# play-with-HOI-generation/HOIG

Hardware: AMD Instinct MI355X
Metric: HOGAN train images/sec at 256x256 (higher is better)
Workload: dtype f16x3 fwd (both operands split hi+lo on fp16, 3 MFMAs per product) / bf16x2 bwd (dy split hi+lo, weights and x single bf16, 2 MFMAs per product), f32 accumulate; 1 GPU; 256x256 HO3Dv3-shaped synthetic, batch 8 per GPU, G+D full step (generator_spade_attn, VGG19 surrogate weights); global_batch=8, parallelism=dp1

## Files before the change

### hoig_amd/_lib.py

```python
import ctypes
import os
import re
import subprocess

_HERE = os.path.dirname(os.path.abspath(__file__))
LIB_PATH = os.path.join(_HERE, 'csrc', '_build', 'libhoig_hip.so')
HEADER_PATH = os.path.join(os.path.dirname(_HERE), 'include', 'hoig_kernels.h')

OK, EINVAL, ELAUNCH, EUNSUPPORTED = 0, -1, -2, -3
ACT_NONE, ACT_RELU, ACT_LRELU, ACT_TANH, ACT_SIGMOID = 0, 1, 2, 3, 4
PREC_F32, PREC_BF16X3, PREC_BF16, PREC_F16X2, PREC_F16F6 = 0, 1, 2, 3, 4
LOSS_L1, LOSS_MSE, LOSS_BCE = 0, 1, 2
POOL_MAX, POOL_AVG = 0, 1
JPEG_SUBSEQ_BYTES = 64
_ERR = {EINVAL: 'invalid argument', ELAUNCH: 'kernel launch failed', EUNSUPPORTED: 'unsupported shape'}


class HoigKernelError(RuntimeError):
    pass


class ConvDesc(ctypes.Structure):
    _fields_ = [(n, ctypes.c_int32) for n in ('B', 'Hi', 'Wi', 'Ci', 'Ho', 'Wo', 'Co', 'R', 'S', 'stride', 'pad',
                                              'transposed', 'act')] + \
               [('slope', ctypes.c_float), ('precision', ctypes.c_int32)]


def build(verbose=False):
    script = os.path.join(_HERE, 'csrc', 'build.sh')
    out = subprocess.run(['bash', script], stdout=subprocess.PIPE, stderr=subprocess.STDOUT, text=True)
    if verbose or out.returncode != 0:
        print(out.stdout)
    if out.returncode != 0:
        raise RuntimeError('hipcc build of libhoig_hip.so failed')
    return LIB_PATH


def declared_symbols():
    text = open(HEADER_PATH).read()
    return sorted(set(re.findall(r'\b(hoig_[a-z0-9_]+)\s*\(', text)) - {'hoig_stream_t'})


_vp, _i, _i64, _f, _d = ctypes.c_void_p, ctypes.c_int, ctypes.c_int64, ctypes.c_float, ctypes.c_double
_SIGS = {
    'hoig_conv2d_fwd': [ctypes.POINTER(ConvDesc), _vp, _vp, _vp, _vp, _vp],
    'hoig_conv2d_bwd_data': [ctypes.POINTER(ConvDesc), _vp, _vp, _vp, _vp],
    'hoig_conv2d_fwd_heads': [ctypes.POINTER(ConvDesc), _vp, _vp, _vp, _vp, ctypes.c_uint64, _vp],
    'hoig_conv2d_bwd_weight': [ctypes.POINTER(ConvDesc), _vp, _vp, _vp, _vp, _vp],
    'hoig_pack_conv_weight_bf16': [_vp, _i, _i, _i, _i, _vp, _vp, _vp],
    'hoig_pack_conv_weights_bf16_all': [_vp, _vp, _i, _i64, _vp, _vp, _vp, _vp, _vp],
    'hoig_conv2d_fwd_packed': [ctypes.POINTER(ConvDesc), _vp, _vp, _vp, _vp, _vp, _vp],
    'hoig_conv2d_bwd_data_packed': [ctypes.POINTER(ConvDesc), _vp, _vp, _vp, _vp, _vp],
    'hoig_conv2d_fwd_packed_stats': [ctypes.POINTER(ConvDesc), _vp, _vp, _vp, _vp, _vp, _vp, _vp],
    'hoig_conv2d_fwd_stats': [ctypes.POINTER(ConvDesc), _vp, _vp, _vp, _vp, _vp, _vp],
    'hoig_conv2d_cat_fwd_packed_stats': [ctypes.POINTER(ConvDesc), _vp, _i, _vp, _vp, _vp, _vp, _vp, _vp, _vp],
    'hoig_inorm_stats_from_sums': [_vp, _i, _i, _i, _f, _vp, _vp, _vp, _vp],
    'hoig_conv2d_bwd_data_packed_add': [ctypes.POINTER(ConvDesc), _vp, _vp, _vp, _vp, _vp, _vp],
    'hoig_pack_conv_weight_f6': [_vp, _i, _i, _i, _vp, _vp, _vp],
    'hoig_conv2d_fwd_f6': [ctypes.POINTER(ConvDesc), _vp, _vp, _vp, _vp, _vp, _vp, _vp],
    'hoig_pack_conv_weights_f6_all': [_vp, _vp, _i, _i64, _vp, _vp, _vp],
    'hoig_conv2d_cat_fwd_f6': [ctypes.POINTER(ConvDesc), _vp, _i, _vp, _vp, _vp, _vp, _vp, _vp, _vp],
    'hoig_conv2d_fwd_f6_ex': [ctypes.POINTER(ConvDesc), _vp, _i, _vp, _vp, _vp, _vp, _vp, _vp, _vp, _i, _vp, _vp, _vp],
    'hoig_conv2d_cat_fwd_packed': [ctypes.POINTER(ConvDesc), _vp, _i, _vp, _vp, _vp, _vp, _vp, _vp],
    'hoig_conv2d_cat_bwd_data_packed': [ctypes.POINTER(ConvDesc), _vp, _vp, _vp, _vp, _i, _vp, _vp],
    'hoig_split_planes_bf16': [_vp, _vp, _i64, _i, _vp],
    'hoig_conv2d_bwd_weight_split': [ctypes.POINTER(ConvDesc), _vp, _vp, _vp, _vp],
    'hoig_conv2d_bwd_data_packed_split': [ctypes.POINTER(ConvDesc), _vp, _vp, _vp, _vp, _vp, _vp],
    'hoig_conv2d_fwd_packed_pair': [ctypes.POINTER(ConvDesc)] + [_vp] * 11,
    'hoig_conv2d_bwd_data_packed_split_pair': [ctypes.POINTER(ConvDesc)] + [_vp] * 11,
    'hoig_conv2d_bwd_weight_split_pair': [ctypes.POINTER(ConvDesc)] + [_vp] * 7,
    'hoig_conv2d_cat_bwd_weight': [ctypes.POINTER(ConvDesc), _vp, _i, _vp, _vp, _vp, _vp, _vp],
    'hoig_inorm_stats': [_vp, _i, _i, _i, _f, _vp, _vp, _vp, _vp],
    'hoig_inorm_apply': [_vp, _vp, _vp, _i, _vp, _vp, _i, _f, _vp, _vp, _i, _i, _i, _vp],
    'hoig_inorm_apply_ld': [_vp, _vp, _vp, _i, _vp, _vp, _i, _i, _f, _vp, _vp, _i, _i, _i, _vp],
    'hoig_inorm_bwd_ld': [_vp, _vp, _vp, _i, _vp, _vp, _i, _vp, _vp, _i, _f, _vp, _vp, _vp, _i, _i, _i, _vp, _vp],
    'hoig_inorm_fwd_fused': [_vp, _i, _vp, _vp, _i, _i, _f, _vp, _f, _vp, _vp, _vp, _i, _i, _i, _vp],
    'hoig_inorm_bwd_fused': [_vp, _vp, _vp, _i, _vp, _vp, _i, _vp, _vp, _i, _f, _vp, _vp, _vp, _i, _i, _i, _vp],
    'hoig_inorm_bwd_add_ld': [_vp, _vp, _vp, _i, _vp, _vp, _i, _vp, _vp, _i, _f, _vp, _vp, _vp, _vp, _i, _i, _i, _vp, _vp],
    'hoig_inorm_bwd_add_ld_split': [_vp, _vp, _vp, _i, _vp, _vp, _i, _vp, _vp, _i, _f, _vp, _vp, _vp, _vp, _i, _i, _i, _vp, _vp],
    'hoig_inorm_bwd_fused_add_split': [_vp, _vp, _vp, _i, _vp, _vp, _i, _vp, _vp, _i, _f, _vp, _vp, _vp, _vp, _i, _i, _i, _vp],
    'hoig_inorm_fold': [_vp, _vp, _vp, _vp, _i, _i, _vp, _vp, _i, _vp],
    'hoig_conv2d_fwd_packed_normin': [_vp, _vp, _i, _vp, _vp, _vp, _vp, _vp, _vp, _i, _vp, _vp, _vp],
    'hoig_unsplit_planes_bf16': [_vp, _vp, _i64, _i, _vp],
    'hoig_inorm_bwd_fused_add': [_vp, _vp, _vp, _i, _vp, _vp, _i, _vp, _vp, _i, _f, _vp, _vp, _vp, _vp, _i, _i, _i, _vp],
    'hoig_inorm_bwd': [_vp, _vp, _vp, _i, _vp, _vp, _vp, _vp, _i, _f, _vp, _vp, _vp, _i, _i, _i, _vp, _vp],
    'hoig_replicate_pad_fwd': [_vp, _vp, _i, _i, _i, _i, _i, _vp],
    'hoig_replicate_pad_bwd': [_vp, _vp, _i, _i, _i, _i, _i, _vp],
    'hoig_replicate_pad_bwd_add': [_vp, _vp, _vp, _i, _i, _i, _i, _i, _vp],
    'hoig_attn_pixel_fwd': [_vp] * 10 + [_i, _i, _i, _i, _vp],
    'hoig_attn_pixel_bwd': [_vp] * 10 + [_i, _i, _i, _i, _vp],
    'hoig_attn_build_index': [_vp, _vp, _i, _i, _i, _vp],
    'hoig_attn_src_gather': [_vp, _vp, _vp, _vp, _vp, _i, _i, _i, _i, _vp],
    'hoig_attn_gs_gather': [_vp, _vp, _vp, _vp, _i, _i, _i, _vp],
    'hoig_block_extractor_forward': [_vp, _vp, _vp] + [_i] * 7 + [_vp],
    'hoig_block_extractor_backward': [_vp] * 5 + [_i] * 7 + [_vp],
    'hoig_local_attn_reshape_forward': [_vp, _vp] + [_i] * 4 + [_vp],
    'hoig_local_attn_reshape_backward': [_vp, _vp] + [_i] * 4 + [_vp],
    'hoig_grid_sample_fwd': [_vp, _vp, _vp] + [_i] * 6 + [_vp],
    'hoig_grid_sample_bwd': [_vp, _vp, _vp] + [_i] * 6 + [_vp],
    'hoig_resize_bilinear_ac': [_vp, _vp] + [_i] * 6 + [_vp],
    'hoig_resize_nearest': [_vp, _vp] + [_i] * 6 + [_vp],
    'hoig_attn_flow': [_vp, _vp, _i, _i, _vp],
    'hoig_maxpool2_fwd': [_vp, _vp] + [_i] * 4 + [_vp],
    'hoig_maxpool2_bwd': [_vp, _vp, _vp, _vp] + [_i] * 4 + [_vp],
    'hoig_nchw_to_nhwc': [_vp, _vp] + [_i] * 4 + [_vp],
    'hoig_nhwc_to_nchw': [_vp, _vp] + [_i] * 4 + [_vp],
    'hoig_copy_channels': [_vp, _vp, _i64, _i, _i, _i, _i, _i, _i, _vp],
    'hoig_cat2_channels': [_vp, _i, _vp, _i, _vp, _i64, _vp],
    'hoig_add': [_vp, _vp, _vp, _i64, _vp],
    'hoig_add_act': [_vp, _vp, _vp, _i, _f, _i64, _vp],
    'hoig_act_bwd': [_vp, _vp, _vp, _i, _f, _i64, _vp],
    'hoig_act_bwd_colsum': [_vp, _vp, _vp, _vp, _i, _f, _i64, _i, _vp],
    'hoig_colsum_accum': [_vp, _vp, _i64, _i, _vp],
    'hoig_compose_fwd': [_vp] * 6 + [_i64, _i, _vp],
    'hoig_compose_bwd': [_vp] * 11 + [_i64, _i, _vp],
    'hoig_loss_fwd_bwd': [_i, _vp, _vp, _f, _f, _vp, _vp, _i64, _vp],
    'hoig_tv_fwd_bwd': [_vp, _f, _f, _vp, _vp, _i, _i, _i, _vp],
    'hoig_loss_accumulate': [_i, _vp, _vp, _f, _f, _vp, _vp, _i64, _vp],
    'hoig_tv_accumulate': [_vp, _f, _f, _vp, _vp, _i, _i, _i, _vp],
    'hoig_sum': [_vp, _vp, _i64, _vp],
    'hoig_sum_scaled': [_vp, _f, _vp, _i64, _vp],
    'hoig_adam_step': [_vp, _vp, _vp, _vp, _i64, _d, _d, _d, _d, _i, _f, _vp],
    'hoig_adam_tick': [_vp, _vp, _vp],
    'hoig_adam_step_dev': [_vp, _vp, _vp, _vp, _i64, _vp, _f, _vp],
    'hoig_resize_linear_u8': [_vp, _i, _i, _i, _i, _vp, _i, _i, _vp],
    'hoig_warp_affine_u8': [_vp, _i, _i, _i, _i, _vp, _i, _i, _i, _vp, _vp],
    'hoig_adam_pack_step': [_vp, _vp, _vp, _vp, _vp, _f, _vp, _i, _i64, _vp, _i64, _vp, _vp, _vp, _vp, _vp],
    'hoig_stream_create': [ctypes.POINTER(ctypes.c_void_p)],
    'hoig_stream_destroy': [_vp],
    'hoig_stream_scratch_set': [_vp, _vp, _i64],
    'hoig_tensor2im_u8': [_vp, _vp] + [_i] * 6 + [_vp],
    'hoig_tensor2im_nhwc_u8': [_vp, _vp, _i64, _i, _vp],
    'hoig_prep_texture': [_vp] * 9,
    'hoig_prep_lookup': [_vp] * 5 + [_i] + [_vp] * 8,
    'hoig_prep_assemble': [_i] + [_vp] * 17 + [_i] + [_vp] * 6,
    'hoig_rasterize_fim_wim': [_vp, _i, _i, _i, _f, _f, _vp, _vp, _vp, _vp],
    'hoig_pack_conv_weight_wino': [_vp, _i, _i, _vp, _vp, _vp],
    'hoig_conv2d_fwd_wino': [ctypes.POINTER(ConvDesc), _vp, _vp, _vp, _vp, _vp, _vp],
    'hoig_project_faces': [_vp, _i, _vp, _i, _vp, _vp, _i, _i, _f, _f, _vp, _vp],
    'hoig_prep_texture_batched': [_i, _vp, _vp, _i64, _vp, _vp, _vp, _vp, _vp, _vp, _vp],
    'hoig_prep_lookup_batched': [_i, _vp, _vp, _vp, _vp, _vp, _vp, _vp, _vp, _i64, _vp, _vp, _vp, _vp, _vp, _vp],
    'hoig_mano_lbs': [_vp, _vp, _vp, _vp, _vp, _vp, _vp, _vp, _vp, _i, _i, _vp, _vp, _vp, _vp, _vp, _i, _vp, _i, _vp],
    'hoig_pool2d_fwd': [_vp, _vp] + [_i] * 10 + [_vp],
    'hoig_stage_images_u8': [_vp, _vp] + [_i] * 7 + [_vp, _vp],
    'hoig_pad2d': [_vp, _vp] + [_i] * 6 + [_vp],
    'hoig_global_avgpool': [_vp, _vp, _i, _i, _i, _vp],
    'hoig_lpips_layer': [_vp, _vp, _vp, _vp, _i, _i, _i, _vp, _vp],
    'hoig_ssim': [_vp, _vp, _vp, _vp, _i, _i, _i, _i, _f, _f, _f, _i, _f, _vp, _vp],
    'hoig_jpeg_entropy_host': [_vp, _i64, _vp, _i, _vp, _i64, _vp, _i64, _vp],
    'hoig_jpeg_decode_bgr_u8': [_vp, _i64, _vp, _vp, _i, _vp, _i64, _vp, _i64, _vp, _vp, _i64, _vp],
    'hoig_jpeg_reconstruct_bgr_u8': [_vp, _vp, _i, _vp, _i64, _vp, _i64, _vp],
    'hoig_jpeg_entropy_par_host': [_vp, _i64, _vp, _i, _vp, _i64, _i, _i, _vp, _i64, _vp, _vp, _vp, _i64],
    'hoig_jpeg_decode_bgr_u8_par': [_vp, _i64, _vp, _vp, _i, _vp, _i64, _vp, _i64, _vp, _vp, _i64, _i, _vp],
    'hoig_pil_bilinear_ksize': [_i, _i],
    'hoig_pil_bilinear_table': [_i, _i, _vp],
    'hoig_resize_pil_bilinear_u8_host': [_vp, _i, _i, _i, _i, _vp, _i, _i],
    'hoig_resize_pil_bilinear_u8': [_vp, _i, _i, _i, _i, _vp, _i, _i, _vp, _vp, _vp, _vp],
}


def _load():
    if not os.path.exists(LIB_PATH):
        raise ImportError(
            'hoig_amd: %s not found. The HIP extension is mandatory (no CPU / eager fallback exists); build it with '
            '`python -c "import __graft_entry__ as g; g.build()"` or `bash hoig_amd/csrc/build.sh`.' % LIB_PATH)
    lib = ctypes.CDLL(LIB_PATH)
    for name, args in _SIGS.items():
        fn = getattr(lib, name)
        fn.argtypes = args
        fn.restype = ctypes.c_int
    lib.hoig_inorm_workspace_bytes.argtypes = [_i, _i, _i]
    lib.hoig_inorm_workspace_bytes.restype = ctypes.c_int64
    lib.hoig_set_f6_min_tiles.argtypes = [_i]
    lib.hoig_set_f6_min_tiles.restype = ctypes.c_int
    lib.hoig_f6_plane_bytes.argtypes = [_i, _i, _i]
    lib.hoig_f6_plane_bytes.restype = ctypes.c_int64
    lib.hoig_wino_plane_halfs.argtypes = [_i, _i]
    lib.hoig_wino_plane_halfs.restype = ctypes.c_int64
    lib.hoig_attn_index_ints.argtypes = [_i, _i, _i]
    lib.hoig_attn_index_ints.restype = ctypes.c_int64
    lib.hoig_rasterize_workspace_bytes.restype = ctypes.c_size_t
    lib.hoig_rasterize_workspace_bytes.argtypes = [ctypes.c_int, ctypes.c_int]
    lib.hoig_set_tuning.argtypes = [ctypes.c_char_p, _i]
    lib.hoig_set_tuning.restype = ctypes.c_int
    lib.hoig_stream_scratch_bytes.argtypes = []
    lib.hoig_stream_scratch_bytes.restype = ctypes.c_int64
    lib.hoig_conv2d_bwd_weight_scratch_bytes.argtypes = [ctypes.POINTER(ConvDesc)]
# ... 46 lines not shown
```

### hoig_amd/csrc/conv_bf16_common.h

```cpp
#pragma once
#include "common.h"

namespace hoig_detail {

#define HOIG_NS_SWITCH(ns, ...)                                                \
    do {                                                                       \
        if ((ns) == 2) { constexpr int NSX = 2; __VA_ARGS__; }                 \
        else if ((ns) == 3) { constexpr int NSX = 3; __VA_ARGS__; }            \
        else { constexpr int NSX = 1; __VA_ARGS__; }                           \
    } while (0)
__host__ __device__ constexpr int ns_a(int nsx) { return nsx == 1 ? 1 : 2; }
__host__ __device__ constexpr int ns_b(int nsx) { return nsx == 2 ? 2 : 1; }
inline int ns_of_precision(int precision) {
    return precision == HOIG_PREC_BF16X3 ? 2 : (precision == HOIG_PREC_F16X2 ? 3 : 1);
}
inline bool is_16bit_precision(int precision) {
    return precision == HOIG_PREC_BF16X3 || precision == HOIG_PREC_BF16 || precision == HOIG_PREC_F16X2;
}

typedef __bf16 bf2_t __attribute__((ext_vector_type(2)));
typedef float f2_t __attribute__((ext_vector_type(2)));
__device__ __forceinline__ unsigned cvt2(float a, float b) {
    f2_t v = {a, b};
    return __builtin_bit_cast(unsigned, __builtin_convertvector(v, bf2_t));
}
typedef _Float16 h2_t __attribute__((ext_vector_type(2)));
typedef _Float16 f16x8 __attribute__((ext_vector_type(8)));
constexpr float W_SCALE_F16 = 256.f;
__device__ __forceinline__ unsigned cvt2h(float a, float b) {
    f2_t v = {a, b};
    return __builtin_bit_cast(unsigned, __builtin_convertvector(v, h2_t));
}
__device__ __forceinline__ void split4h(const float4 v, uint2 &hi, uint2 &lo) {
    hi.x = cvt2h(v.x, v.y);
    hi.y = cvt2h(v.z, v.w);
    const h2_t h0 = __builtin_bit_cast(h2_t, hi.x), h1 = __builtin_bit_cast(h2_t, hi.y);
    lo.x = cvt2h(v.x - (float)h0[0], v.y - (float)h0[1]);
    lo.y = cvt2h(v.z - (float)h1[0], v.w - (float)h1[1]);
}
template <bool F16>
__device__ __forceinline__ f32x16 mfma16(const bf16x8 a, const bf16x8 b, const f32x16 c) {
    if constexpr (F16)
        return __builtin_amdgcn_mfma_f32_32x32x16_f16(__builtin_bit_cast(f16x8, a), __builtin_bit_cast(f16x8, b), c, 0, 0, 0);
    else
        return __builtin_amdgcn_mfma_f32_32x32x16_bf16(a, b, c, 0, 0, 0);
}

__device__ __forceinline__ void split4(const float4 v, uint2 &hi, uint2 &lo) {
    hi.x = cvt2(v.x, v.y);
    hi.y = cvt2(v.z, v.w);
    const float r0 = v.x - __uint_as_float(hi.x << 16), r1 = v.y - __uint_as_float(hi.x & 0xFFFF0000u);
    const float r2 = v.z - __uint_as_float(hi.y << 16), r3 = v.w - __uint_as_float(hi.y & 0xFFFF0000u);
    lo.x = cvt2(r0, r1);
    lo.y = cvt2(r2, r3);
}
template <bool F16>
__device__ __forceinline__ void split4t(const float4 v, uint2 &hi, uint2 &lo) {
    if constexpr (F16) split4h(v, hi, lo);
    else split4(v, hi, lo);
}

__host__ __device__ __forceinline__ size_t plane_index(int n, int k, int K) {
    return ((size_t)(n >> 5) * (K >> 5) + (k >> 5)) * 1024 + (n & 31) * 32 + (((((k & 31) >> 3) ^ ((n >> 2) & 3))) << 3) +
           (k & 7);
}

struct HaloArgs {
    const float *A;
    const unsigned short *Wh, *Wl;
    const float *bias;
    float *C;
    int Bn, H, W, Cg;
    int N, K;
    int pad;
    int flip;
    int act;
    float slope;
    int nblk_n, nblk;
    int tiles_x, tiles_y;
    int nmajor;
    int f16;
    float oscale;
    const float *A2;
    int cg1;
    float *C2;
    int n1;
    const float *addend;
    const float *in_scale = nullptr, *in_shift = nullptr;
    int in_relu_c0 = 0;
    int b_split;
    const float *A_g2;
    const unsigned short *Wh_g2, *Wl_g2;
    const float *bias_g2, *addend_g2;
    float *C_g2;
    int a_split;
    double *stats;
};

struct Geom {
    int Bn, Hg, Wg, Cg;
    int Hp, Wp;
    int R, S, stride, pad;
    int gatherT, phase_major, tile_skip;
};

struct Args {
    const float *A;
    const unsigned short *Wh;
    const unsigned short *Wl;
    const float *bias;
    float *C;
    Geom g;
    int M, N, K;
    int act;
    float slope;
    int nblk_n, nblk;
    int ksplit, steps_per_split;
    int f16;
    float oscale;
};

__device__ __forceinline__ void decode_m(const Geom &g, int m, int &b, int &hp, int &wp) {
    if (!g.phase_major) {
        const int hw = g.Hp * g.Wp;
        b = m / hw;
        const int rem = m - b * hw;
        hp = rem / g.Wp;
        wp = rem - hp * g.Wp;
    } else {
        const int W2 = g.Wp >> 1, q = (g.Hp >> 1) * W2, bq = g.Bn * q;
        const int ph = m / bq;
        const int rem = m - ph * bq;
        b = rem / q;
        const int r2 = rem - b * q;
        const int h2 = r2 / W2;
        hp = 2 * h2 + (ph >> 1);
        wp = 2 * (r2 - h2 * W2) + (ph & 1);
    }
}
__device__ __forceinline__ int row_base(const Geom &g, int p) { return g.gatherT ? p + g.pad : p * g.stride - g.pad; }
__device__ __forceinline__ int gcoord(const Geom &g, int base, int r, int lim) {
    if (!g.gatherT) {
        const int c = base + r;
        return (c >= 0 && c < lim) ? c : -1;
    }
    int t = base - r;
    if (t < 0) return -1;
    if (g.stride == 2) {
        if (t & 1) return -1;
        t >>= 1;
    } else if (g.stride != 1) {
        if (t % g.stride) return -1;
        t /= g.stride;
    }
    return t < lim ? t : -1;
}
__device__ __forceinline__ bool tap_alive(const Geom &g, int hp, int wp, int rs) {
    const int r = rs / g.S, s = rs - r * g.S;
    return (((hp + g.pad - r) & 1) == 0) && (((wp + g.pad - s) & 1) == 0);
}

struct WFlatArgs {
    const float *X, *DY;
    float *DW, *DB;
    int Ci, Co, Wc, HWc, Q, Ho, Wo, HPOS;
    int nblk_ci, nblk, n_mtiles, mt_per_split;
};
int launch_wgrad_flat5(const float *x, const float *dy, float *dw, float *dbias, int Bn, int Hi, int Wi, int Ci, int Co, int ns,
                       hipStream_t st);

int launch_igemm_m16(Args a, int ns, int cfg, hipStream_t st);

struct FlatArgs {
    const float *A;
    const unsigned short *Wh, *Wl;
    const float *bias;
    float *C;
    const float *addend;
    int Bn, Hc, Wc;
    int Hs, Ws, oy, ox;
    int Hd, Wd;
    int KS, Cg, N, K, flip, f16;
    int act;
    float slope, oscale;
    int HWc, Q, HP;
    int nblk, nblk_n, steps_per_split;
};
int launch_flat_m16(FlatArgs a, int ns, hipStream_t st);
int launch_halo5_m16(FlatArgs a, int ns, hipStream_t st);

struct WHaloArgs {
    const float *DY, *X, *X2;
    int ci1;
    float *DW, *DB;
    int Bn, H, W, Co, Ci;
    int Hin, Win, pad;
    int tout;
    int tiles_x, tiles_y, n_mtiles, mt_per_split;
    int nblk_ci, nblk;
    int b_split;
    const float *DY_g2, *X_g2;
    float *DW_g2;
};

int launch_halo_s2_m16p(const HaloArgs &a, int ns, bool scatter, bool rows8, hipStream_t st);
int launch_dgrad_thin(const float *dy, const unsigned short *wh, const unsigned short *wl, float *dx, int M, int N, int ns, hipStream_t st);
int launch_wgrad_dma(const WHaloArgs &a, int ns, dim3 grid, hipStream_t st);

int launch_halo3_m16(HaloArgs a, int ns, int bn, hipStream_t st);
int launch_halo_s2_m16(const HaloArgs &a, int ns, bool scatter, hipStream_t st);

}
```

### hoig_amd/csrc/conv_flat16.hip

```cpp
#include "conv_bf16_common.h"
#include "tuning.h"

namespace hoig_detail {
namespace {

template <bool F16>
__device__ __forceinline__ f32x4 mfma_m16(const bf16x8 a, const bf16x8 b, const f32x4 c) {
    if constexpr (F16)
        return __builtin_amdgcn_mfma_f32_16x16x32_f16(__builtin_bit_cast(f16x8, a), __builtin_bit_cast(f16x8, b), c, 0, 0, 0);
    else
        return __builtin_amdgcn_mfma_f32_16x16x32_bf16(a, b, c, 0, 0, 0);
}
typedef unsigned u2_t __attribute__((ext_vector_type(2)));
constexpr int round128(int v) { return (v + 127) / 128 * 128; }

constexpr int PT = 256, BN = 128, TPS = 3, HSL = 8;
constexpr int W23 = BN * 32 + 64, PLANE_W = round128(W23 + BN * 32);

template <int NSX, int KS, bool F16, bool SPLITK, bool WDMA = false>
__global__ __launch_bounds__(512) void conv_flat_m16_kernel(const FlatArgs p) {
    constexpr int NS = NSX == 1 ? 1 : 2, NB = NSX == 2 ? 2 : 1;
    constexpr int NT = 512, WN = 2, MT = 4, NTW = 4, KK = KS * KS;
    constexpr int NGRP = (KK + TPS - 1) / TPS;
    constexpr int BBUF = TPS * NB * PLANE_W;
// ... 164 lines not shown
                    } else {
                        if (NS == 2) acc[j][m] = mfma_m16<F16>(wc.h, pc.l[m], acc[j][m]);
                        if (NB == 2) acc[j][m] = mfma_m16<F16>(wc.l, pc.h[m], acc[j][m]);
                        acc[j][m] = mfma_m16<F16>(wc.h, pc.h[m], acc[j][m]);
                    }
                }
                __builtin_amdgcn_sched_barrier(0);
            }
        }
        if constexpr (WDMA) {
            if (dma_step >= 0) {
#pragma unroll
                for (int i = 0; i < NPW; ++i)
                    if (i >= ntap * NTW) dma_piece(dma_step, bbuf ^ 1, i);
            }
        }
    };

    if (T > 0) {
        halo_load(s_begin / NGRP);
        halo_store();
        if constexpr (WDMA) {
#pragma unroll
            for (int i = 0; i < NPW; ++i) dma_piece(0, 0, i);
        } else {
            load_b(0);
            store_b(0);
            if (T > 1) load_b(1);
        }
    }
    if constexpr (WDMA) asm volatile("s_waitcnt vmcnt(0)" ::: "memory");
    __syncthreads();
    int bbuf = 0;
#pragma unroll 1
    for (int step = 0; step < T; ++step) {
        const int cb = (s_begin + step) / NGRP, g = (s_begin + step) - cb * NGRP;
        const bool more = step + 1 < T;
        const bool boundary = more && g == NGRP - 1;
        if constexpr (!WDMA) {
            if (more) store_b(bbuf ^ 1);
            if (step + 2 < T) load_b(step + 2);
        }
        if (boundary) halo_load(cb + 1);
        compute(g, bbuf, (WDMA && more) ? step + 1 : -1);
        if (boundary) {
            __syncthreads();
            halo_store();
        }
        if constexpr (WDMA) asm volatile("s_waitcnt vmcnt(0)" ::: "memory");
        __syncthreads();
        bbuf ^= 1;
    }

    auto dest = [&](int q) -> long {
        if (q >= p.Q) return -1;
        const int b = q / p.HWc, rem = q - b * p.HWc;
        const int y = rem / p.Wc, x = rem - y * p.Wc;
        if (y >= p.Hd || x >= p.Wd) return -1;
        return ((long)(b * p.Hd + y) * p.Wd + x) * p.N;
    };
    if (!SPLITK) {
        const float nslope = p.act == HOIG_ACT_NONE ? 1.f : (p.act == HOIG_ACT_RELU ? 0.f : p.slope);
        const bool special = p.act == HOIG_ACT_TANH || p.act == HOIG_ACT_SIGMOID;
#pragma unroll
        for (int m = 0; m < MT; ++m) {
            const long d = dest(q0 + wm * 64 + m * 16 + l15);
            if (d < 0) continue;
#pragma unroll
            for (int j = 0; j < NTW; ++j) {
                const int n = n0 + wn * 64 + j * 16 + lg * 4;
                if (n < p.N) {
                    float4 o = make_float4(acc[j][m][0] * p.oscale, acc[j][m][1] * p.oscale, acc[j][m][2] * p.oscale,
                                           acc[j][m][3] * p.oscale);
                    if (p.bias) {
                        const float4 bv = *reinterpret_cast<const float4 *>(p.bias + n);
                        o.x += bv.x; o.y += bv.y; o.z += bv.z; o.w += bv.w;
                    }
                    o.x = fast_act(o.x, nslope, special, p.act, p.slope); o.y = fast_act(o.y, nslope, special, p.act, p.slope);
                    o.z = fast_act(o.z, nslope, special, p.act, p.slope); o.w = fast_act(o.w, nslope, special, p.act, p.slope);
                    if (p.addend) {
                        const float4 ad = *reinterpret_cast<const float4 *>(p.addend + d + n);
                        o.x += ad.x; o.y += ad.y; o.z += ad.z; o.w += ad.w;
                    }
                    *reinterpret_cast<float4 *>(p.C + d + n) = o;
                }
            }
        }
    } else {
        const int l31 = lane & 31, lh = lane >> 5;
#pragma unroll
        for (int m = 0; m < MT; ++m)
#pragma unroll
            for (int r = 0; r < 4; ++r) {
                long d[2];
#pragma unroll
                for (int h = 0; h < 2; ++h) d[h] = dest(q0 + wm * 64 + m * 16 + r + 8 * lh + 4 * h);
#pragma unroll
                for (int j = 0; j < NTW; j += 2) {
                    const int n = n0 + wn * 64 + j * 16 + l31;
                    const u2_t sw = __builtin_amdgcn_permlane16_swap(__float_as_uint(acc[j][m][r]), __float_as_uint(acc[j + 1][m][r]),
                                                                     false, false);
#pragma unroll
                    for (int h = 0; h < 2; ++h)
                        if (d[h] >= 0 && n < p.N) {
                            float v = __uint_as_float(sw[h]) * p.oscale;
                            if (blockIdx.y == 0 && p.bias) v += p.bias[n];
                            atomicAdd(p.C + d[h] + n, v);
                        }
                }
            }
    }
}

template <int NSX, int KS, bool F16, bool SPLITK>
int launch_one(const FlatArgs &a, dim3 grid, size_t shm, hipStream_t st) {
    if (hoig_tuning(HOIG_TUNE_WDMA16) >= 2) {
        static hoig_once once_d;
        if (!once_d.done()) {
            if (hipFuncSetAttribute(reinterpret_cast<const void *>(&conv_flat_m16_kernel<NSX, KS, F16, SPLITK, true>),
                                    hipFuncAttributeMaxDynamicSharedMemorySize, 160 * 1024) != hipSuccess)
                return HOIG_ELAUNCH;
            once_d.set();
        }
        conv_flat_m16_kernel<NSX, KS, F16, SPLITK, true><<<grid, 512, shm, st>>>(a);
        HOIG_LAUNCH_CHECK();
        return HOIG_OK;
    }
    static hoig_once once;
    if (!once.done()) {
        if (hipFuncSetAttribute(reinterpret_cast<const void *>(&conv_flat_m16_kernel<NSX, KS, F16, SPLITK>),
                                hipFuncAttributeMaxDynamicSharedMemorySize, 160 * 1024) != hipSuccess)
            return HOIG_ELAUNCH;
        once.set();
    }
    conv_flat_m16_kernel<NSX, KS, F16, SPLITK><<<grid, 512, shm, st>>>(a);
    HOIG_LAUNCH_CHECK();
    return HOIG_OK;
}

template <int KS>
int launch_ks(const FlatArgs &a, int ns, dim3 grid, size_t shm, bool split, hipStream_t st) {
    if (split) {
        if (a.f16) HOIG_NS_SWITCH(ns, return launch_one<NSX, KS, true, true>(a, grid, shm, st));
        else HOIG_NS_SWITCH(ns, return launch_one<NSX, KS, false, true>(a, grid, shm, st));
    }
    if (a.f16) HOIG_NS_SWITCH(ns, return launch_one<NSX, KS, true, false>(a, grid, shm, st));
    else HOIG_NS_SWITCH(ns, return launch_one<NSX, KS, false, false>(a, grid, shm, st));
    return HOIG_EINVAL;
}

}

int launch_flat_m16(FlatArgs a, int ns, hipStream_t st) {
    const int KS = a.KS;
    if ((KS != 3 && KS != 5) || a.N % 128 || a.Cg % 32) return HOIG_EUNSUPPORTED;
    a.HWc = a.Hc * a.Wc;
    a.Q = a.Bn * a.HWc;
    a.HP = PT + (KS - 1) * (a.Wc + 1);
    if (a.HP * 8 > HSL * 512) return HOIG_EUNSUPPORTED;
    const int p23 = round128(a.HP * 32) + 64, plane_p = round128(p23 + a.HP * 32);
    const size_t shm = (size_t)ns_a(ns) * plane_p + 2 * TPS * ns_b(ns) * PLANE_W;
    if (shm > 160 * 1024) return HOIG_EUNSUPPORTED;
    const int n_mt = (int)hoig_cdiv(a.Q, PT);
    a.nblk_n = a.N / BN;
    a.nblk = n_mt * a.nblk_n;
    const int ncb = a.Cg >> 5;
    const int steps = ncb * ((KS * KS + TPS - 1) / TPS);
    int split = 1;
    if (a.nblk <= 128 && !a.addend && a.act == HOIG_ACT_NONE) {
        split = 256 / a.nblk;
        if (split > steps / 8) split = steps / 8;
        if (split < 1) split = 1;
    }
    a.steps_per_split = (int)hoig_cdiv(steps, split);
    split = (int)hoig_cdiv(steps, a.steps_per_split);
    dim3 grid(a.nblk, split);
    if (split > 1 && hipMemsetAsync(a.C, 0, (size_t)a.Bn * a.Hd * a.Wd * a.N * sizeof(float), st) != hipSuccess) return HOIG_ELAUNCH;
    return KS == 3 ? launch_ks<3>(a, ns, grid, shm, split > 1, st) : launch_ks<5>(a, ns, grid, shm, split > 1, st);
}

}
```

### hoig_amd/csrc/conv_halo16.hip

```cpp
#include "conv_bf16_common.h"
#include "conv_m16_common.h"
#include "tuning.h"

namespace hoig_detail {
namespace {

template <int WM, int BN>
struct M16Layout {
    static constexpr int TH = 2 * WM, HW = 34, HPIX = (TH + 2) * HW;
    static constexpr int PHALF = HPIX * 32;
    static constexpr int P23 = round128(PHALF) + 64;
    static constexpr int PLANE_P = round128(P23 + PHALF);
    static constexpr int W23 = BN * 32 + 64;
    static constexpr int PLANE_W = round128(W23 + BN * 32);
    static constexpr size_t bytes(int nsx) { return (size_t)ns_a(nsx) * PLANE_P + 2 * 3 * ns_b(nsx) * PLANE_W; }
};

template <int NSX, int WM, int WN, int BN, bool F16, bool ASPLIT = false, bool WDMA = false, bool NORMIN = false>
__global__ __launch_bounds__(64 * WM * WN) void conv_halo3_m16_kernel(const HaloArgs p) {
    constexpr int NS = NSX == 1 ? 1 : 2, NB = NSX == 2 ? 2 : 1;
    using LY = M16Layout<WM, BN>;
    constexpr int KS = 3, TH = LY::TH, HW = LY::HW, HPIX = LY::HPIX;
    constexpr int NT = 64 * WM * WN;
    constexpr int P23 = LY::P23, PLANE_P = LY::PLANE_P, W23 = LY::W23, PLANE_W = LY::PLANE_W;
// ... 219 lines not shown
            if (t + 1 < KS) {
#pragma unroll
                for (int q = 0; q < PPG; ++q)
                    if (j * PPG + q < MT) read_p(pf[(t + 1) & 1], t + 1, j * PPG + q);
            }
            if constexpr (WDMA) {
                if (dma_step >= 0 && g < NPW) dma_piece(dma_step, bbuf ^ 1, g);
            }
            __builtin_amdgcn_sched_barrier(0);
            const PF &pc = pf[t & 1];
            const WF &wc = wf[g & 1];
#pragma unroll
            for (int m = 0; m < MT; ++m) {
                if (NS == 2) acc[j][m] = mfma_m16<F16>(wc.h, pc.l[m], acc[j][m]);
                if (NB == 2) acc[j][m] = mfma_m16<F16>(wc.l, pc.h[m], acc[j][m]);
                acc[j][m] = mfma_m16<F16>(wc.h, pc.h[m], acc[j][m]);
            }
            __builtin_amdgcn_sched_barrier(0);
        }
    };

    halo_load(0);
    halo_store();
    if constexpr (WDMA) {
#pragma unroll
        for (int i = 0; i < NPW; ++i) dma_piece(0, 0, i);
        asm volatile("s_waitcnt vmcnt(0)" ::: "memory");
    } else {
        load_b(0);
        store_b(0);
        if (T > 1) load_b(1);
    }
    __syncthreads();
    int bbuf = 0;
#pragma unroll 1
    for (int step = 0; step < T; ++step) {
        const int cb = step / KS, r = step - cb * KS;
        const bool more = step + 1 < T;
        const bool boundary = more && r == KS - 1;
        if constexpr (!WDMA) {
            if (more) store_b(bbuf ^ 1);
            if (step + 2 < T) load_b(step + 2);
        }
        if (boundary) halo_load(cb + 1);
        compute(r, bbuf, (WDMA && more) ? step + 1 : -1);
        if (boundary) {
            __syncthreads();
            halo_store();
        }
        if constexpr (WDMA) asm volatile("s_waitcnt vmcnt(0)" ::: "memory");
        __syncthreads();
        bbuf ^= 1;
    }

    const float nslope = p.act == HOIG_ACT_NONE ? 1.f : (p.act == HOIG_ACT_RELU ? 0.f : p.slope);
    const bool special = p.act == HOIG_ACT_TANH || p.act == HOIG_ACT_SIGMOID;
    float4 bias_r[NTW];
#pragma unroll
    for (int j = 0; j < NTW; ++j) {
        const int n = n0 + wn * (NTW * 16) + j * 16 + lg * 4;
        bias_r[j] = (gbias && n < p.N) ? *reinterpret_cast<const float4 *>(gbias + n) : make_float4(0.f, 0.f, 0.f, 0.f);
    }
    float st1[NTW][4], st2[NTW][4];
#pragma unroll
    for (int j = 0; j < NTW; ++j)
#pragma unroll
        for (int q = 0; q < 4; ++q) st1[j][q] = st2[j][q] = 0.f;
#pragma unroll
    for (int m = 0; m < MT; ++m) {
        const int oy = y0 + wm * 2 + (m >> 1), ox = x0 + (m & 1) * 16 + l15;
        const size_t pix = ((size_t)bi * p.H + oy) * p.W + ox;
#pragma unroll
        for (int j = 0; j < NTW; ++j) {
            const int n = n0 + wn * (NTW * 16) + j * 16 + lg * 4;
            if (n < p.N) {
                float v[4];
                const float bq[4] = {bias_r[j].x, bias_r[j].y, bias_r[j].z, bias_r[j].w};
#pragma unroll
                for (int q = 0; q < 4; ++q) v[q] = fast_act(acc[j][m][q] * p.oscale + bq[q], nslope, special, p.act, p.slope);
                if (gadd) {
                    const float4 ad = *reinterpret_cast<const float4 *>(gadd + pix * p.N + n);
                    v[0] += ad.x; v[1] += ad.y; v[2] += ad.z; v[3] += ad.w;
                }
#pragma unroll
                for (int q = 0; q < 4; ++q) {
                    st1[j][q] += v[q];
                    st2[j][q] += v[q] * v[q];
                }
                const float4 o = make_float4(v[0], v[1], v[2], v[3]);
                if (!p.C2) *reinterpret_cast<float4 *>(gC + pix * p.N + n) = o;
                else if (n < p.n1) *reinterpret_cast<float4 *>(gC + pix * p.n1 + n) = o;
                else *reinterpret_cast<float4 *>(p.C2 + pix * (p.N - p.n1) + (n - p.n1)) = o;
            }
        }
    }
    if (p.stats) m16_stats_epilogue<NTW, WM, BN, NT>(st1, st2, smem, p.stats, b, p.N, n0, wm, wn, lane, tid);
}

template <int NSX, int BN, bool SCATTER, bool F16>
__global__ __launch_bounds__(256) void conv_halo_s2_m16_kernel(const HaloArgs p) {
    constexpr int NS = NSX == 1 ? 1 : 2, NB = NSX == 2 ? 2 : 1;
    constexpr int TH = 4, TW = 32, NT = 256, WN = 2;
    constexpr int RB = BN * 4 / NT;
    constexpr int HH = TH + 1, HW = TW + 1, HPIX = HH * HW;
    constexpr int PHALF = HPIX * 32, P23 = round128(PHALF) + 64, PLANE_P = round128(P23 + PHALF);
    constexpr int W23 = BN * 32 + 64, PLANE_W = round128(W23 + BN * 32);
    constexpr int MT = 4, NTW = BN / (16 * WN);
    __shared__ __attribute__((aligned(16))) unsigned char smem[NS * PLANE_P + 2 * NB * PLANE_W];
    unsigned char *Ph = smem, *Pl = smem + PLANE_P;
    unsigned char *Wbase = smem + NS * PLANE_P;

    const int tid = threadIdx.x, lane = tid & 63, wave = tid >> 6;
    const int l15 = lane & 15, lg = lane >> 4;
    const int wm = wave / WN, wn = wave % WN;
    int tile = hoig_xcd_remap(blockIdx.x, p.nblk);
    int P = 0, Q = 0;
    if (SCATTER) {
        P = (tile >> 1) & 1;
        Q = tile & 1;
        tile >>= 2;
    }
    int mt_ = tile / p.nblk_n;
    const int n0 = (tile % p.nblk_n) * BN;
    const int tx_ = mt_ % p.tiles_x;
    mt_ /= p.tiles_x;
    const int ty_ = mt_ % p.tiles_y, b = mt_ / p.tiles_y;
    const int y0 = ty_ * TH, x0 = tx_ * TW;

    const int brow = tid >> 2, bpos = tid & 3;
    const unsigned short *wrow_h[RB], *wrow_l[RB];
    int woff[RB];
#pragma unroll
    for (int i = 0; i < RB; ++i) {
        const int row = brow + (NT / 4) * i;
        const int n = n0 + row;
        const size_t o = ((size_t)(n >> 5) * (p.K >> 5)) * 1024 + (n & 31) * 32 + bpos * 8;
        wrow_h[i] = n < p.N ? p.Wh + o : nullptr;
        wrow_l[i] = (NB == 2 && n < p.N) ? p.Wl + o : nullptr;
        const int c = bpos ^ ((row >> 2) & 3);
        woff[i] = (c >> 1) * W23 + row * 32 + (c & 1) * 16;
    }
    int wread[NTW], pread[MT];
#pragma unroll
    for (int j = 0; j < NTW; ++j) wread[j] = (lg >> 1) * W23 + (wn * (NTW * 16) + j * 16 + l15) * 32 + (lg & 1) * 16;
#pragma unroll
    for (int m = 0; m < MT; ++m)
        pread[m] = (lg >> 1) * P23 + ((wm * 2 + (m >> 1)) * HW + (m & 1) * 16 + l15) * 32 + (lg & 1) * 16;

    f32x4 acc[NTW][MT];
#pragma unroll
    for (int j = 0; j < NTW; ++j)
#pragma unroll
        for (int m = 0; m < MT; ++m) acc[j][m] = f32x4{0.f, 0.f, 0.f, 0.f};

    struct Step {
        int cb, ntap, tap[2], pp, qq;
        bool load;
    };
    const int spc = SCATTER ? ((P ? 2 : 1) * (Q ? 2 : 1) + 1) / 2 : 5;
    const int ncb = p.Cg >> 5, T = ncb * spc;
    auto step_info = [&](int step) -> Step {
        Step s_;
        s_.cb = step / spc;
        const int idx = step - s_.cb * spc;
        s_.pp = s_.qq = 0;
        if (!SCATTER) {
// ... 307 lines not shown
```

### hoig_amd/csrc/conv_igemm_bf16.hip

```cpp
#include "conv_bf16_common.h"
#include "tuning.h"
#include <cstdlib>

#ifndef HOIG_HALO_BSTAGES
#define HOIG_HALO_BSTAGES 1
#endif

namespace {
using namespace hoig_detail;


template <int BK>
__device__ __forceinline__ int lds_swz(int row) {
    return BK == 32 ? ((row >> 2) & 3) : ((row >> 1) & 7);
}
template <int BK>
__device__ __forceinline__ int lds_off(int row, int k) {
    return row * (BK * 2) + (((k >> 3) ^ lds_swz<BK>(row)) << 4) + ((k & 4) << 1);
}

template <int BM, int BN, int WM, int WN, int NSX, int BK, bool F16>
__global__ __launch_bounds__(WM * WN * 64) void igemm_bf16_kernel(const Args p) {
    constexpr int NS = NSX == 1 ? 1 : 2, NB = NSX == 2 ? 2 : 1;
    constexpr int NT = WM * WN * 64;
// ... 847 lines not shown
            if (more) load_b(step + 1);
            if (boundary) halo_load(cb + 1);
            compute(r, 0, 0);
            if (more) {
                __syncthreads();
                if (boundary) halo_store(0);
                store_b(0);
                __syncthreads();
            }
        }
    }

    const float nslope = p.act == HOIG_ACT_NONE ? 1.f : (p.act == HOIG_ACT_RELU ? 0.f : p.slope);
    const bool special = p.act == HOIG_ACT_TANH || p.act == HOIG_ACT_SIGMOID;
    float bias_r[TN];
#pragma unroll
    for (int j = 0; j < TN; ++j) {
        const int n = n0 + wn * (TN * 32) + j * 32 + l31;
        bias_r[j] = (p.bias && n < p.N) ? p.bias[n] : 0.f;
    }
    float st1[TN], st2[TN];
#pragma unroll
    for (int j = 0; j < TN; ++j) st1[j] = st2[j] = 0.f;
#pragma unroll
    for (int i = 0; i < TM; ++i) {
        const int oy = y0 + wm * TM + i;
#pragma unroll
        for (int r = 0; r < 16; ++r) {
            const int ox = x0 + (r & 3) + 8 * (r >> 2) + 4 * lh;
            const size_t pix = ((size_t)b * p.H + oy) * p.W + ox;
#pragma unroll
            for (int j = 0; j < TN; ++j) {
                const int n = n0 + wn * (TN * 32) + j * 32 + l31;
                if (n < p.N) {
                    float v = acc[i][j][r] * p.oscale;
                    v += bias_r[j];
                    v = fast_act(v, nslope, special, p.act, p.slope);
                    if (p.addend) v += p.addend[pix * p.N + n];
                    st1[j] += v;
                    st2[j] += v * v;
                    if (!p.C2) p.C[pix * p.N + n] = v;
                    else if (n < p.n1) p.C[pix * p.n1 + n] = v;
                    else p.C2[pix * (p.N - p.n1) + (n - p.n1)] = v;
                }
            }
        }
    }
    if (p.stats) halo_stats_epilogue<TN, WM, WN, NT>(st1, st2, smem, p.stats, b, p.N, n0, wm, wn, lane);
}

template <int NS, int WM, int WN, int BN, int MODE>
int launch_halo3_one(const HaloArgs &a, hipStream_t st) {
    constexpr int HPIX = (2 * WM + 2) * 34;
    constexpr size_t shm = (MODE == 1 ? 2 : 1) * (ns_a(NS) * (HPIX * 80)) + (MODE == 0 ? 1 : 2) * (3 * ns_b(NS) * (BN * 64));
    static hoig_once once;
    if (!once.done()) {
        if (hipFuncSetAttribute(reinterpret_cast<const void *>(&conv_halo3_bf16_kernel<NS, WM, WN, BN, MODE, true>),
                                hipFuncAttributeMaxDynamicSharedMemorySize, (int)shm) != hipSuccess ||
            hipFuncSetAttribute(reinterpret_cast<const void *>(&conv_halo3_bf16_kernel<NS, WM, WN, BN, MODE, false>),
                                hipFuncAttributeMaxDynamicSharedMemorySize, (int)shm) != hipSuccess)
            return HOIG_ELAUNCH;
        once.set();
    }
    if (a.f16) conv_halo3_bf16_kernel<NS, WM, WN, BN, MODE, true><<<a.nblk, 64 * WM * WN, shm, st>>>(a);
    else conv_halo3_bf16_kernel<NS, WM, WN, BN, MODE, false><<<a.nblk, 64 * WM * WN, shm, st>>>(a);
    HOIG_LAUNCH_CHECK();
    return HOIG_OK;
}


int launch_halo3(HaloArgs a, int ns, hipStream_t st) {
    a.tiles_x = a.W / 32;
    a.tiles_y = a.H / 4;
    a.nmajor = 1;
    const bool n64 = (a.N % 128) != 0 || (a.C2 && a.n1 % 128 != 0);
    a.nblk_n = (int)hoig_cdiv(a.N, n64 ? 64 : 128);
    a.nblk = a.Bn * a.tiles_x * a.tiles_y * a.nblk_n;
    if (n64) {
        if (a.H % 8 == 0 && a.nblk / 2 >= 256) {
            a.tiles_y = a.H / 8;
            a.nblk = a.Bn * a.tiles_x * a.tiles_y * a.nblk_n;
            return launch_halo3_m16(a, ns, 64, st);
        }
        if (a.a_split || a.b_split || a.in_scale) return HOIG_EUNSUPPORTED;
        HOIG_NS_SWITCH(ns, return launch_halo3_one<NSX, 2, 2, 64, 0>(a, st));
    }
    if (a.H % 8 == 0 && a.nblk / 2 < 256 && a.nblk >= 192 && a.N % 128 == 0) {
        a.tiles_y = a.H / 8;
        a.nblk = a.Bn * a.tiles_x * a.tiles_y * a.nblk_n;
        return launch_halo3_m16(a, ns, 128, st);
    }
    if (a.H % 8 == 0 && a.nblk / 2 < 256 && a.nblk >= 192) {
        a.tiles_y = a.H / 8;
        a.nblk_n = a.N / 64;
        a.nblk = a.Bn * a.tiles_x * a.tiles_y * a.nblk_n;
        return launch_halo3_m16(a, ns, 64, st);
    }
    if (a.H % 8 == 0 && a.nblk / 2 >= 256) {
        a.tiles_y = a.H / 8;
        a.nblk = a.Bn * a.tiles_x * a.tiles_y * a.nblk_n;
        return launch_halo3_m16(a, ns, 128, st);
    }
    if (a.a_split || a.b_split || a.in_scale) return HOIG_EUNSUPPORTED;
    const bool wide = a.nblk < 384;
    HOIG_NS_SWITCH(ns, return wide ? launch_halo3_one<NSX, 2, 4, 128, 1>(a, st) : launch_halo3_one<NSX, 2, 2, 128, 0>(a, st));
    return HOIG_EINVAL;
}

template <int NSX, int BN, bool SCATTER, bool F16>
__global__ __launch_bounds__(256) void conv_halo_s2_bf16_kernel(const HaloArgs p) {
    constexpr int NS = NSX == 1 ? 1 : 2, NB = NSX == 2 ? 2 : 1;
    constexpr int TH = 4, TW = 32, NT = 256, WN = 2;
    constexpr int RB = BN * 4 / NT;
    constexpr int HH = TH + 1, HW = TW + 1, HPIX = HH * HW;
    constexpr int AROW = 80;
    constexpr int PLANE_A = HPIX * AROW, PLANE_B = BN * 64;
    constexpr int TM = 2, TN = BN / (32 * WN);
    __shared__ __attribute__((aligned(16))) unsigned char smem[NS * PLANE_A + 2 * NB * PLANE_B];
    unsigned char *Ah = smem, *Al = smem + PLANE_A;
    unsigned char *Bbase = smem + NS * PLANE_A;

    const int tid = threadIdx.x, lane = tid & 63, wave = tid >> 6;
    const int l31 = lane & 31, lh = lane >> 5;
    const int wm = wave / WN, wn = wave % WN;
    int tile = hoig_xcd_remap(blockIdx.x, p.nblk);
    int P = 0, Q = 0;
    if (SCATTER) {
        P = (tile >> 1) & 1;
        Q = tile & 1;
        tile >>= 2;
    }
    int mt = tile / p.nblk_n;
    const int n0 = (tile % p.nblk_n) * BN;
    const int tx_ = mt % p.tiles_x;
    mt /= p.tiles_x;
    const int ty_ = mt % p.tiles_y, b = mt / p.tiles_y;
    const int y0 = ty_ * TH, x0 = tx_ * TW;

    const int brow = tid >> 2, bchunk = tid & 3;
    const unsigned short *wrow_h[RB], *wrow_l[RB];
    int boff[RB];
#pragma unroll
    for (int i = 0; i < RB; ++i) {
        const int n = n0 + brow + (NT / 4) * i;
        const size_t o = plane_index(n, bchunk * 8, p.K);
        wrow_h[i] = n < p.N ? p.Wh + o : nullptr;
        wrow_l[i] = (NB == 2 && n < p.N) ? p.Wl + o : nullptr;
        const int row = brow + (NT / 4) * i;
        boff[i] = row * 64 + ((bchunk ^ ((row >> 2) & 3)) << 4);
    }
    int aread[TM], bread[TN];
#pragma unroll
    for (int i = 0; i < TM; ++i) aread[i] = ((wm * TM + i) * HW + l31) * AROW + lh * 16;
#pragma unroll
    for (int j = 0; j < TN; ++j) {
        const int row = wn * (TN * 32) + j * 32 + l31;
        bread[j] = row * 64 + ((lh ^ ((row >> 2) & 3)) << 4);
    }
    f32x16 acc[TM][TN];
#pragma unroll
    for (int i = 0; i < TM; ++i)
#pragma unroll
        for (int j = 0; j < TN; ++j)
#pragma unroll
            for (int r = 0; r < 16; ++r) acc[i][j][r] = 0.f;

    struct Step {
        int cb, ntap, tap[2], pp, qq;
        bool load;
    };
    const int spc = SCATTER ? ((P ? 2 : 1) * (Q ? 2 : 1) + 1) / 2 : 5;
    const int ncb = p.Cg >> 5, T = ncb * spc;
    auto step_info = [&](int step) -> Step {
        Step s_;
        s_.cb = step / spc;
        const int idx = step - s_.cb * spc;
        s_.pp = s_.qq = 0;
        if (!SCATTER) {
            s_.load = idx != 1;
            switch (idx) {
                case 0: s_.pp = 1; s_.qq = 1; s_.ntap = 2; s_.tap[0] = 0; s_.tap[1] = 2; break;
                case 1: s_.pp = 1; s_.qq = 1; s_.ntap = 2; s_.tap[0] = 6; s_.tap[1] = 8; break;
                case 2: s_.pp = 1; s_.qq = 0; s_.ntap = 2; s_.tap[0] = 1; s_.tap[1] = 7; break;
                case 3: s_.pp = 0; s_.qq = 1; s_.ntap = 2; s_.tap[0] = 3; s_.tap[1] = 5; break;
                default: s_.ntap = 1; s_.tap[0] = 4; s_.tap[1] = 4; break;
            }
// ... 177 lines not shown
                    st2[j] += v * v;
                    p.C[pix * p.N + n] = v;
                }
            }
        }
    }
    if (p.stats) halo_stats_epilogue<TN, 2, WN, NT>(st1, st2, smem, p.stats, b, p.N, n0, wm, wn, lane);
}

template <bool SCATTER>
int launch_halo_s2(HaloArgs a, int ns, hipStream_t st) {
    const int ch = SCATTER ? a.H : a.H / 2, cw = SCATTER ? a.W : a.W / 2;
    a.tiles_x = cw / 32;
    a.tiles_y = ch / 4;
    const bool n64 = (a.N % 128) != 0;
    a.nblk_n = a.N / (n64 ? 64 : 128);
    a.nblk = a.Bn * a.tiles_x * a.tiles_y * a.nblk_n * (SCATTER ? 4 : 1);
    a.nmajor = 0;
    if (hoig_tuning(HOIG_TUNE_S2_16) != 0 && !(SCATTER && n64 && ns == 2)) return launch_halo_s2_m16(a, ns, SCATTER, st);
    if (n64) {
        if (a.f16) HOIG_NS_SWITCH(ns, conv_halo_s2_bf16_kernel<NSX, 64, SCATTER, true><<<a.nblk, 256, 0, st>>>(a));
        else HOIG_NS_SWITCH(ns, conv_halo_s2_bf16_kernel<NSX, 64, SCATTER, false><<<a.nblk, 256, 0, st>>>(a));
    } else {
        if (a.f16) HOIG_NS_SWITCH(ns, conv_halo_s2_bf16_kernel<NSX, 128, SCATTER, true><<<a.nblk, 256, 0, st>>>(a));
        else HOIG_NS_SWITCH(ns, conv_halo_s2_bf16_kernel<NSX, 128, SCATTER, false><<<a.nblk, 256, 0, st>>>(a));
    }
    HOIG_LAUNCH_CHECK();
    return HOIG_OK;
}

template <int KS>
int launch_halo(HaloArgs a, int ns, hipStream_t st) {
    a.tiles_x = a.W / 32;
    a.tiles_y = a.H / 4;
    const bool n64 = (a.N % 128) != 0;
    a.nblk_n = (int)hoig_cdiv(a.N, n64 ? 64 : 128);
    a.nblk = a.Bn * a.tiles_x * a.tiles_y * a.nblk_n;
    if (n64) {
        if (a.f16) HOIG_NS_SWITCH(ns, conv_halo_bf16_kernel<KS, NSX, 2, 64, true><<<a.nblk, 256, 0, st>>>(a));
        else HOIG_NS_SWITCH(ns, conv_halo_bf16_kernel<KS, NSX, 2, 64, false><<<a.nblk, 256, 0, st>>>(a));
        HOIG_LAUNCH_CHECK();
        return HOIG_OK;
    }
    const bool wide = a.nblk < 384;
    if (wide) {
        if (a.f16) HOIG_NS_SWITCH(ns, conv_halo_bf16_kernel<KS, NSX, 4, 128, true><<<a.nblk, 512, 0, st>>>(a));
        else HOIG_NS_SWITCH(ns, conv_halo_bf16_kernel<KS, NSX, 4, 128, false><<<a.nblk, 512, 0, st>>>(a));
    } else {
        if (a.f16) HOIG_NS_SWITCH(ns, conv_halo_bf16_kernel<KS, NSX, 2, 128, true><<<a.nblk, 256, 0, st>>>(a));
        else HOIG_NS_SWITCH(ns, conv_halo_bf16_kernel<KS, NSX, 2, 128, false><<<a.nblk, 256, 0, st>>>(a));
    }
    HOIG_LAUNCH_CHECK();
    return HOIG_OK;
}

struct InNorm {
    const float *scale, *shift;
    int relu_c0;
};
struct PairSet {
    const float *a;
    const unsigned short *wh, *wl;
    const float *bias, *addend;
    float *c;
};

struct Conv {
    const hoig_conv_desc *d = nullptr;
    const float *a = nullptr;
    const unsigned short *wh = nullptr, *wl = nullptr;
    const float *bias = nullptr;
    float *c = nullptr;
    bool dgrad = false;
    hipStream_t st = nullptr;
    const float *a2 = nullptr;
    int cg1 = 0;
    float *c2 = nullptr;
    int n1 = 0;
    const float *addend = nullptr;
    double *stats = nullptr;
    bool a_split = false;
    const PairSet *g2 = nullptr;
    const InNorm *in = nullptr;
};

int run(const Conv &q) {
    const hoig_conv_desc *d = q.d;
    const float *a = q.a, *bias = q.bias, *a2 = q.a2, *addend = q.addend;
    const unsigned short *wh = q.wh, *wl = q.wl;
    float *c = q.c, *c2 = q.c2;
    const bool dgrad = q.dgrad, a_split = q.a_split;
    const int cg1 = q.cg1, n1 = q.n1;
    double *stats = q.stats;
    const PairSet *g2 = q.g2;
    const InNorm *in = q.in;
    hipStream_t st = q.st;
    if (in && (dgrad || d->R != 3 || d->S != 3 || d->stride != 1 || d->pad != 1 || d->transposed || a_split || g2))
        return HOIG_EUNSUPPORTED;
    Args p;
    p.A = a; p.Wh = wh; p.Wl = wl; p.bias = bias; p.C = c;
    p.f16 = dgrad ? 0 : 1;
    p.oscale = dgrad ? 1.f : 1.f / W_SCALE_F16;
    Geom &g = p.g;
    g.Bn = d->B;
    if (!dgrad) {
        g.Hg = d->Hi; g.Wg = d->Wi; g.Cg = d->Ci; g.Hp = d->Ho; g.Wp = d->Wo;
        g.gatherT = d->transposed ? 1 : 0;
        p.M = d->B * d->Ho * d->Wo; p.N = d->Co; p.K = d->R * d->S * d->Ci;
        p.act = d->act; p.slope = d->slope;
    } else {
        g.Hg = d->Ho; g.Wg = d->Wo; g.Cg = d->Co; g.Hp = d->Hi; g.Wp = d->Wi;
        g.gatherT = d->transposed ? 0 : 1;
        p.M = d->B * d->Hi * d->Wi; p.N = d->Ci; p.K = d->R * d->S * d->Co;
        p.act = HOIG_ACT_NONE; p.slope = 0.f;
    }
    g.R = d->R; g.S = d->S; g.stride = d->stride; g.pad = d->pad;
    g.phase_major = 0; g.tile_skip = 0;
    if (g.Cg % 32 != 0) return HOIG_EUNSUPPORTED;
    if (g.gatherT && g.stride == 2 && ((g.Hp | g.Wp) & 1)) return HOIG_EUNSUPPORTED;
    const int ns = ns_of_precision(d->precision);
    if (ns == 2 && !wl) return HOIG_EINVAL;
    const long t128 = hoig_cdiv(p.M, 128);
    if (p.N <= 32 || p.N % 32 != 0) return HOIG_EUNSUPPORTED;
    if (dgrad && !d->transposed && d->R == 1 && d->S == 1 && d->stride == 1 && d->pad == 0 && g.Cg == 128 &&
        p.N >= 1024 && p.N % 64 == 0 && p.M % 128 == 0 && !a2 && !c2 && !addend && !stats)
        return launch_dgrad_thin(a, wh, wl, c, p.M, p.N, ns, st);
    if (!d->transposed && d->stride == 1 && d->R == d->S && 2 * d->pad == d->R - 1 && (d->R == 1 || d->R == 3 || d->R == 5) &&
        d->Wi % 32 == 0 && d->Hi % 4 == 0 && p.N % 64 == 0 &&
        (long)(g2 ? 2 : 1) * d->B * (d->Hi / 4) * (d->Wi / 32) * ((p.N + 127) / 128) >= 160) {
        HaloArgs h;
        h.b_split = 0;
        h.A_g2 = nullptr; h.Wh_g2 = h.Wl_g2 = nullptr; h.bias_g2 = h.addend_g2 = nullptr; h.C_g2 = nullptr;
        h.A = a; h.Wh = wh; h.Wl = wl; h.bias = bias; h.C = c;
        h.A2 = a2; h.cg1 = cg1; h.C2 = c2; h.n1 = n1;
        h.addend = addend;
        h.stats = stats;
        h.a_split = a_split ? 1 : 0;
        h.in_scale = in ? in->scale : nullptr; h.in_shift = in ? in->shift : nullptr; h.in_relu_c0 = in ? in->relu_c0 : 0;
        if (a_split && (d->R != 3 || a2 || !dgrad)) return HOIG_EUNSUPPORTED;
        if ((addend || stats) && c2) return HOIG_EUNSUPPORTED;
        if (stats && d->R != 3) return HOIG_EUNSUPPORTED;
        if ((a2 || c2) && d->R != 3) return HOIG_EUNSUPPORTED;
        if (a2 && (cg1 % 32 || cg1 <= 0 || cg1 >= g.Cg)) return HOIG_EINVAL;
        if (c2 && (n1 % 64 || n1 <= 0 || n1 >= p.N)) return HOIG_EINVAL;
        h.Bn = d->B; h.H = d->Hi; h.W = d->Wi; h.Cg = g.Cg; h.N = p.N; h.K = p.K;
        if (g2) {
            if (d->R != 3 || a2 || c2 || stats) return HOIG_EUNSUPPORTED;
            h.Bn = 2 * d->B; h.b_split = d->B;
            h.A_g2 = g2->a; h.Wh_g2 = g2->wh; h.Wl_g2 = g2->wl; h.bias_g2 = g2->bias; h.addend_g2 = g2->addend; h.C_g2 = g2->c;
        }
        h.pad = d->pad;
        h.flip = dgrad ? 1 : 0;
        h.act = p.act; h.slope = p.slope;
            h.f16 = p.f16; h.oscale = p.oscale;
        if (d->R == 1) return launch_halo<1>(h, ns, st);
        if (d->R == 3) return launch_halo3(h, ns, st);
        return launch_halo<5>(h, ns, st);
    }
    if (a2 || c2 || a_split || g2 || in) return HOIG_EUNSUPPORTED;
    if (hoig_tuning(HOIG_TUNE_FLAT5) >= 2 && !d->transposed && d->stride == 1 && d->R == 3 && d->S == 3 && d->pad == 1 &&
        p.N % 128 == 0 && !stats) {
        FlatArgs f;
        f.A = a; f.Wh = wh; f.Wl = wl; f.bias = bias; f.C = c; f.addend = addend;
        f.Bn = d->B; f.Hc = d->Hi + 2; f.Wc = d->Wi + 2; f.KS = 3; f.act = p.act; f.slope = p.slope;
        f.Cg = g.Cg; f.N = p.N; f.K = p.K; f.flip = dgrad ? 1 : 0; f.f16 = p.f16; f.oscale = p.oscale;
        f.Hs = d->Hi; f.Ws = d->Wi; f.oy = f.ox = 1; f.Hd = d->Hi; f.Wd = d->Wi;
        const int rc = launch_flat_m16(f, ns, st);
        if (rc != HOIG_EUNSUPPORTED) return rc;
    }
    if (hoig_tuning(HOIG_TUNE_FLAT5) != 0 && !d->transposed && d->stride == 1 && d->R == 5 && d->S == 5 && d->pad == 0 &&
        d->Ho == d->Hi - 4 && d->Wo == d->Wi - 4 && p.N % 128 == 0 && !stats) {
        FlatArgs f;
        f.A = a; f.Wh = wh; f.Wl = wl; f.bias = bias; f.C = c; f.addend = addend;
        f.Bn = d->B; f.Hc = d->Hi; f.Wc = d->Wi; f.KS = 5; f.act = p.act; f.slope = p.slope;
        f.Cg = g.Cg; f.N = p.N; f.K = p.K; f.flip = dgrad ? 1 : 0; f.f16 = p.f16; f.oscale = p.oscale;
        if (!dgrad) {
            f.Hs = d->Hi; f.Ws = d->Wi; f.oy = f.ox = 0; f.Hd = d->Ho; f.Wd = d->Wo;
        } else {
            f.Hs = d->Ho; f.Ws = d->Wo; f.oy = f.ox = 4; f.Hd = d->Hi; f.Wd = d->Wi;
        }
        const int rc = launch_flat_m16(f, ns, st);
        if (rc != HOIG_EUNSUPPORTED) return rc;
        if (hoig_tuning(HOIG_TUNE_HALO5) != 0) {
            const int rc5 = launch_halo5_m16(f, ns, st);
            if (rc5 != HOIG_EUNSUPPORTED) return rc5;
        }
    }
    if (d->stride == 2 && d->R == 3 && d->S == 3 && d->pad == 1 && d->Hi % 2 == 0 && d->Wi % 2 == 0 &&
        p.N % 64 == 0) {
        const int fine_h = d->transposed ? d->Ho : d->Hi, fine_w = d->transposed ? d->Wo : d->Wi;
        const int coarse_h = d->transposed ? d->Hi : d->Ho, coarse_w = d->transposed ? d->Wi : d->Wo;
        if (fine_h == 2 * coarse_h && fine_w == 2 * coarse_w && coarse_w % 32 == 0 && coarse_h % 4 == 0) {
            HaloArgs h;
            h.A = a; h.Wh = wh; h.Wl = wl; h.bias = bias; h.C = c;
            h.Bn = d->B; h.Cg = g.Cg; h.N = p.N; h.K = p.K;
            h.pad = 1; h.flip = 0;
            h.A2 = nullptr; h.cg1 = 0; h.C2 = nullptr; h.n1 = 0; h.addend = addend; h.stats = stats; h.a_split = 0;
            h.b_split = 0;
            h.act = p.act; h.slope = p.slope;
            h.f16 = p.f16; h.oscale = p.oscale;
            const bool gather = !g.gatherT;
            if (gather) {
                h.H = fine_h; h.W = fine_w;
                return launch_halo_s2<false>(h, ns, st);
            }
            h.H = coarse_h; h.W = coarse_w;
            return launch_halo_s2<true>(h, ns, st);
        }
    }
    if (addend || stats) return HOIG_EUNSUPPORTED;
    const int t16 = hoig_tuning(HOIG_TUNE_IGEMM16);
    const bool m16 = t16 >= 2 || (t16 == 1 && !dgrad);
    if (p.N <= 64) {
        if (t128 >= 512) return m16 ? launch_igemm_m16(p, ns, 3, st) : launch<128, 64, 2, 2>(p, ns, st);
        return m16 ? launch_igemm_m16(p, ns, 4, st) : launch<64, 64, 2, 2>(p, ns, st);
    }
    const long n128 = hoig_cdiv(p.N, 128);
    if (t128 * n128 >= 512) return m16 ? launch_igemm_m16(p, ns, 0, st) : launch<128, 128, 2, 2>(p, ns, st);
    if (t128 * n128 >= 128) return m16 ? launch_igemm_m16(p, ns, 1, st) : launch<128, 128, 2, 4>(p, ns, st);
    return m16 ? launch_igemm_m16(p, ns, 2, st) : launch<64, 128, 2, 2>(p, ns, st);
}

}

extern "C" int hoig_pack_conv_weight_bf16(const float *w, int Co, int RS, int Ci, int for_dgrad, uint16_t *hi,
                                          uint16_t *lo, hoig_stream_t stream) {
    if (!w || !hi || Co <= 0 || RS <= 0 || Ci <= 0) return HOIG_EINVAL;
    if ((Co & 31) || (Ci & 31)) return HOIG_EUNSUPPORTED;
    const int64_t n = (int64_t)Co * RS * Ci;
    pack_weight_kernel<<<hoig_stream_grid(n, 256), 256, 0, (hipStream_t)stream>>>(w, Co, RS, Ci, for_dgrad ? 1 : 0, hi, lo);
    HOIG_LAUNCH_CHECK();
    return HOIG_OK;
}

extern "C" int hoig_pack_conv_weights_bf16_all(const float *flat, const int64_t *segs, int nseg, int64_t ntiles,
                                               uint16_t *hi_f, uint16_t *lo_f, uint16_t *hi_d, uint16_t *lo_d,
                                               hoig_stream_t stream) {
    if (!flat || !segs || nseg <= 0 || ntiles <= 0 || !hi_f || !lo_f || !hi_d || !lo_d) return HOIG_EINVAL;
    pack_all_kernel<<<(unsigned)ntiles, 256, 0, (hipStream_t)stream>>>(flat, segs, nseg, hi_f, lo_f, hi_d, lo_d);
    HOIG_LAUNCH_CHECK();
    return HOIG_OK;
}

extern "C" int hoig_adam_pack_step(float *flat, const float *grad, float *exp_avg, float *exp_avg_sq, const float *derived,
                                   float grad_scale, const int64_t *segs, int nseg, int64_t ntiles, const int64_t *plain,
                                   int64_t nplain, uint16_t *hi_f, uint16_t *lo_f, uint16_t *hi_d, uint16_t *lo_d,
                                   hoig_stream_t stream) {
    if (!flat || !grad || !exp_avg || !exp_avg_sq || !derived || !segs || nseg <= 0 || ntiles <= 0 || nplain < 0 || (nplain && !plain) ||
        !hi_f || !lo_f || !hi_d || !lo_d)
        return HOIG_EINVAL;
    adam_pack_kernel<<<(unsigned)(ntiles + nplain), 256, 0, (hipStream_t)stream>>>(flat, grad, exp_avg, exp_avg_sq, derived, grad_scale, segs,
                                                                                 nseg, ntiles, plain, hi_f, lo_f, hi_d, lo_d);
    HOIG_LAUNCH_CHECK();
    return HOIG_OK;
}

extern "C" int hoig_conv2d_fwd_packed(const hoig_conv_desc *d, const float *x, const uint16_t *w_hi, const uint16_t *w_lo,
                                      const float *bias, float *y, hoig_stream_t stream) {
    if (!d || !x || !w_hi || !y) return HOIG_EINVAL;
    if (!is_16bit_precision(d->precision)) return HOIG_EINVAL;
    return run(Conv{.d = d, .a = x, .wh = w_hi, .wl = w_lo, .bias = bias, .c = y, .st = (hipStream_t)stream});
}

extern "C" int hoig_conv2d_bwd_data_packed(const hoig_conv_desc *d, const float *dy, const uint16_t *wt_hi,
                                           const uint16_t *wt_lo, float *dx, hoig_stream_t stream) {
    if (!d || !dy || !wt_hi || !dx) return HOIG_EINVAL;
    if (!is_16bit_precision(d->precision)) return HOIG_EINVAL;
    return run(Conv{.d = d, .a = dy, .wh = wt_hi, .wl = wt_lo, .c = dx, .dgrad = true, .st = (hipStream_t)stream});
}

extern "C" int hoig_conv2d_fwd_packed_stats(const hoig_conv_desc *d, const float *x, const uint16_t *w_hi, const uint16_t *w_lo,
                                            const float *bias, float *y, double *stats, hoig_stream_t stream) {
    if (!d || !x || !w_hi || !y || !stats) return HOIG_EINVAL;
    if (!is_16bit_precision(d->precision)) return HOIG_EINVAL;
    return run(Conv{.d = d, .a = x, .wh = w_hi, .wl = w_lo, .bias = bias, .c = y, .st = (hipStream_t)stream, .stats = stats});
}
extern "C" int hoig_conv2d_cat_fwd_packed_stats(const hoig_conv_desc *d, const float *x1, int C1, const float *x2,
                                                const uint16_t *w_hi, const uint16_t *w_lo, const float *bias, float *y,
                                                double *stats, hoig_stream_t stream) {
    if (!d || !x1 || !x2 || !w_hi || !y || !stats) return HOIG_EINVAL;
    if (!is_16bit_precision(d->precision)) return HOIG_EINVAL;
    return run(Conv{.d = d, .a = x1, .wh = w_hi, .wl = w_lo, .bias = bias, .c = y, .st = (hipStream_t)stream, .a2 = x2, .cg1 = C1, .stats = stats});
}

extern "C" int hoig_conv2d_fwd_packed_normin(const hoig_conv_desc *d, const float *x, int C1, const float *x2, const uint16_t *w_hi,
                                             const uint16_t *w_lo, const float *bias, const float *in_scale, const float *in_shift,
                                             int in_relu_c0, float *y, double *stats, hoig_stream_t stream) {
    if (!d || !x || !w_hi || !y || !in_scale || !in_shift || in_relu_c0 < 0) return HOIG_EINVAL;
    if (!is_16bit_precision(d->precision)) return HOIG_EINVAL;
    const InNorm in{in_scale, in_shift, in_relu_c0};
    return run(Conv{.d = d, .a = x, .wh = w_hi, .wl = w_lo, .bias = bias, .c = y, .st = (hipStream_t)stream, .a2 = x2, .cg1 = x2 ? C1 : 0,
                    .stats = stats, .in = &in});
}

extern "C" int hoig_conv2d_bwd_data_packed_add(const hoig_conv_desc *d, const float *dy, const uint16_t *wt_hi,
                                               const uint16_t *wt_lo, const float *addend, float *dx, hoig_stream_t stream) {
    if (!d || !dy || !wt_hi || !dx || !addend) return HOIG_EINVAL;
    if (!is_16bit_precision(d->precision)) return HOIG_EINVAL;
    return run(Conv{.d = d, .a = dy, .wh = wt_hi, .wl = wt_lo, .c = dx, .dgrad = true, .st = (hipStream_t)stream, .addend = addend});
}

extern "C" int hoig_conv2d_bwd_data_packed_split(const hoig_conv_desc *d, const uint16_t *dy_split, const uint16_t *wt_hi,
                                                 const uint16_t *wt_lo, const float *addend, float *dx, hoig_stream_t stream) {
    if (!d || !dy_split || !wt_hi || !dx) return HOIG_EINVAL;
    if (!is_16bit_precision(d->precision)) return HOIG_EINVAL;
    if (d->precision == HOIG_PREC_BF16X3 || d->transposed || d->stride != 1 || d->R != 3 || d->S != 3) return HOIG_EUNSUPPORTED;
    return run(Conv{.d = d, .a = reinterpret_cast<const float *>(dy_split), .wh = wt_hi, .wl = wt_lo, .c = dx, .dgrad = true,
                    .st = (hipStream_t)stream, .addend = addend, .a_split = true});
}

extern "C" int hoig_conv2d_fwd_packed_pair(const hoig_conv_desc *d, const float *xa, const float *xb, const uint16_t *wa_hi,
                                           const uint16_t *wa_lo, const uint16_t *wb_hi, const uint16_t *wb_lo, const float *bias_a,
                                           const float *bias_b, float *ya, float *yb, hoig_stream_t stream) {
    if (!d || !xa || !xb || !wa_hi || !wb_hi || !ya || !yb) return HOIG_EINVAL;
    if (!is_16bit_precision(d->precision)) return HOIG_EINVAL;
    if (d->transposed || d->stride != 1 || d->R != 3 || d->S != 3) return HOIG_EUNSUPPORTED;
    const PairSet g2{xb, wb_hi, wb_lo, bias_b, nullptr, yb};
    return run(Conv{.d = d, .a = xa, .wh = wa_hi, .wl = wa_lo, .bias = bias_a, .c = ya, .st = (hipStream_t)stream, .g2 = &g2});
}
extern "C" int hoig_conv2d_bwd_data_packed_split_pair(const hoig_conv_desc *d, const uint16_t *dys_a, const uint16_t *dys_b,
                                                      const uint16_t *wta_hi, const uint16_t *wta_lo, const uint16_t *wtb_hi,
                                                      const uint16_t *wtb_lo, const float *addend_a, const float *addend_b, float *dxa,
                                                      float *dxb, hoig_stream_t stream) {
    if (!d || !dys_a || !dys_b || !wta_hi || !wtb_hi || !dxa || !dxb) return HOIG_EINVAL;
    if (!is_16bit_precision(d->precision)) return HOIG_EINVAL;
    if (d->precision == HOIG_PREC_BF16X3 || d->transposed || d->stride != 1 || d->R != 3 || d->S != 3) return HOIG_EUNSUPPORTED;
    if ((addend_a == nullptr) != (addend_b == nullptr)) return HOIG_EINVAL;
    const PairSet g2{reinterpret_cast<const float *>(dys_b), wtb_hi, wtb_lo, nullptr, addend_b, dxb};
    return run(Conv{.d = d, .a = reinterpret_cast<const float *>(dys_a), .wh = wta_hi, .wl = wta_lo, .c = dxa, .dgrad = true,
                    .st = (hipStream_t)stream, .addend = addend_a, .a_split = true, .g2 = &g2});
}

extern "C" int hoig_conv2d_cat_fwd_packed(const hoig_conv_desc *d, const float *x1, int C1, const float *x2,
                                          const uint16_t *w_hi, const uint16_t *w_lo, const float *bias, float *y,
                                          hoig_stream_t stream) {
    if (!d || !x1 || !x2 || !w_hi || !y) return HOIG_EINVAL;
    if (!is_16bit_precision(d->precision)) return HOIG_EINVAL;
    return run(Conv{.d = d, .a = x1, .wh = w_hi, .wl = w_lo, .bias = bias, .c = y, .st = (hipStream_t)stream, .a2 = x2, .cg1 = C1});
}
extern "C" int hoig_conv2d_cat_bwd_data_packed(const hoig_conv_desc *d, const float *dy, const uint16_t *wt_hi,
                                               const uint16_t *wt_lo, float *dx1, int C1, float *dx2,
                                               hoig_stream_t stream) {
    if (!d || !dy || !wt_hi || !dx1 || !dx2) return HOIG_EINVAL;
    if (!is_16bit_precision(d->precision)) return HOIG_EINVAL;
    return run(Conv{.d = d, .a = dy, .wh = wt_hi, .wl = wt_lo, .c = dx1, .dgrad = true, .st = (hipStream_t)stream, .c2 = dx2, .n1 = C1});
}
```

### hoig_amd/csrc/pointwise.hip

```cpp
#include "common.h"
#include <cstdio>
#include <map>
#include <mutex>

namespace {
constexpr int NT = 256;

__device__ __forceinline__ float block_sum(float v) {
    __shared__ float part[NT / 64];
    v = hoig_wave_sum(v);
    const int lane = threadIdx.x & 63, w = threadIdx.x >> 6;
    __syncthreads();
    if (lane == 0) part[w] = v;
    __syncthreads();
    float s = 0.f;
#pragma unroll
    for (int i = 0; i < NT / 64; ++i) s += part[i];
    return s;
}

__global__ void transpose_kernel(const float *__restrict__ x, float *__restrict__ y, int rows, int cols) {
    __shared__ float t[32][33];
    const size_t base = (size_t)blockIdx.z * rows * cols;
    const int c0 = blockIdx.x * 32, r0 = blockIdx.y * 32;
// ... 62 lines not shown
        int64_t pix = e0 / Cy;
        int c = (int)(e0 - pix * Cy);
        float v[4];
#pragma unroll
        for (int k = 0; k < 4; ++k) {
            v[k] = c < C1 ? x1[pix * C1 + c] : x2[pix * C2 + (c - C1)];
            if (++c == Cy) {
                c = 0;
                ++pix;
            }
        }
        reinterpret_cast<float4 *>(y)[i] = make_float4(v[0], v[1], v[2], v[3]);
    }
    if (blockIdx.x == 0 && threadIdx.x < (ntotal & 3)) {
        const int64_t e = (n4 << 2) + threadIdx.x;
        const int64_t pix = e / Cy;
        const int c = (int)(e - pix * Cy);
        y[e] = c < C1 ? x1[pix * C1 + c] : x2[pix * C2 + (c - C1)];
    }
}

template <int VEC>
__global__ void cat2_kernel(const float *__restrict__ x1, int C1, const float *__restrict__ x2, int C2,
                            float *__restrict__ y, int64_t npix) {
    const int Cy = C1 + C2;
    if (VEC == 4) {
        const int Q1 = C1 >> 2, Qy = Cy >> 2;
        const int64_t n = npix * Qy;
        for (int64_t i = (int64_t)blockIdx.x * NT + threadIdx.x; i < n; i += (int64_t)gridDim.x * NT) {
            const int64_t p = i / Qy;
            const int q = (int)(i - p * Qy);
            const float4 v = q < Q1 ? reinterpret_cast<const float4 *>(x1)[p * Q1 + q]
                                    : reinterpret_cast<const float4 *>(x2)[p * (C2 >> 2) + (q - Q1)];
            reinterpret_cast<float4 *>(y)[i] = v;
        }
    } else {
        const int64_t n = npix * Cy;
        if (n < (int64_t)1 << 31) {
            const unsigned n32 = (unsigned)n, n4 = n32 >> 2, step = gridDim.x * NT, cy = (unsigned)Cy;
            const unsigned c1 = (unsigned)C1, c2 = (unsigned)C2;
            for (unsigned q = blockIdx.x * NT + threadIdx.x; q < n4; q += step) {
                float v[4];
#pragma unroll
                for (int k = 0; k < 4; ++k) {
                    const unsigned i = q * 4 + k, p = i / cy, c = i - p * cy;
                    v[k] = c < c1 ? x1[p * c1 + c] : x2[p * c2 + (c - c1)];
                }
                reinterpret_cast<float4 *>(y)[q] = make_float4(v[0], v[1], v[2], v[3]);
            }
            for (unsigned i = (n4 << 2) + blockIdx.x * NT + threadIdx.x; i < n32; i += step) {
                const unsigned p = i / cy, c = i - p * cy;
                y[i] = c < c1 ? x1[p * c1 + c] : x2[p * c2 + (c - c1)];
            }
            return;
        }
        for (int64_t i = (int64_t)blockIdx.x * NT + threadIdx.x; i < n; i += (int64_t)gridDim.x * NT) {
            const int64_t p = i / Cy;
            const int c = (int)(i - p * Cy);
            y[i] = c < C1 ? x1[p * C1 + c] : x2[p * C2 + (c - C1)];
        }
    }
}

__global__ void add_kernel(const float *__restrict__ a, const float *__restrict__ b, float *__restrict__ y, int64_t n) {
    const int64_t n4 = n >> 2;
    for (int64_t i = (int64_t)blockIdx.x * NT + threadIdx.x; i < n4; i += (int64_t)gridDim.x * NT) {
        const float4 u = reinterpret_cast<const float4 *>(a)[i], v = reinterpret_cast<const float4 *>(b)[i];
        reinterpret_cast<float4 *>(y)[i] = make_float4(u.x + v.x, u.y + v.y, u.z + v.z, u.w + v.w);
    }
    for (int64_t i = (n4 << 2) + (int64_t)blockIdx.x * NT + threadIdx.x; i < n; i += (int64_t)gridDim.x * NT)
        y[i] = a[i] + b[i];
}

__global__ void add_act_kernel(const float *__restrict__ a, const float *__restrict__ b, float *__restrict__ y, int act,
                               float slope, int64_t n) {
    for (int64_t i = (int64_t)blockIdx.x * NT + threadIdx.x; i < n; i += (int64_t)gridDim.x * NT)
        y[i] = hoig_act(a[i] + b[i], act, slope);
}

__global__ void act_bwd_kernel(const float *__restrict__ y, const float *__restrict__ dy, float *__restrict__ dx,
                               int act, float slope, int64_t n) {
    for (int64_t i = (int64_t)blockIdx.x * NT + threadIdx.x; i < n; i += (int64_t)gridDim.x * NT)
        dx[i] = dy[i] * hoig_act_grad_from_y(y[i], act, slope);
}

__global__ __launch_bounds__(NT) void act_bwd_colsum_kernel(const float *__restrict__ y, const float *__restrict__ dy,
                                                            float *__restrict__ g, float *__restrict__ dbias, int act,
                                                            float slope, int64_t rows, int C, int64_t rows_per_block) {
    const int64_t r0 = (int64_t)blockIdx.x * rows_per_block;
    const int64_t r1 = r0 + rows_per_block < rows ? r0 + rows_per_block : rows;
    const int lanes = C < NT ? C : NT;
    const int rl_n = NT / lanes;
    const int c0 = threadIdx.x % lanes, rl = threadIdx.x / lanes;
    extern __shared__ float red[];
    if (threadIdx.x < lanes * rl_n) {
        for (int c = c0; c < C; c += lanes) {
            float s = 0.f;
            for (int64_t r = r0 + rl; r < r1; r += rl_n) {
                const float v = dy[r * C + c] * hoig_act_grad_from_y(y[r * C + c], act, slope);
                g[r * C + c] = v;
                s += v;
            }
            red[rl * C + c] = s;
        }
    }
    __syncthreads();
    for (int c = threadIdx.x; c < C; c += NT) {
        float s = 0.f;
        for (int k = 0; k < rl_n; ++k) s += red[k * C + c];
        atomicAdd(&dbias[c], s);
    }
}

template <bool FUSED>
__global__ __launch_bounds__(NT) void colsum4_kernel(const float *__restrict__ y, const float *__restrict__ dy,
                                                     float *__restrict__ g, float *__restrict__ out, int act, float slope,
                                                     int64_t rows, int C, int64_t rows_per_block) {
    const int64_t r0 = (int64_t)blockIdx.x * rows_per_block;
    const int64_t r1 = r0 + rows_per_block < rows ? r0 + rows_per_block : rows;
    const int CV = C >> 2;
    const int lanes = CV < NT ? CV : NT;
    const int rl_n = NT / lanes;
    const int c0 = threadIdx.x % lanes, rl = threadIdx.x / lanes;
    extern __shared__ float red[];
    if (threadIdx.x < lanes * rl_n) {
        for (int cv = c0; cv < CV; cv += lanes) {
            float4 s = make_float4(0.f, 0.f, 0.f, 0.f);
            for (int64_t r = r0 + rl; r < r1; r += rl_n) {
                float4 v = reinterpret_cast<const float4 *>(dy)[r * CV + cv];
                if (FUSED) {
                    const float4 yy = reinterpret_cast<const float4 *>(y)[r * CV + cv];
                    v.x *= hoig_act_grad_from_y(yy.x, act, slope);
                    v.y *= hoig_act_grad_from_y(yy.y, act, slope);
                    v.z *= hoig_act_grad_from_y(yy.z, act, slope);
                    v.w *= hoig_act_grad_from_y(yy.w, act, slope);
                    reinterpret_cast<float4 *>(g)[r * CV + cv] = v;
                }
                s.x += v.x; s.y += v.y; s.z += v.z; s.w += v.w;
            }
            *reinterpret_cast<float4 *>(&red[rl * C + cv * 4]) = s;
        }
    }
    __syncthreads();
    for (int c = threadIdx.x; c < C; c += NT) {
        float s = 0.f;
        for (int k = 0; k < rl_n; ++k) s += red[k * C + c];
        atomicAdd(&out[c], s);
    }
}

__global__ __launch_bounds__(NT) void colsum_kernel(const float *__restrict__ x, float *__restrict__ out, int64_t rows,
                                                    int C, int64_t rows_per_block) {
    const int64_t r0 = (int64_t)blockIdx.x * rows_per_block;
    const int64_t r1 = r0 + rows_per_block < rows ? r0 + rows_per_block : rows;
    const int lanes = C < NT ? C : NT;
    const int rl_n = NT / lanes;
    const int c0 = threadIdx.x % lanes, rl = threadIdx.x / lanes;
    extern __shared__ float red[];
    if (threadIdx.x < lanes * rl_n) {
        for (int c = c0; c < C; c += lanes) {
            float s = 0.f;
            for (int64_t r = r0 + rl; r < r1; r += rl_n) s += x[r * C + c];
            red[rl * C + c] = s;
        }
    }
    __syncthreads();
// ... 87 lines not shown
    for (int64_t i = (int64_t)blockIdx.x * NT + threadIdx.x; i < n; i += (int64_t)gridDim.x * NT) {
        const int x = (int)(i % W), y = (int)((i / W) % H);
        const float v = m[i];
        float g = 0.f;
        if (x + 1 < W) {
            const float d = v - m[i + 1];
            ax += fabsf(d);
            g += gx * (d > 0.f ? 1.f : (d < 0.f ? -1.f : 0.f));
        }
        if (x > 0) {
            const float d = m[i - 1] - v;
            g -= gx * (d > 0.f ? 1.f : (d < 0.f ? -1.f : 0.f));
        }
        if (y + 1 < H) {
            const float d = v - m[i + W];
            ay += fabsf(d);
            g += gy * (d > 0.f ? 1.f : (d < 0.f ? -1.f : 0.f));
        }
        if (y > 0) {
            const float d = m[i - W] - v;
            g -= gy * (d > 0.f ? 1.f : (d < 0.f ? -1.f : 0.f));
        }
        if (dm) dm[i] = g;
    }
    const float sx = block_sum(ax);
    const float sy = block_sum(ay);
    if (threadIdx.x == 0) {
        if (one) {
            atomicAdd(&out[0], sx * gx + sy * gy);
        } else {
            atomicAdd(&out[0], sx);
            atomicAdd(&out[1], sy);
        }
    }
}

__global__ __launch_bounds__(NT) void sum_kernel(const float *__restrict__ x, float *__restrict__ out, int64_t n, float scale) {
    float acc = 0.f;
    for (int64_t i = (int64_t)blockIdx.x * NT + threadIdx.x; i < n; i += (int64_t)gridDim.x * NT) acc += x[i];
    const float s = block_sum(acc);
    if (threadIdx.x == 0) atomicAdd(out, s * scale);
}

__global__ void maxpool_fwd_kernel(const float *__restrict__ x, float *__restrict__ y, int B, int H, int W, int C) {
    const int Ho = H / 2, Wo = W / 2;
    const int64_t n = (int64_t)B * Ho * Wo * C;
    for (int64_t i = (int64_t)blockIdx.x * NT + threadIdx.x; i < n; i += (int64_t)gridDim.x * NT) {
        const int c = (int)(i % C);
        int64_t p = i / C;
        const int wo = (int)(p % Wo);
        p /= Wo;
        const int ho = (int)(p % Ho), b = (int)(p / Ho);
        const float *s = x + (((size_t)b * H + 2 * ho) * W + 2 * wo) * C + c;
        const float a = s[0], bb = s[C], cc = s[(size_t)W * C], d = s[(size_t)W * C + C];
        y[i] = fmaxf(fmaxf(a, bb), fmaxf(cc, d));
    }
}

__global__ void maxpool_bwd_kernel(const float *__restrict__ x, const float *__restrict__ dy, float *__restrict__ dx,
                                   int B, int H, int W, int C) {
    const int Ho = H / 2, Wo = W / 2;
    const int64_t n = (int64_t)B * Ho * Wo * C;
    for (int64_t i = (int64_t)blockIdx.x * NT + threadIdx.x; i < n; i += (int64_t)gridDim.x * NT) {
        const int c = (int)(i % C);
        int64_t p = i / C;
        const int wo = (int)(p % Wo);
        p /= Wo;
        const int ho = (int)(p % Ho), b = (int)(p / Ho);
        const size_t o = (((size_t)b * H + 2 * ho) * W + 2 * wo) * C + c;
        const size_t offs[4] = {0, (size_t)C, (size_t)W * C, (size_t)W * C + C};
        int best = 0;
        float bv = x[o];
#pragma unroll
        for (int k = 1; k < 4; ++k) {
            const float v = x[o + offs[k]];
            if (v > bv) { bv = v; best = k; }
        }
        const float g = dy[i];
#pragma unroll
        for (int k = 0; k < 4; ++k) dx[o + offs[k]] = (k == best) ? g : 0.f;
    }
}

__global__ __launch_bounds__(NT) void adam_kernel(float *__restrict__ p, const float *__restrict__ g, float *__restrict__ m,
                                                  float *__restrict__ v, int64_t n, float step_size, float omb1, float b2,
                                                  float omb2, float eps, float bc2_sqrt, float gscale) {
    const int64_t n4 = n >> 2;
    for (int64_t i = (int64_t)blockIdx.x * NT + threadIdx.x; i < n4; i += (int64_t)gridDim.x * NT) {
        float4 pp = reinterpret_cast<float4 *>(p)[i];
        const float4 gg = reinterpret_cast<const float4 *>(g)[i];
        float4 mm = reinterpret_cast<float4 *>(m)[i], vv = reinterpret_cast<float4 *>(v)[i];
        float *pe = &pp.x, *me = &mm.x, *ve = &vv.x;
        const float *ge = &gg.x;
#pragma unroll
        for (int k = 0; k < 4; ++k) {
            const float gk = ge[k] * gscale;
            me[k] = me[k] + (gk - me[k]) * omb1;
            ve[k] = ve[k] * b2 + omb2 * (gk * gk);
            const float denom = sqrtf(ve[k]) / bc2_sqrt + eps;
            pe[k] = pe[k] - step_size * (me[k] / denom);
        }
        reinterpret_cast<float4 *>(p)[i] = pp;
        reinterpret_cast<float4 *>(m)[i] = mm;
        reinterpret_cast<float4 *>(v)[i] = vv;
    }
    for (int64_t i = (n4 << 2) + (int64_t)blockIdx.x * NT + threadIdx.x; i < n; i += (int64_t)gridDim.x * NT) {
        const float gk = g[i] * gscale;
        const float mk = m[i] + (gk - m[i]) * omb1;
        const float vk = v[i] * b2 + omb2 * (gk * gk);
        m[i] = mk;
        v[i] = vk;
        p[i] = p[i] - step_size * (mk / (sqrtf(vk) / bc2_sqrt + eps));
    }
}

__global__ void adam_tick_kernel(double *__restrict__ state, float *__restrict__ derived) {
    if (threadIdx.x != 0 || blockIdx.x != 0) return;
    const double lr = state[0], b1 = state[1], b2 = state[2], eps = state[3];
    const double step = state[4] + 1.0;
    state[4] = step;
    const double bc1 = 1.0 - pow(b1, step), bc2 = 1.0 - pow(b2, step);
    derived[0] = (float)(lr / bc1);
    derived[1] = (float)(1.0 - b1);
    derived[2] = (float)b2;
    derived[3] = (float)(1.0 - b2);
    derived[4] = (float)eps;
    derived[5] = (float)sqrt(bc2);
}

__global__ __launch_bounds__(NT) void adam_dev_kernel(float *__restrict__ p, const float *__restrict__ g, float *__restrict__ m,
                                                      float *__restrict__ v, int64_t n, const float *__restrict__ derived,
                                                      float gscale) {
    const float step_size = derived[0], omb1 = derived[1], b2 = derived[2], omb2 = derived[3], eps = derived[4],
                bc2_sqrt = derived[5];
    const int64_t n4 = n >> 2;
    for (int64_t i = (int64_t)blockIdx.x * NT + threadIdx.x; i < n4; i += (int64_t)gridDim.x * NT) {
        float4 pp = reinterpret_cast<float4 *>(p)[i];
        const float4 gg = reinterpret_cast<const float4 *>(g)[i];
        float4 mm = reinterpret_cast<float4 *>(m)[i], vv = reinterpret_cast<float4 *>(v)[i];
        float *pe = &pp.x, *me = &mm.x, *ve = &vv.x;
        const float *ge = &gg.x;
#pragma unroll
        for (int k = 0; k < 4; ++k) {
            const float gk = ge[k] * gscale;
            me[k] = me[k] + (gk - me[k]) * omb1;
            ve[k] = ve[k] * b2 + omb2 * (gk * gk);
            const float denom = sqrtf(ve[k]) / bc2_sqrt + eps;
            pe[k] = pe[k] - step_size * (me[k] / denom);
        }
        reinterpret_cast<float4 *>(p)[i] = pp;
        reinterpret_cast<float4 *>(m)[i] = mm;
        reinterpret_cast<float4 *>(v)[i] = vv;
    }
    for (int64_t i = (n4 << 2) + (int64_t)blockIdx.x * NT + threadIdx.x; i < n; i += (int64_t)gridDim.x * NT) {
        const float gk = g[i] * gscale;
        const float mk = m[i] + (gk - m[i]) * omb1;
        const float vk = v[i] * b2 + omb2 * (gk * gk);
        m[i] = mk;
        v[i] = vk;
        p[i] = p[i] - step_size * (mk / (sqrtf(vk) / bc2_sqrt + eps));
    }
}

__device__ __forceinline__ uint8_t tensor2im_byte(float v, int unnorm) {
    if (unnorm) { v += 1.0f; v /= 2.0f; }
    v *= 255.0f;
// ... 116 lines not shown
    if (!bg || !obj || !hand || !mbg || !mh || !img) return HOIG_EINVAL;
    compose_fwd_kernel<<<hoig_stream_grid(npix * C, NT), NT, 0, ST>>>(bg, obj, hand, mbg, mh, img, npix, C);
    HOIG_LAUNCH_CHECK();
    return HOIG_OK;
}
extern "C" int hoig_compose_bwd(const float *bg, const float *obj, const float *hand, const float *mbg, const float *mh,
                                const float *dimg, float *dbg, float *dobj, float *dhand, float *dmbg, float *dmh,
                                int64_t npix, int C, hoig_stream_t stream) {
    if (!bg || !obj || !hand || !mbg || !mh || !dimg || !dbg || !dobj || !dhand || !dmbg || !dmh) return HOIG_EINVAL;
    compose_bwd_kernel<<<hoig_stream_grid(npix, NT), NT, 0, ST>>>(bg, obj, hand, mbg, mh, dimg, dbg, dobj, dhand, dmbg,
                                                                 dmh, npix, C);
    HOIG_LAUNCH_CHECK();
    return HOIG_OK;
}
static bool loss_vec_ok(const void *a, const void *b, const void *c) {
    return (((uintptr_t)a | (uintptr_t)b | (uintptr_t)c) & 15) == 0;
}
extern "C" int hoig_loss_fwd_bwd(int kind, const float *pred, const float *target, float target_const, float gscale,
                                 float *out, float *dpred, int64_t n, hoig_stream_t stream) {
    if (!pred || !out || kind < 0 || kind > 2) return HOIG_EINVAL;
    int g = hoig_stream_grid(n / 4 + 1, NT);
    if (g > 256) g = 256;
    loss_kernel<<<g, NT, 0, ST>>>(kind, pred, target, target_const, gscale, out, dpred, n, 1.f, loss_vec_ok(pred, target, dpred));
    HOIG_LAUNCH_CHECK();
    return HOIG_OK;
}
extern "C" int hoig_loss_accumulate(int kind, const float *pred, const float *target, float target_const, float gscale,
                                    float *term, float *dpred, int64_t n, hoig_stream_t stream) {
    if (!pred || !term || kind < 0 || kind > 2) return HOIG_EINVAL;
    int g = hoig_stream_grid(n / 4 + 1, NT);
    if (g > 256) g = 256;
    loss_kernel<<<g, NT, 0, ST>>>(kind, pred, target, target_const, gscale, term, dpred, n, gscale, loss_vec_ok(pred, target, dpred));
    HOIG_LAUNCH_CHECK();
    return HOIG_OK;
}
extern "C" int hoig_tv_fwd_bwd(const float *m, float gx, float gy, float *out, float *dm, int B, int H, int W,
                               hoig_stream_t stream) {
    if (!m || !out) return HOIG_EINVAL;
    int g = hoig_stream_grid((int64_t)B * H * W, NT);
    if (g > 512) g = 512;
    tv_kernel<<<g, NT, 0, ST>>>(m, gx, gy, out, dm, B, H, W, false);
    HOIG_LAUNCH_CHECK();
    return HOIG_OK;
}
extern "C" int hoig_tv_accumulate(const float *m, float gx, float gy, float *term, float *dm, int B, int H, int W,
                                  hoig_stream_t stream) {
    if (!m || !term) return HOIG_EINVAL;
    int g = hoig_stream_grid((int64_t)B * H * W, NT);
    if (g > 512) g = 512;
    tv_kernel<<<g, NT, 0, ST>>>(m, gx, gy, term, dm, B, H, W, true);
    HOIG_LAUNCH_CHECK();
    return HOIG_OK;
}
extern "C" int hoig_sum(const float *x, float *out, int64_t n, hoig_stream_t stream) {
    if (!x || !out) return HOIG_EINVAL;
    int g = hoig_stream_grid(n, NT);
    if (g > 512) g = 512;
    sum_kernel<<<g, NT, 0, ST>>>(x, out, n, 1.f);
    HOIG_LAUNCH_CHECK();
    return HOIG_OK;
}
extern "C" int hoig_sum_scaled(const float *x, float scale, float *out, int64_t n, hoig_stream_t stream) {
    if (!x || !out) return HOIG_EINVAL;
    int g = hoig_stream_grid(n, NT);
    if (g > 512) g = 512;
    sum_kernel<<<g, NT, 0, ST>>>(x, out, n, scale);
    HOIG_LAUNCH_CHECK();
    return HOIG_OK;
}
extern "C" int hoig_maxpool2_fwd(const float *x, float *y, int B, int H, int W, int C, hoig_stream_t stream) {
    if (!x || !y || (H & 1) || (W & 1)) return HOIG_EINVAL;
    maxpool_fwd_kernel<<<hoig_stream_grid((int64_t)B * H * W * C / 4, NT), NT, 0, ST>>>(x, y, B, H, W, C);
    HOIG_LAUNCH_CHECK();
    return HOIG_OK;
}
extern "C" int hoig_maxpool2_bwd(const float *x, const float *y, const float *dy, float *dx, int B, int H, int W, int C,
                                 hoig_stream_t stream) {
    (void)y;
    if (!x || !dy || !dx || (H & 1) || (W & 1)) return HOIG_EINVAL;
    maxpool_bwd_kernel<<<hoig_stream_grid((int64_t)B * H * W * C / 4, NT), NT, 0, ST>>>(x, dy, dx, B, H, W, C);
    HOIG_LAUNCH_CHECK();
    return HOIG_OK;
}
extern "C" int hoig_adam_step(float *param, const float *grad, float *exp_avg, float *exp_avg_sq, int64_t n, double lr,
                              double beta1, double beta2, double eps, int step, float grad_scale,
                              hoig_stream_t stream) {
    if (!param || !grad || !exp_avg || !exp_avg_sq || step < 1) return HOIG_EINVAL;
    const double bc1 = 1.0 - pow(beta1, step), bc2 = 1.0 - pow(beta2, step);
    const float step_size = (float)(lr / bc1);
    const float bc2_sqrt = (float)sqrt(bc2);
    adam_kernel<<<hoig_stream_grid(n / 4 + 1, NT), NT, 0, ST>>>(param, grad, exp_avg, exp_avg_sq, n, step_size,
                                                               (float)(1.0 - beta1), (float)beta2, (float)(1.0 - beta2),
                                                               (float)eps, bc2_sqrt, grad_scale);
    HOIG_LAUNCH_CHECK();
    return HOIG_OK;
}
extern "C" int hoig_adam_tick(double *state, float *derived, hoig_stream_t stream) {
    if (!state || !derived) return HOIG_EINVAL;
    adam_tick_kernel<<<1, 64, 0, ST>>>(state, derived);
    HOIG_LAUNCH_CHECK();
    return HOIG_OK;
}
extern "C" int hoig_adam_step_dev(float *param, const float *grad, float *exp_avg, float *exp_avg_sq, int64_t n,
                                  const float *derived, float grad_scale, hoig_stream_t stream) {
    if (!param || !grad || !exp_avg || !exp_avg_sq || !derived) return HOIG_EINVAL;
    adam_dev_kernel<<<hoig_stream_grid(n / 4 + 1, NT), NT, 0, ST>>>(param, grad, exp_avg, exp_avg_sq, n, derived, grad_scale);
    HOIG_LAUNCH_CHECK();
    return HOIG_OK;
}
extern "C" int hoig_tensor2im_u8(const float *x, uint8_t *out, int B, int H, int W, int C, int nrow, int unnormalize,
                                 hoig_stream_t stream) {
    if (!x || !out || nrow <= 0) return HOIG_EINVAL;
    const int ncol = nrow < B ? nrow : B;
    const int nrw = (B + ncol - 1) / ncol;
    tensor2im_kernel<<<hoig_stream_grid((int64_t)B * H * W * C, NT), NT, 0, ST>>>(x, out, B, H, W, C, ncol, nrw,
                                                                                 unnormalize);
    HOIG_LAUNCH_CHECK();
    return HOIG_OK;
}
extern "C" int hoig_tensor2im_nhwc_u8(const float *x, uint8_t *out, int64_t n, int unnormalize, hoig_stream_t stream) {
    if (!x || !out || n < 0) return HOIG_EINVAL;
    if (n == 0) return HOIG_OK;
    tensor2im_nhwc_kernel<<<hoig_stream_grid(n, NT), NT, 0, ST>>>(x, out, n, unnormalize);
    HOIG_LAUNCH_CHECK();
    return HOIG_OK;
}
extern "C" int hoig_stream_create(hoig_stream_t *out) {
    if (!out) return HOIG_EINVAL;
    hipStream_t s = nullptr;
    if (hipStreamCreateWithPriority(&s, hipStreamNonBlocking, 0) != hipSuccess) return HOIG_ELAUNCH;
    *out = (hoig_stream_t)s;
    return HOIG_OK;
}
namespace {
struct Scratch { void *ptr; int64_t bytes; };
std::mutex g_scratch_mu;
std::map<std::pair<int, hipStream_t>, Scratch> g_scratch;
std::pair<int, hipStream_t> scratch_key(hipStream_t st) {
    int dev = 0;
    (void)hipGetDevice(&dev);
    return std::make_pair(dev, st);
}
bool g_scratch_warned = false;
}
namespace hoig_detail {
void *stream_scratch(hipStream_t st, size_t bytes) {
    std::lock_guard<std::mutex> lock(g_scratch_mu);
    auto it = g_scratch.find(scratch_key(st));
    if (it != g_scratch.end() && (size_t)it->second.bytes >= bytes) return it->second.ptr;
    if (!g_scratch_warned) {
        g_scratch_warned = true;
        fprintf(stderr, "hoig: no scratch block of %zu bytes registered for stream %p (hoig_stream_scratch_set): partial sums fall back to "
                        "atomics\n", bytes, (void *)st);
    }
    return nullptr;
}
}
extern "C" int64_t hoig_stream_scratch_bytes(void) { return (int64_t)16 << 20; }
extern "C" int hoig_stream_scratch_set(hoig_stream_t stream, void *ptr, int64_t bytes) {
    std::lock_guard<std::mutex> lock(g_scratch_mu);
    if (!ptr || bytes <= 0) g_scratch.erase(scratch_key((hipStream_t)stream));
    else g_scratch[scratch_key((hipStream_t)stream)] = Scratch{ptr, bytes};
    return HOIG_OK;
}
extern "C" int hoig_stream_destroy(hoig_stream_t stream) {
    if (!stream) return HOIG_EINVAL;
// ... 5 lines not shown
```

### hoig_amd/csrc/tuning.h

```cpp
#pragma once
enum HoigTuning { HOIG_TUNE_IGEMM16 = 0, HOIG_TUNE_S2_16, HOIG_TUNE_FLAT5, HOIG_TUNE_WFLAT5, HOIG_TUNE_HEAD16, HOIG_TUNE_D_EARLY, HOIG_TUNE_SPLIT_GRADS, HOIG_TUNE_PAIR, HOIG_TUNE_WDMA16, HOIG_TUNE_S2_PIPE, HOIG_TUNE_NORM_IN, HOIG_TUNE_WINO8, HOIG_TUNE_HALO5, HOIG_TUNE_COUNT };
int hoig_tuning(int id);
```

### hoig_amd/csrc/tuning.hip

```cpp
#include <cstring>
#include "hoig_kernels.h"
#include "tuning.h"

namespace {
struct Entry {
    const char *key;
    int value;
};
Entry g_table[HOIG_TUNE_COUNT] = {
    {"igemm16", 1},
    {"s2_16", 1},
    {"flat5", 2},
    {"wflat5", 1},
    {"head16", 1},
    {"d_early", 1},
    {"split_grads", 1},
    {"pair", 2},
    {"wdma16", 2},
    {"s2_pipe", 1},
    {"norm_in", 1},
    {"wino8", 0},
    {"halo5", 1},
};
}

int hoig_tuning(int id) { return (id >= 0 && id < HOIG_TUNE_COUNT) ? g_table[id].value : 0; }

extern "C" int hoig_set_tuning(const char *key, int value) {
    if (!key) return -1;
    for (int i = 0; i < HOIG_TUNE_COUNT; ++i)
        if (strcmp(g_table[i].key, key) == 0) {
            const int prev = g_table[i].value;
            if (value >= 0) g_table[i].value = value;
            return prev;
        }
    return -1;
}
```

### hoig_amd/ops.py

```python
import collections
import contextlib
import ctypes
import os

import torch
from torch.autograd import Function

from . import _lib as L
from ._lib import ConvDesc

_PREC = {'f32': L.PREC_F32, 'bf16x3': L.PREC_BF16X3, 'f16x3': L.PREC_BF16X3, 'f16x2': L.PREC_F16X2, 'bf16x2': L.PREC_F16X2,
         'bf16': L.PREC_BF16, 'f16': L.PREC_BF16, 'f16f6': L.PREC_F16F6}
precision = precision_dgrad = precision_wgrad = L.PREC_F32


def set_precision(name):
    global precision, precision_dgrad, precision_wgrad
    parts = name.split(':')
    if len(parts) > 3:
        raise ValueError('precision %r' % name)
    precision = _PREC[parts[0]]
    if precision == L.PREC_F16F6 and len(parts) == 1:
        parts = [parts[0], 'f16x2']
    if L.PREC_F16F6 in [_PREC[q] for q in parts[1:]]:
        raise ValueError('f16f6 is a forward arithmetic')
    precision_dgrad = _PREC[parts[1]] if len(parts) > 1 else precision
    precision_wgrad = _PREC[parts[2]] if len(parts) > 2 else precision_dgrad


set_precision(os.environ.get('HOIG_PRECISION', 'f32'))


@contextlib.contextmanager
def inference_forward_precision(name='f16f6'):
    global precision
    if name in (None, '', 'same') or precision != L.PREC_BF16X3 or torch.is_grad_enabled():
        yield False
        return
    prev, precision = precision, _PREC[name]
    try:
        yield True
    finally:
        precision = prev

_subnet_prec = {}


def set_subnet_precision(mapping):
    _subnet_prec.clear()
    if not mapping:
        return
    if isinstance(mapping, str):
        mapping = dict(kv.split('=') for kv in mapping.split(',') if kv)
    for k, v in mapping.items():
        _subnet_prec[k] = _PREC[v]


def subnet_precision(name):
    return None if precision == L.PREC_F32 else _subnet_prec.get(name)


set_subnet_precision(os.environ.get('HOIG_PRECISION_MAP'))


def _bwd_descs(d):
    same = d.precision == precision or (precision == L.PREC_F16F6 and d.precision == L.PREC_BF16X3)
    if not same:
        return d, d
    out = []
    for prec in (precision_dgrad, precision_wgrad):
        if (d.precision == prec and prec != L.PREC_F16F6) or d.precision == L.PREC_F32:
            out.append(d)
        else:
            b = ConvDesc.from_buffer_copy(d)
            b.precision = prec
            out.append(b)
    return tuple(out)


def _st():
    return torch.cuda.current_stream().cuda_stream


def _p(t):
    return None if t is None else t.data_ptr()


def _chk(t, name='tensor'):
    if t is None:
        return
    if not t.is_cuda:
        raise NotImplementedError('%s: hoig_amd ops run on the HIP device only (no CPU path), as the reference ops '
                                  'do (block_extractor.py:23-24)' % name)
    if t.dtype != torch.float32:
        raise TypeError('%s must be float32' % name)


_index_cache = collections.OrderedDict()


def device_index(rows, device):
    dev = torch.device(device)
    key = (dev, torch.cuda.current_stream(dev).cuda_stream, tuple(int(r) for r in rows))
    hit = _index_cache.get(key)
    if hit is not None:
        _index_cache.move_to_end(key)
        return hit
    t = torch.tensor(key[2], dtype=torch.int64).pin_memory().to(dev, non_blocking=True)
    _index_cache[key] = t
    if len(_index_cache) > 1024:
        _index_cache.popitem(last=False)
    return t


def packed_strides(shape, transposed):
    if transposed:
        ci, co, r, s = shape
        return (1, r * s * ci, s * ci, ci)
    co, ci, r, s = shape
    return (r * s * ci, 1, s * ci, ci)


def pack_weight(w, transposed=False):
    out = torch.empty_strided(tuple(w.shape), packed_strides(w.shape, transposed), dtype=w.dtype, device=w.device)
    out.copy_(w)
    return out


_grad_observer = None


def set_grad_observer(fn):
    global _grad_observer
    prev, _grad_observer = _grad_observer, fn
    return prev


def _grad_epoch():
    if _grad_observer is not None:
        _grad_observer(None)


def _grad_target(p):
    if getattr(p, '_hoig_flat', False):
        if p.grad is None:
            raise RuntimeError('flat parameter without a gradient view')
        if _grad_observer is not None:
            _grad_observer(p)
        return p.grad, False
    if p.dim() == 4:
        g = torch.empty_strided(tuple(p.shape), p.stride(), dtype=p.dtype, device=p.device).zero_()
    else:
        g = torch.zeros_like(p)
    return g, True


_plane_cache = {'bf16': {}, 'f6': {}, 'wino': {}}


def _cached_planes(kind, key, w, alloc, pack, size=None):
    owner = getattr(w, '_hoig_owner', None)
    ver = owner.version if owner is not None else None
    cache = _plane_cache[kind]
    hit = cache.get(key)
    if hit is not None and ver is not None and hit[0] == ver:
        return hit[1], hit[2]
    if hit is not None and (size is None or hit[1].numel() == size):
        a, b = hit[1], hit[2]
    else:
        a, b = alloc()
    pack(a, b)
    if ver is not None:
        cache[key] = (ver, a, b)
    return a, b


def _packed_planes(w, transposed, for_dgrad):
    if transposed:
# ... 217 lines not shown

def wgrad_side_streams():
    return list(_wgrad_streams.values())


def join_wgrad_streams():
    if capturing():
        for s in list(_capture_forked):
            torch.cuda.current_stream(s.device).wait_stream(s)
        _capture_forked.clear()
        return
    for s in _wgrad_streams.values():
        torch.cuda.current_stream(s.device).wait_stream(s)
    _wgrad_pending.clear()


class _SplitToken(object):
    __slots__ = ('readers', 'offered', '__weakref__')

    def __init__(self):
        self.readers, self.offered = 0, None


_split_live = set()


def _split_backward_ok(d, w, live_bias, transposed):
    if not L.lib.hoig_set_tuning(b'split_grads', -1) or transposed or live_bias or d.act != L.ACT_NONE:
        return False
    if not getattr(w, '_hoig_flat', False) or (d.R, d.S, d.stride, d.pad) != (3, 3, 1, 1) or (d.Ho, d.Wo) != (d.Hi, d.Wi):
        return False
    if d.Co % 128 or d.Ci % 32 or d.Wo % 32 or d.Ho % 8:
        return False
    dg, wg = _bwd_descs(d)
    return dg.precision in (L.PREC_F16X2, L.PREC_BF16) and wg.precision in (L.PREC_F16X2, L.PREC_BF16)


def _tag_split(y, slot=0):
    tok = _SplitToken()
    toks = getattr(y.grad_fn, 'split_toks', None)
    if toks is None:
        toks = y.grad_fn.split_toks = {}
    toks[slot] = tok
    y._hoig_split_grad = tok
    return y


def _claim_split(x):
    tok = getattr(x, '_hoig_split_grad', None)
    if tok is not None:
        tok.readers += 1
    return tok


def _writes_split(tok):
    return tok is not None and tok.readers == 1


def _offer_split(tok, dx):
    tok.offered = dx
    _split_live.add(tok)


def _take_split(ctx, dy, slot=0):
    tok = getattr(ctx, 'split_toks', {}).get(slot)
    if tok is None or tok.offered is None:
        return False
    off, tok.offered = tok.offered, None
    _split_live.discard(tok)
    if dy is not off and (dy.data_ptr() != off.data_ptr() or dy.shape != off.shape):
        raise RuntimeError('a norm wrote this convolution\'s incoming gradient as bf16 hi | lo planes, but the gradient that arrived is '
                           'another tensor: the tagged output had a second consumer (autograd summed plane bits with an fp32 gradient) '
                           'or a hook replaced it.  Give the second consumer its own copy, or set the tuning key split_grads=0.')
    return True


def check_split_grads_consumed():
    if _split_live:
        n = len(_split_live)
        for tok in list(_split_live):
            tok.offered = None
        _split_live.clear()
        raise RuntimeError('%d pre-split gradient tensor(s) were not consumed by a convolution backward' % n)


def _unsplit(dys):
    out = torch.empty_like(dys)
    L.call('hoig_unsplit_planes_bf16', _p(dys), _p(out), dys.numel() // dys.shape[-1], dys.shape[-1], _st())
    return out


def _wgrad_launch(device, on_caller, held, launch, d, *args):
    side = None if on_caller else _wgrad_side_stream(device)
    if side is not None:
        side.wait_stream(torch.cuda.current_stream())
    with torch.cuda.stream(side) if side is not None else contextlib.nullcontext():
        if side is not None:
            test_delay('wgrad')
        made = launch(d, *args) if callable(launch) else wgrad_call(launch, d, *args, _st())
    made = tuple(made or ())
    if side is not None:
        _wgrad_hold(side, tuple(held) + made)
    return side is not None, made


def _wgrad_from_split(d, x, dys, dw):
    if L.attempt('hoig_conv2d_bwd_weight_split', ctypes.byref(d), _p(x), _p(dys), _p(dw), _st()):
        return ()
    plain = _unsplit(dys)
    wgrad_call('hoig_conv2d_bwd_weight', d, _p(x), _p(plain), _p(dw), None, _st())
    return (plain,)


def _wgrad_pair_from_split(d, xs, dys, dws):
    if None not in dws and L.attempt('hoig_conv2d_bwd_weight_split_pair', ctypes.byref(d), _p(xs[0]), _p(xs[1]), _p(dys[0]), _p(dys[1]),
                                     _p(dws[0]), _p(dws[1]), _st()):
        return ()
    made = ()
    for x, sp, dw in zip(xs, dys, dws):
        if dw is not None:
            made += _wgrad_from_split(d, x, sp, dw)
    return made


def _dgrad_from_split(d, dys, w, planes, add, dx, unsplit=None):
    if not L.attempt('hoig_conv2d_bwd_data_packed_split', ctypes.byref(d), _p(dys), _p(planes[0]), _p(planes[1]), _p(add), _p(dx), _st()):
        _conv_dgrad_raw(d, unsplit if unsplit is not None else _unsplit(dys), w, dx, False, addend=add)


class _Conv(Function):
    @staticmethod
    def forward(ctx, x, w, b, stride, pad, transposed, act, slope, out_hw, prec, dead_bias=False, fork=False):
        _chk(x, 'x'); _chk(w, 'w'); _chk(b, 'bias')
        assert x.is_contiguous() and x.dim() == 4
        B, Hi, Wi, Ci = x.shape
        if transposed:
            ci_w, Co, R, S = w.shape
        else:
            Co, ci_w, R, S = w.shape
        assert ci_w == Ci, 'channel mismatch %d vs %d' % (ci_w, Ci)
        assert tuple(w.stride()) == packed_strides(w.shape, transposed), 'conv weight is not in packed layout'
        if out_hw is None:
            if transposed:
                raise ValueError('out_hw required for transposed conv')
            out_hw = ((Hi + 2 * pad - R) // stride + 1, (Wi + 2 * pad - S) // stride + 1)
        Ho, Wo = out_hw
        y = torch.empty((B, Ho, Wo, Co), dtype=x.dtype, device=x.device)
        d = ConvDesc(B, Hi, Wi, Ci, Ho, Wo, Co, R, S, stride, pad, 1 if transposed else 0, act, slope, prec)
        _conv_fwd_raw(d, x, w, b, y, transposed, norm_next=dead_bias)
        ctx.d = d
        ctx.d_dg, ctx.d_wg = _bwd_descs(d)
        ctx.transposed = transposed
        ctx.has_bias = b is not None and not dead_bias
        ctx.save_for_backward(x, w, b, y if act != L.ACT_NONE else None)
        ctx.fork = fork
        ctx.split_ok = dead_bias and _split_backward_ok(d, w, ctx.has_bias, transposed)
        if fork:
            ctx.set_materialize_grads(False)
            return y, x
        return y

    @staticmethod
    def backward(ctx, dy, dxr=None):
        _grad_epoch()
        x, w, b, y = ctx.saved_tensors
        d = ctx.d
        if dy is None:
            return (dxr,) + (None,) * 11
        dy = dy.contiguous()
        if _take_split(ctx, dy):
            return _Conv._backward_split(ctx, dy, dxr, x, w)
        dw_ret = db_ret = None
        db, ret_b = None, False
        if ctx.needs_input_grad[1] and ctx.has_bias and ctx.needs_input_grad[2]:
            db, ret_b = _grad_target(b)
            db_ret = db if ret_b else None
        if d.act != L.ACT_NONE:
            g = torch.empty_like(dy)
            if db is not None:
                L.call('hoig_act_bwd_colsum', _p(y), _p(dy), _p(g), _p(db), d.act, d.slope, dy.numel() // d.Co, d.Co, _st())
                db = None
            else:
                L.call('hoig_act_bwd', _p(y), _p(dy), _p(g), d.act, d.slope, dy.numel(), _st())
        else:
            g = dy
        if ctx.needs_input_grad[1]:
            dw, ret_w = _grad_target(w)
            _wgrad_launch(x.device, ret_w or (db is not None and ret_b), (x, g),
                          'hoig_conv2d_bwd_weight', ctx.d_wg, _p(x), _p(g), _p(dw), _p(db))
            dw_ret = dw if ret_w else None
        dx = None
        if ctx.needs_input_grad[0]:
            dx = torch.empty_like(x)
            _conv_dgrad_raw(ctx.d_dg, g, w, dx, ctx.transposed, addend=dxr.contiguous() if dxr is not None else None)
        return dx, dw_ret, db_ret, None, None, None, None, None, None, None, None, None

    @staticmethod
    def _backward_split(ctx, dys, dxr, x, w):
        unsplit = None
        if ctx.needs_input_grad[1]:
            dw, ret_w = _grad_target(w)
            on_side, made = _wgrad_launch(x.device, ret_w, (x, dys), _wgrad_from_split, ctx.d_wg, x, dys, dw)
            if made and not on_side:
                unsplit = made[0]
        dx = None
        if ctx.needs_input_grad[0]:
            dx = torch.empty_like(x)
            add = dxr.contiguous() if dxr is not None else None
            _dgrad_from_split(ctx.d_dg, dys, w, _packed_planes(w, False, True), add, dx, unsplit)
        return (dx, (dw if (ctx.needs_input_grad[1] and ret_w) else None)) + (None,) * 10


def conv2d(x, w, b=None, stride=1, pad=0, act=L.ACT_NONE, slope=0.0, prec=None, dead_bias=False):
    y = _Conv.apply(x, w, b, stride, pad, False, act, slope, None, precision if prec is None else prec, dead_bias)
    return _tag_split(y) if getattr(y.grad_fn, 'split_ok', False) else y


def conv2d_fork(x, w, b=None, stride=1, pad=0, act=L.ACT_NONE, slope=0.0, prec=None, dead_bias=False):
    if not x.requires_grad:
        return conv2d(x, w, b, stride, pad, act, slope, prec, dead_bias), x
    y, xr = _Conv.apply(x, w, b, stride, pad, False, act, slope, None, precision if prec is None else prec, dead_bias, True)
    return (_tag_split(y) if getattr(y.grad_fn, 'split_ok', False) else y), xr


def pair_ok(xa, xb, wa, wb, prec=None):
    prec = precision if prec is None else prec
    mode = L.lib.hoig_set_tuning(b'pair', -1)
    if not mode or (mode == 2 and not capturing()) or prec in (L.PREC_F32, L.PREC_F16F6) or not xa.is_cuda:
        return False
    if xa.shape != xb.shape or wa.shape != wb.shape or tuple(wa.shape[2:]) != (3, 3) or wa.shape[1] != xa.shape[-1]:
        return False
    if not (getattr(wa, '_hoig_flat', False) and getattr(wb, '_hoig_flat', False)):
        return False
    B, H, W_, Ci = xa.shape
    Co = wa.shape[0]
    if W_ % 32 or H % 8 or Ci % 32 or Co % 128 or 2 * B * (H // 8) * (W_ // 32) * (Co // 128) < 96:
        return False
    return precision_dgrad in (L.PREC_F16X2, L.PREC_BF16) and precision_wgrad in (L.PREC_F16X2, L.PREC_BF16) and prec == precision


class _ConvPair(Function):

    @staticmethod
    def forward(ctx, xa, xb, wa, wb, ba, bb, prec, dead_bias, fork):
        for t in (xa, xb, wa, wb, ba, bb):
            _chk(t)
        assert xa.is_contiguous() and xb.is_contiguous()
        B, H, W_, Ci = xa.shape
        Co = wa.shape[0]
        d = ConvDesc(B, H, W_, Ci, H, W_, Co, 3, 3, 1, 1, 0, L.ACT_NONE, 0.0, prec)
        ya, yb = torch.empty((B, H, W_, Co), dtype=xa.dtype, device=xa.device), torch.empty((B, H, W_, Co), dtype=xa.dtype, device=xa.device)
        live = ba is not None and not dead_bias
        (ha, la), (hb, lb) = _packed_planes(wa, False, False), _packed_planes(wb, False, False)
        if not L.attempt('hoig_conv2d_fwd_packed_pair', ctypes.byref(d), _p(xa), _p(xb), _p(ha), _p(la), _p(hb), _p(lb),
                         _p(ba) if live else None, _p(bb) if live else None, _p(ya), _p(yb), _st()):
            _conv_fwd_raw(d, xa, wa, ba if live else None, ya)
            _conv_fwd_raw(d, xb, wb, bb if live else None, yb)
        ctx.d_dg, ctx.d_wg = _bwd_descs(d)
        ctx.live_bias = live
        ctx.save_for_backward(xa, xb, wa, wb, ba if live else None, bb if live else None)
        ctx.split_ok = dead_bias and _split_backward_ok(d, wa, live, False)
        ctx.fork = fork
        if fork:
            ctx.set_materialize_grads(False)
            return ya, yb, xa, xb
        return ya, yb

    @staticmethod
    def backward(ctx, dya, dyb, dxra=None, dxrb=None):
        _grad_epoch()
        xa, xb, wa, wb, ba, bb = ctx.saved_tensors
        if dya is None or dyb is None:
            raise RuntimeError('conv2d_pair: both outputs must be used (a grouped launch has no half)')
        d_dg, d_wg = ctx.d_dg, ctx.d_wg
        B, H, W_, Co = dya.shape
        npix = B * H * W_
        dys, db_ret = [], [None, None]
        for i, (dy, b) in enumerate(((dya, ba), (dyb, bb))):
            dy = dy.contiguous()
            if _take_split(ctx, dy, i):
                dys.append(dy)
                continue
            if ctx.live_bias and ctx.needs_input_grad[4 + i]:
                db, ret_b = _grad_target(b)
                L.call('hoig_colsum_accum', _p(dy), _p(db), npix, Co, _st())
                db_ret[i] = db if ret_b else None
            sp = torch.empty_like(dy)
            L.call('hoig_split_planes_bf16', _p(dy), _p(sp), npix, Co, _st())
            dys.append(sp)
        need = (bool(ctx.needs_input_grad[2]), bool(ctx.needs_input_grad[3]))
        dwa, ret_a = _grad_target(wa) if need[0] else (None, False)
        dwb, ret_b = _grad_target(wb) if need[1] else (None, False)
        if need[0] or need[1]:
            _wgrad_launch(xa.device, ret_a or ret_b, (xa, xb, dys[0], dys[1]), _wgrad_pair_from_split, d_wg, (xa, xb), dys, (dwa, dwb))
        dxa = dxb = None
        if ctx.needs_input_grad[0] or ctx.needs_input_grad[1]:
            dxa, dxb = torch.empty_like(xa), torch.empty_like(xb)
            adds = [None if t is None else t.contiguous() for t in (dxra, dxrb)]
            if (adds[0] is None) != (adds[1] is None):
                adds = [t if t is not None else torch.zeros_like(xa) for t in adds]
            pa, pb = _packed_planes(wa, False, True), _packed_planes(wb, False, True)
            if not L.attempt('hoig_conv2d_bwd_data_packed_split_pair', ctypes.byref(d_dg), _p(dys[0]), _p(dys[1]), _p(pa[0]), _p(pa[1]),
                             _p(pb[0]), _p(pb[1]), _p(adds[0]), _p(adds[1]), _p(dxa), _p(dxb), _st()):
                _dgrad_from_split(d_dg, dys[0], wa, pa, adds[0], dxa)
# ... 72 lines not shown
    HW = H * W_
    C1 = first.shape[-1] if first is not None else 0
    Co = w.shape[0]
    if (precision == L.PREC_F32 or tuple(w.shape[2:]) != (3, 3) or w.shape[1] != C1 + C or C % 32 or C1 % 32 or Co % 64
            or W_ % 32 or H % 8 or not xraw.is_contiguous() or (first is not None and (not first.is_contiguous() or first.shape[:3] != xraw.shape[:3]))
            or not L.lib.hoig_set_tuning(b'norm_in', -1)):
        _stats_drop(xraw)
        return None
    dev = xraw.device
    mean = torch.empty(B * C, dtype=torch.float32, device=dev)
    rstd = torch.empty_like(mean)
    ws, have = _norm_workspace(L.lib.hoig_inorm_workspace_bytes(B, HW, C) // 4, dev, take=(xraw.data_ptr(), B, HW, C))
    if have:
        L.call('hoig_inorm_stats_from_sums', _p(xraw), B, HW, C, eps, _p(mean), _p(rstd), _p(ws), _st())
    else:
        L.call('hoig_inorm_stats', _p(xraw), B, HW, C, eps, _p(mean), _p(rstd), _p(ws), _st())
    Cg = C1 + C
    fold = torch.empty(2, B, Cg, dtype=torch.float32, device=dev)
    if C1:
        fold[0, :, :C1] = 1.0
        fold[1, :, :C1] = 0.0
    L.call('hoig_inorm_fold', _p(mean), _p(rstd), _p(gamma), _p(beta), B, C, fold.data_ptr() + 4 * C1, fold.data_ptr() + 4 * (B * Cg + C1), Cg,
           _st())
    y = torch.empty((B, H, W_, Co), dtype=xraw.dtype, device=dev)
    d = ConvDesc(B, H, W_, Cg, H, W_, Co, 3, 3, 1, 1, 0, L.ACT_NONE, 0.0, precision)
    hi, lo = _packed_planes(w, False, False)
    sws = _conv_stats_workspace(y) if norm_next else None
    a, a2 = (first, xraw) if first is not None else (xraw, None)
    done = False
    if precision == L.PREC_F16F6 and Cg % 64 == 0:
        qh, ql = _f6_planes(w)
        done = L.attempt('hoig_conv2d_fwd_f6_ex', ctypes.byref(d), _p(a), C1, _p(a2), _p(hi), _p(qh), _p(ql), _p(b), fold.data_ptr(),
                         fold.data_ptr() + 4 * B * Cg, C1, _p(y), _p(sws), _st())
    if not done:
        d = _x3(d)
        if not L.attempt('hoig_conv2d_fwd_packed_normin', ctypes.byref(d), _p(a), C1, _p(a2), _p(hi), _p(lo), _p(b), fold.data_ptr(),
                         fold.data_ptr() + 4 * B * Cg, C1, _p(y), _p(sws), _st()):
            return None
    if sws is not None:
        _stats_offer(y)
    return y


class _ConvHeads(Function):

    @staticmethod
    def forward(ctx, x, w, splits, acts, prec):
        _chk(x, 'x'); _chk(w, 'w')
        assert x.is_contiguous() and tuple(w.stride()) == packed_strides(w.shape, False)
        B, H, W_, Ci = x.shape
        Co, _, R, S = w.shape
        assert sum(splits) == Co and len(splits) == len(acts)
        assert Co <= 16, 'the activation codes of the fused heads are 4 bits x 16 channels (hoig_conv2d_fwd_heads)'
        if Co > 16:
            raise ValueError('conv_heads: %d output channels, the per-channel activation codes hold 16' % Co)
        d = _x3(ConvDesc(B, H, W_, Ci, H, W_, Co, R, S, 1, R // 2, 0, L.ACT_NONE, 0.0, prec))
        codes, ch = 0, 0
        for n, a in zip(splits, acts):
            for _ in range(n):
                codes |= (a & 15) << (4 * ch)
                ch += 1
        y = torch.empty((B, H, W_, Co), dtype=x.dtype, device=x.device)
        L.call('hoig_conv2d_fwd_heads', ctypes.byref(d), _p(x), _p(w), None, _p(y), codes, _st())
        outs, off = [], 0
        for n in splits:
            o = torch.empty((B, H, W_, n), dtype=x.dtype, device=x.device)
            _copy_channels(y, o, off, 0, n)
            outs.append(o)
            off += n
        ctx.d_dg, ctx.d_wg = _bwd_descs(d)
        ctx.cfg = (tuple(splits), tuple(acts))
        ctx.save_for_backward(x, w, *[o if a != L.ACT_NONE else None for o, a in zip(outs, acts)])
        return tuple(outs)

    @staticmethod
    def backward(ctx, *douts):
        _grad_epoch()
        x, w = ctx.saved_tensors[:2]
        ys = ctx.saved_tensors[2:]
        splits, acts = ctx.cfg
        B, H, W_, _ = x.shape
        Co = w.shape[0]
        g = torch.empty((B, H, W_, Co), dtype=x.dtype, device=x.device)
        off = 0
        for n, a, yv, dy in zip(splits, acts, ys, douts):
            if dy is None:
                dy = torch.zeros((B, H, W_, n), dtype=x.dtype, device=x.device)
            dy = dy.contiguous()
            if a != L.ACT_NONE:
                t = torch.empty_like(dy)
                L.call('hoig_act_bwd', _p(yv), _p(dy), _p(t), a, 0.0, dy.numel(), _st())
                dy = t
            _copy_channels(dy, g, 0, off, n)
            off += n
        dw_ret = None
        if ctx.needs_input_grad[1]:
            dw, ret_w = _grad_target(w)
            wgrad_call('hoig_conv2d_bwd_weight', ctx.d_wg, _p(x), _p(g), _p(dw), None, _st())
            dw_ret = dw if ret_w else None
        dx = None
        if ctx.needs_input_grad[0]:
            dx = torch.empty_like(x)
            _conv_dgrad_raw(ctx.d_dg, g, w, dx)
        return dx, dw_ret, None, None, None


def conv_heads(x, w, splits, acts, prec=None):
    return _ConvHeads.apply(x, w, tuple(splits), tuple(acts), precision if prec is None else prec)


def conv_transpose2d(x, w, stride=2, pad=1, output_padding=1, prec=None, norm_next=False):
    B, Hi, Wi, _ = x.shape
    R, S = w.shape[2], w.shape[3]
    out_hw = ((Hi - 1) * stride - 2 * pad + R + output_padding, (Wi - 1) * stride - 2 * pad + S + output_padding)
    return _Conv.apply(x, w, None, stride, pad, True, L.ACT_NONE, 0.0, out_hw, precision if prec is None else prec, norm_next)


def set_f6_min_tiles(n):
    return L.lib.hoig_set_f6_min_tiles(int(n))


def _f6_planes(w):
    co, ci, r, s = w.shape
    owner = getattr(w, '_hoig_owner', None)
    if owner is not None and hasattr(owner, 'packed_f6'):
        planes = owner.packed_f6(w)
        if planes is not None:
            return planes
    return _cached_planes(
        'f6', (w.data_ptr(), tuple(w.shape)), w,
        lambda: tuple(torch.empty(L.lib.hoig_f6_plane_bytes(co, r * s, ci), dtype=torch.uint8, device=w.device) for _ in range(2)),
        lambda qh, ql: L.call('hoig_pack_conv_weight_f6', _p(w), co, r * s, ci, _p(qh), _p(ql), _st()))


def _wino_planes(w):
    co, ci = w.shape[0], w.shape[1]
    return _cached_planes(
        'wino', (w.data_ptr(), tuple(w.shape)), w,
        lambda: tuple(torch.empty(L.lib.hoig_wino_plane_halfs(co, ci), dtype=torch.int16, device=w.device) for _ in range(2)),
        lambda uh, ul: L.call('hoig_pack_conv_weight_wino', _p(w), co, ci, _p(uh), _p(ul), _st()))


def _x3(d):
    if d.precision != L.PREC_F16F6:
        return d
    c = ConvDesc.from_buffer_copy(d)
    c.precision = L.PREC_BF16X3
    return c


def _conv_fwd_raw(d, x, w, b, y, transposed=False, norm_next=False):
    if _conv_fwd_ladder(d, x, w, b, y, transposed, norm_next):
        _stats_offer(y)


def _conv_fwd_ladder(d, x, w, b, y, transposed, norm_next):
    ws = None
    if norm_next and d.precision != L.PREC_F32 and d.Ci % 32 == 0 and d.Co % 32 == 0 and d.Co > 32:
        ws = _conv_stats_workspace(y)
    elif norm_next and d.precision != L.PREC_F32 and not transposed and d.Ci <= 12 and d.Co % 64 == 0 and d.stride == 1:
        ws0 = _conv_stats_workspace(y)
        if ws0 is not None and L.attempt('hoig_conv2d_fwd_stats', ctypes.byref(_x3(d)), _p(x), _p(w), _p(b), _p(y), _p(ws0), _st()):
            return True
    if d.precision == L.PREC_F16F6:
        if (not transposed and d.R == 3 and d.S == 3 and d.stride == 1 and d.pad == 1 and d.Ci % 64 == 0 and d.Co % 64 == 0
                and d.Hi % 8 == 0 and d.Wi % 32 == 0):
            hi, _ = _packed_planes(w, False, False)
            qh, ql = _f6_planes(w)
            if L.attempt('hoig_conv2d_fwd_f6_ex', ctypes.byref(d), _p(x), 0, None, _p(hi), _p(qh), _p(ql), _p(b), None, None, 0, _p(y),
                         _p(ws), _st()):
                return ws is not None
        d = _x3(d)
    if (ws is None and d.precision == L.PREC_BF16X3 and not transposed and d.R == 3 and d.S == 3 and d.stride == 1 and d.pad == 1
            and d.Ci % 32 == 0 and d.Co % 64 == 0 and d.Hi % 16 == 0 and d.Wi % 16 == 0 and L.lib.hoig_set_tuning(b'wino8', -1) == 1
            and d.B * (d.Hi // 16) * (d.Wi // 16) * (d.Co // 64) <= 256 and d.B * (d.Hi // 8) * ((d.Wi + 31) // 32) * ((d.Co + 127) // 128) <= 128):
        uh, ul = _wino_planes(w)
        if L.attempt('hoig_conv2d_fwd_wino', ctypes.byref(d), _p(x), _p(uh), _p(ul), _p(b), _p(y), _st()):
            return False
    if ws is not None:
        hi, lo = _packed_planes(w, transposed, False)
        if L.attempt('hoig_conv2d_fwd_packed_stats', ctypes.byref(d), _p(x), _p(hi), _p(lo), _p(b), _p(y), _p(ws), _st()):
            return True
    if d.precision != L.PREC_F32 and d.Ci % 32 == 0 and d.Co % 32 == 0 and d.Co > 32:
        hi, lo = _packed_planes(w, transposed, False)
        if L.attempt('hoig_conv2d_fwd_packed', ctypes.byref(d), _p(x), _p(hi), _p(lo), _p(b), _p(y), _st()):
            return False
    L.call('hoig_conv2d_fwd', ctypes.byref(d), _p(x), _p(w), _p(b), _p(y), _st())
    return False


def _conv_dgrad_raw(d, g, w, dx, transposed=False, addend=None):
    packed = d.precision != L.PREC_F32 and d.Co % 32 == 0 and d.Ci % 32 == 0 and d.Ci > 32
    if packed:
        hi, lo = _packed_planes(w, transposed, True)
        if addend is not None and L.attempt('hoig_conv2d_bwd_data_packed_add', ctypes.byref(d), _p(g), _p(hi), _p(lo), _p(addend), _p(dx), _st()):
            return
    out = dx if addend is None else torch.empty_like(dx)
    if not (packed and L.attempt('hoig_conv2d_bwd_data_packed', ctypes.byref(d), _p(g), _p(hi), _p(lo), _p(out), _st())):
        L.call('hoig_conv2d_bwd_data', ctypes.byref(d), _p(g), _p(w), _p(out), _st())
    if addend is not None:
        L.call('hoig_add', _p(out), _p(addend), _p(dx), dx.numel(), _st())


def _reexport():
    import importlib
    g = globals()
    for mod in ('ops_norm', 'ops_small', 'ops_attn', 'ops_loss'):
        m = importlib.import_module('.' + mod, __package__)
        for k, v in vars(m).items():
            if not k.startswith('__') and k not in ('_o', 'L', 'ConvDesc', 'Function', 'torch', 'contextlib'):
                g[k] = v


_reexport()
```

### hoig_amd/ops_small.py

```python
import torch
from torch.autograd import Function

from . import _lib as L
from . import ops as _o
from .ops import _chk, _p, _st, packed_strides

class _Add(Function):
    @staticmethod
    def forward(ctx, a, b):
        _chk(a); _chk(b)
        assert a.shape == b.shape and a.is_contiguous() and b.is_contiguous()
        y = torch.empty_like(a)
        L.call('hoig_add', _p(a), _p(b), _p(y), a.numel(), _st())
        return y

    @staticmethod
    def backward(ctx, dy):
        return dy, dy


def add(a, b):
    return _Add.apply(a, b)


# ... 55 lines not shown
                outs.append(dy[..., off:off + c])
            else:
                outs.append(None)
            off += c
        return tuple(outs)


def cat_channels(xs):
    return _Cat.apply(*xs)


class _PadChannels(Function):

    @staticmethod
    def forward(ctx, x, c_to):
        _chk(x)
        assert x.is_contiguous() and c_to > x.shape[-1]
        y = torch.zeros(x.shape[:-1] + (c_to,), dtype=x.dtype, device=x.device)
        _copy_channels(x, y, 0, 0, x.shape[-1])
        ctx.c = x.shape[-1]
        return y

    @staticmethod
    def backward(ctx, dy):
        return dy[..., :ctx.c], None


class _PadConvIn(Function):

    @staticmethod
    def forward(ctx, w, c_to):
        co, ci, r, s_ = w.shape
        assert tuple(w.stride()) == packed_strides(w.shape, False) and c_to > ci
        out = torch.empty_strided((co, c_to, r, s_), packed_strides((co, c_to, r, s_), False), dtype=w.dtype, device=w.device)
        out.zero_()
        out[:, :ci].copy_(w)
        ctx.ci = ci
        return out

    @staticmethod
    def backward(ctx, dw):
        return dw[:, :ctx.ci], None


def conv2d_padded_in(x, w, b, stride, pad, act=L.ACT_NONE, slope=0.0, prec=None, to=32):
    p = _o.precision if prec is None else prec
    if p == L.PREC_F32 or x.shape[-1] % 32 == 0 or not x.is_cuda:
        return _o.conv2d(x, w, b, stride, pad, act, slope, prec=prec)
    return _o.conv2d(_PadChannels.apply(x, to), _PadConvIn.apply(w, to), b, stride, pad, act, slope, prec=prec)


def slice_channels(x, a, b):
    y = torch.empty(x.shape[:-1] + (b - a,), dtype=x.dtype, device=x.device)
    _copy_channels(x, y, a, 0, b - a)
    return y


def nchw_to_nhwc(x):
    _chk(x)
    x = x.contiguous()
    B, C, H, W = x.shape
    y = torch.empty((B, H, W, C), dtype=x.dtype, device=x.device)
    L.call('hoig_nchw_to_nhwc', _p(x), _p(y), B, C, H, W, _st())
    return y


def nhwc_to_nchw(x):
    _chk(x)
    x = x.contiguous()
    B, H, W, C = x.shape
    y = torch.empty((B, C, H, W), dtype=x.dtype, device=x.device)
    L.call('hoig_nhwc_to_nchw', _p(x), _p(y), B, C, H, W, _st())
    return y


class _MaxPool(Function):
    @staticmethod
    def forward(ctx, x):
        _chk(x)
        B, H, W, C = x.shape
        y = torch.empty((B, H // 2, W // 2, C), dtype=x.dtype, device=x.device)
        L.call('hoig_maxpool2_fwd', _p(x), _p(y), B, H, W, C, _st())
        ctx.save_for_backward(x)
        return y

    @staticmethod
    def backward(ctx, dy):
        x, = ctx.saved_tensors
        B, H, W, C = x.shape
        dx = torch.empty_like(x)
        L.call('hoig_maxpool2_bwd', _p(x), None, _p(dy.contiguous()), _p(dx), B, H, W, C, _st())
        return dx


def maxpool2(x):
    return _MaxPool.apply(x)


def resize_bilinear_ac(x, ho, wo):
    B, Hi, Wi, C = x.shape
    y = torch.empty((B, ho, wo, C), dtype=x.dtype, device=x.device)
    L.call('hoig_resize_bilinear_ac', _p(x.contiguous()), _p(y), B, Hi, Wi, C, ho, wo, _st())
    return y


def resize_nearest(x, ho, wo):
    B, Hi, Wi, C = x.shape
    if (Hi, Wi) == (ho, wo):
        return x
    y = torch.empty((B, ho, wo, C), dtype=x.dtype, device=x.device)
    L.call('hoig_resize_nearest', _p(x.contiguous()), _p(y), B, Hi, Wi, C, ho, wo, _st())
    return y


def attn_flow(tscale):
    B, h = tscale.shape[0], tscale.shape[1]
    flow = torch.empty((B, 2, h, h), dtype=tscale.dtype, device=tscale.device)
    L.call('hoig_attn_flow', _p(tscale.contiguous()), _p(flow), B, h, _st())
    return flow


class _GridSample(Function):
    @staticmethod
    def forward(ctx, x, grid):
        _chk(x); _chk(grid)
        B, H, W, C = x.shape
        Ho, Wo = grid.shape[1], grid.shape[2]
        y = torch.empty((B, Ho, Wo, C), dtype=x.dtype, device=x.device)
        L.call('hoig_grid_sample_fwd', _p(x), _p(grid), _p(y), B, H, W, C, Ho, Wo, _st())
        ctx.save_for_backward(grid)
        ctx.shape = (B, H, W, C, Ho, Wo)
        return y

    @staticmethod
    def backward(ctx, dy):
        grid, = ctx.saved_tensors
        B, H, W, C, Ho, Wo = ctx.shape
        dx = torch.zeros((B, H, W, C), dtype=dy.dtype, device=dy.device)
        L.call('hoig_grid_sample_bwd', _p(grid), _p(dy.contiguous()), _p(dx), B, H, W, C, Ho, Wo, _st())
        return dx, None


def grid_sample(x, grid):
    return _GridSample.apply(x, grid.contiguous())
```

### include/hoig_kernels.h

```cpp
#ifndef HOIG_KERNELS_H
#define HOIG_KERNELS_H

#include <stddef.h>
#include <stdint.h>

#ifdef __cplusplus
extern "C" {
#endif

typedef void *hoig_stream_t;

enum { HOIG_OK = 0, HOIG_EINVAL = -1, HOIG_ELAUNCH = -2, HOIG_EUNSUPPORTED = -3 };

enum { HOIG_ACT_NONE = 0, HOIG_ACT_RELU = 1, HOIG_ACT_LRELU = 2, HOIG_ACT_TANH = 3, HOIG_ACT_SIGMOID = 4 };

enum { HOIG_PREC_F32 = 0, HOIG_PREC_BF16X3 = 1, HOIG_PREC_BF16 = 2, HOIG_PREC_F16X2 = 3, HOIG_PREC_F16F6 = 4 };

typedef struct hoig_conv_desc {
    int32_t B, Hi, Wi, Ci;
    int32_t Ho, Wo, Co;
    int32_t R, S;
    int32_t stride, pad;
    int32_t transposed;
    int32_t act;
    float slope;
    int32_t precision;
} hoig_conv_desc;

int hoig_conv2d_fwd(const hoig_conv_desc *d, const float *x, const float *w, const float *bias ,
                    float *y, hoig_stream_t stream);
int hoig_conv2d_bwd_data(const hoig_conv_desc *d, const float *dy, const float *w, float *dx, hoig_stream_t stream);
int hoig_conv2d_bwd_weight(const hoig_conv_desc *d, const float *x, const float *dy, float *dw, float *dbias,
                           hoig_stream_t stream);

int hoig_split_planes_bf16(const float *x, uint16_t *out, int64_t npix, int C, hoig_stream_t stream);
int hoig_unsplit_planes_bf16(const uint16_t *in, float *out, int64_t npix, int C, hoig_stream_t stream);
int hoig_inorm_bwd_add_ld_split(const float *x, const float *mean, const float *rstd, int mode, const float *p0, const float *p1,
                                int ld_p, const float *y, const float *dy, int act, float slope, const float *addend ,
                                uint16_t *dx_split, float *dp0, float *dp1, int B, int HW, int C, void *workspace,
                                hoig_stream_t stream);
int hoig_inorm_bwd_fused_add_split(const float *x, const float *mean, const float *rstd, int mode, const float *p0, const float *p1,
                                   int ld_p, const float *y, const float *dy, int act, float slope, const float *addend ,
                                   uint16_t *dx_split, float *dp0, float *dp1, int B, int HW, int C, hoig_stream_t stream);
int64_t hoig_wino_plane_halfs(int Co, int Ci);
int hoig_pack_conv_weight_wino(const float *w , int Co, int Ci, uint16_t *u_hi, uint16_t *u_lo, hoig_stream_t stream);
int hoig_conv2d_fwd_wino(const hoig_conv_desc *d, const float *x, const uint16_t *u_hi, const uint16_t *u_lo, const float *bias ,
                         float *y, hoig_stream_t stream);
int hoig_inorm_fold(const float *mean, const float *rstd, const float *gamma , const float *beta , int B, int C,
                    float *scale, float *shift, int ld_out, hoig_stream_t stream);
int hoig_conv2d_fwd_packed_normin(const hoig_conv_desc *d, const float *x, int C1, const float *x2 , const uint16_t *w_hi,
                                  const uint16_t *w_lo, const float *bias , const float *in_scale, const float *in_shift,
                                  int in_relu_c0, float *y, double *stats , hoig_stream_t stream);
int hoig_conv2d_bwd_weight_split(const hoig_conv_desc *d, const float *x, const uint16_t *dy_split, float *dw, hoig_stream_t stream);
int hoig_conv2d_bwd_data_packed_split(const hoig_conv_desc *d, const uint16_t *dy_split, const uint16_t *wt_hi, const uint16_t *wt_lo,
                                      const float *addend , float *dx, hoig_stream_t stream);

int hoig_conv2d_fwd_packed_pair(const hoig_conv_desc *d, const float *xa, const float *xb, const uint16_t *wa_hi, const uint16_t *wa_lo,
                                const uint16_t *wb_hi, const uint16_t *wb_lo, const float *bias_a ,
                                const float *bias_b , float *ya, float *yb, hoig_stream_t stream);
int hoig_conv2d_bwd_data_packed_split_pair(const hoig_conv_desc *d, const uint16_t *dys_a, const uint16_t *dys_b, const uint16_t *wta_hi,
                                           const uint16_t *wta_lo, const uint16_t *wtb_hi, const uint16_t *wtb_lo,
                                           const float *addend_a , const float *addend_b , float *dxa, float *dxb,
                                           hoig_stream_t stream);
int hoig_conv2d_bwd_weight_split_pair(const hoig_conv_desc *d, const float *xa, const float *xb, const uint16_t *dys_a,
                                      const uint16_t *dys_b, float *dwa, float *dwb, hoig_stream_t stream);

int hoig_conv2d_fwd_heads(const hoig_conv_desc *d, const float *x, const float *w, const float *bias , float *y,
                          uint64_t acts, hoig_stream_t stream);

int hoig_pack_conv_weight_bf16(const float *w, int Co, int RS, int Ci, int for_dgrad, uint16_t *hi, uint16_t *lo ,
                               hoig_stream_t stream);
int hoig_pack_conv_weights_bf16_all(const float *flat, const int64_t *segs, int nseg, int64_t ntiles, uint16_t *hi_f,
                                    uint16_t *lo_f, uint16_t *hi_d, uint16_t *lo_d, hoig_stream_t stream);
int hoig_conv2d_fwd_packed(const hoig_conv_desc *d, const float *x, const uint16_t *w_hi, const uint16_t *w_lo,
                           const float *bias , float *y, hoig_stream_t stream);
int hoig_conv2d_bwd_data_packed(const hoig_conv_desc *d, const float *dy, const uint16_t *wt_hi, const uint16_t *wt_lo,
                                float *dx, hoig_stream_t stream);
int hoig_conv2d_fwd_packed_stats(const hoig_conv_desc *d, const float *x, const uint16_t *w_hi, const uint16_t *w_lo,
                                 const float *bias , float *y, double *stats, hoig_stream_t stream);
int hoig_conv2d_cat_fwd_packed_stats(const hoig_conv_desc *d, const float *x1, int C1, const float *x2, const uint16_t *w_hi,
                                     const uint16_t *w_lo, const float *bias , float *y, double *stats,
                                     hoig_stream_t stream);
int hoig_conv2d_fwd_stats(const hoig_conv_desc *d, const float *x, const float *w, const float *bias , float *y, double *stats,
                          hoig_stream_t stream);
int hoig_conv2d_bwd_data_packed_add(const hoig_conv_desc *d, const float *dy, const uint16_t *wt_hi, const uint16_t *wt_lo,
                                    const float *addend, float *dx, hoig_stream_t stream);

int64_t hoig_f6_plane_bytes(int Co, int RS, int Ci);
int hoig_pack_conv_weight_f6(const float *w, int Co, int RS, int Ci, uint8_t *q_hi, uint8_t *q_lo, hoig_stream_t stream);
int hoig_conv2d_fwd_f6(const hoig_conv_desc *d, const float *x, const uint16_t *w_hi, const uint8_t *q_hi, const uint8_t *q_lo,
                       const float *bias , float *y, hoig_stream_t stream);
int hoig_conv2d_cat_fwd_f6(const hoig_conv_desc *d, const float *x1, int C1, const float *x2, const uint16_t *w_hi,
                           const uint8_t *q_hi, const uint8_t *q_lo, const float *bias , float *y,
                           hoig_stream_t stream);
int hoig_conv2d_fwd_f6_ex(const hoig_conv_desc *d, const float *x, int C1, const float *x2 , const uint16_t *w_hi,
                          const uint8_t *q_hi, const uint8_t *q_lo, const float *bias , const float *in_scale ,
                          const float *in_shift , int in_relu_c0, float *y, double *stats , hoig_stream_t stream);
int hoig_pack_conv_weights_f6_all(const float *flat, const int64_t *rows, int nrows, int64_t ntasks, uint8_t *q_hi, uint8_t *q_lo,
                                  hoig_stream_t stream);
int hoig_set_f6_min_tiles(int n);

int hoig_conv2d_cat_fwd_packed(const hoig_conv_desc *d, const float *x1, int C1, const float *x2, const uint16_t *w_hi,
                               const uint16_t *w_lo, const float *bias , float *y, hoig_stream_t stream);
int hoig_conv2d_cat_bwd_data_packed(const hoig_conv_desc *d, const float *dy, const uint16_t *wt_hi, const uint16_t *wt_lo,
                                    float *dx1, int C1, float *dx2, hoig_stream_t stream);
int hoig_conv2d_cat_bwd_weight(const hoig_conv_desc *d, const float *x1, int C1, const float *x2, const float *dy, float *dw,
                               float *dbias , hoig_stream_t stream);

int64_t hoig_inorm_workspace_bytes(int B, int HW, int C);
int hoig_inorm_stats(const float *x, int B, int HW, int C, float eps, float *mean, float *rstd, void *workspace,
                     hoig_stream_t stream);
int hoig_inorm_apply(const float *x, const float *mean, const float *rstd, int mode, const float *p0, const float *p1,
                     int act, float slope, const float *residual , float *y, int B, int HW, int C,
                     hoig_stream_t stream);
int hoig_inorm_stats_from_sums(const float *y, int B, int HW, int C, float eps, float *mean, float *rstd, void *workspace,
                               hoig_stream_t stream);
int hoig_inorm_apply_ld(const float *x, const float *mean, const float *rstd, int mode, const float *p0, const float *p1,
                        int ld_p, int act, float slope, const float *residual , float *y, int B, int HW, int C,
                        hoig_stream_t stream);
int hoig_inorm_bwd_ld(const float *x, const float *mean, const float *rstd, int mode, const float *p0, const float *p1,
                      int ld_p, const float *y, const float *dy, int act, float slope, float *dx, float *dp0, float *dp1, int B,
                      int HW, int C, void *workspace, hoig_stream_t stream);
int hoig_inorm_fwd_fused(const float *x, int mode, const float *p0, const float *p1, int ld_p, int act, float slope,
                         const float *residual , float eps, float *y, float *mean, float *rstd, int B, int HW,
                         int C, hoig_stream_t stream);
int hoig_inorm_bwd_fused(const float *x, const float *mean, const float *rstd, int mode, const float *p0, const float *p1,
                         int ld_p, const float *y , const float *dy, int act, float slope,
                         float *dx, float *dp0, float *dp1, int B, int HW, int C, hoig_stream_t stream);
int hoig_inorm_bwd_add_ld(const float *x, const float *mean, const float *rstd, int mode, const float *p0, const float *p1,
                          int ld_p, const float *y, const float *dy, int act, float slope, const float *addend, float *dx,
                          float *dp0, float *dp1, int B, int HW, int C, void *workspace, hoig_stream_t stream);
int hoig_inorm_bwd_fused_add(const float *x, const float *mean, const float *rstd, int mode, const float *p0, const float *p1,
                             int ld_p, const float *y, const float *dy, int act, float slope, const float *addend, float *dx,
                             float *dp0, float *dp1, int B, int HW, int C, hoig_stream_t stream);

int hoig_inorm_bwd(const float *x, const float *mean, const float *rstd, int mode, const float *p0, const float *p1,
                   const float *y, const float *dy, int act, float slope, float *dx, float *dp0, float *dp1, int B, int HW,
                   int C, void *workspace, hoig_stream_t stream);

int hoig_replicate_pad_fwd(const float *x, float *y, int B, int H, int W, int C, int pad, hoig_stream_t stream);
int hoig_replicate_pad_bwd(const float *dy, float *dx, int B, int H, int W, int C, int pad, hoig_stream_t stream);
int hoig_replicate_pad_bwd_add(const float *dy, const float *addend, float *dx, int B, int H, int W, int C, int pad,
                               hoig_stream_t stream);
int hoig_attn_pixel_fwd(const float *gt, const float *gs, const float *flow, const float *w2, const float *b2,
                        const float *source, float *hidden, float *attn, float *out, float *kf , int B, int H,
                        int W, int C, hoig_stream_t stream);
int hoig_attn_pixel_bwd(const float *hidden, const float *attn, const float *w2, const float *source, const float *flow,
                        const float *dout, float *dhidden, float *dw2, float *db2, float *e_ws, int B, int H, int W, int C,
                        hoig_stream_t stream);
int64_t hoig_attn_index_ints(int B, int H, int W);
int hoig_attn_build_index(const float *flow, int32_t *index, int B, int H, int W, hoig_stream_t stream);
int hoig_attn_src_gather(const int32_t *index, const float *kf, const float *dout, const float *init, float *dsource, int B,
                         int H, int W, int C, hoig_stream_t stream);
int hoig_attn_gs_gather(const int32_t *index, const float *flow, const float *dhidden, float *dgs, int B, int H, int W,
                        hoig_stream_t stream);

int hoig_block_extractor_forward(const float *source, const float *flow, float *output, int B, int C, int Hs, int Ws,
                                 int Hf, int Wf, int kernel_size, hoig_stream_t stream);
int hoig_block_extractor_backward(const float *source, const float *flow, const float *grad_output, float *grad_source,
                                  float *grad_flow, int B, int C, int Hs, int Ws, int Hf, int Wf, int kernel_size,
                                  hoig_stream_t stream);
int hoig_local_attn_reshape_forward(const float *inputs, float *output, int B, int Hs, int Ws, int kernel_size,
                                    hoig_stream_t stream);
int hoig_local_attn_reshape_backward(const float *grad_output, float *grad_inputs, int B, int Hs, int Ws,
                                     int kernel_size, hoig_stream_t stream);

int hoig_grid_sample_fwd(const float *x, const float *grid, float *y, int B, int H, int W, int C, int Ho, int Wo,
                         hoig_stream_t stream);
int hoig_grid_sample_bwd(const float *grid, const float *dy, float *dx, int B, int H, int W, int C, int Ho, int Wo,
                         hoig_stream_t stream);
int hoig_resize_bilinear_ac(const float *x, float *y, int B, int Hi, int Wi, int C, int Ho, int Wo,
                            hoig_stream_t stream);
int hoig_resize_nearest(const float *x, float *y, int B, int Hi, int Wi, int C, int Ho, int Wo, hoig_stream_t stream);
int hoig_attn_flow(const float *tscale, float *flow, int B, int h, hoig_stream_t stream);

int hoig_maxpool2_fwd(const float *x, float *y, int B, int H, int W, int C, hoig_stream_t stream);
int hoig_maxpool2_bwd(const float *x, const float *y, const float *dy, float *dx, int B, int H, int W, int C,
                      hoig_stream_t stream);

int hoig_nchw_to_nhwc(const float *x, float *y, int B, int C, int H, int W, hoig_stream_t stream);
int hoig_nhwc_to_nchw(const float *x, float *y, int B, int C, int H, int W, hoig_stream_t stream);
int hoig_copy_channels(const float *x, float *y, int64_t npix, int Cx, int x_off, int Cy, int y_off, int Ccopy,
                       int accumulate, hoig_stream_t stream);
int hoig_cat2_channels(const float *x1, int C1, const float *x2, int C2, float *y, int64_t npix, hoig_stream_t stream);
int hoig_add(const float *a, const float *b, float *y, int64_t n, hoig_stream_t stream);
int hoig_add_act(const float *a, const float *b, float *y, int act, float slope, int64_t n, hoig_stream_t stream);
int hoig_act_bwd(const float *y, const float *dy, float *dx, int act, float slope, int64_t n, hoig_stream_t stream);
int hoig_act_bwd_colsum(const float *y, const float *dy, float *g, float *dbias, int act, float slope, int64_t rows, int C,
                        hoig_stream_t stream);
int hoig_colsum_accum(const float *x, float *out, int64_t rows, int C, hoig_stream_t stream);

int hoig_compose_fwd(const float *bg, const float *obj, const float *hand, const float *mbg, const float *mh, float *img,
                     int64_t npix, int C, hoig_stream_t stream);
int hoig_compose_bwd(const float *bg, const float *obj, const float *hand, const float *mbg, const float *mh,
                     const float *dimg, float *dbg, float *dobj, float *dhand, float *dmbg, float *dmh, int64_t npix,
                     int C, hoig_stream_t stream);

enum { HOIG_LOSS_L1 = 0, HOIG_LOSS_MSE = 1, HOIG_LOSS_BCE = 2 };
int hoig_loss_fwd_bwd(int kind, const float *pred, const float *target, float target_const, float gscale, float *out,
                      float *dpred, int64_t n, hoig_stream_t stream);
int hoig_tv_fwd_bwd(const float *m, float gx, float gy, float *out, float *dm, int B, int H, int W, hoig_stream_t stream);
int hoig_loss_accumulate(int kind, const float *pred, const float *target, float target_const, float gscale, float *term,
                         float *dpred, int64_t n, hoig_stream_t stream);
int hoig_tv_accumulate(const float *m, float gx, float gy, float *term, float *dm, int B, int H, int W, hoig_stream_t stream);
int hoig_sum(const float *x, float *out, int64_t n, hoig_stream_t stream);
int hoig_sum_scaled(const float *x, float scale, float *out, int64_t n, hoig_stream_t stream);

int hoig_adam_step(float *param, const float *grad, float *exp_avg, float *exp_avg_sq, int64_t n, double lr,
                   double beta1, double beta2, double eps, int step, float grad_scale, hoig_stream_t stream);

int hoig_adam_tick(double *state, float *derived, hoig_stream_t stream);
int hoig_adam_step_dev(float *param, const float *grad, float *exp_avg, float *exp_avg_sq, int64_t n, const float *derived,
                       float grad_scale, hoig_stream_t stream);
int hoig_adam_pack_step(float *flat, const float *grad, float *exp_avg, float *exp_avg_sq, const float *derived, float grad_scale,
                        const int64_t *segs, int nseg, int64_t ntiles, const int64_t *plain, int64_t nplain, uint16_t *hi_f,
                        uint16_t *lo_f, uint16_t *hi_d, uint16_t *lo_d, hoig_stream_t stream);

int hoig_stream_create(hoig_stream_t *out);
int hoig_stream_destroy(hoig_stream_t stream);
int64_t hoig_stream_scratch_bytes(void);
int64_t hoig_conv2d_bwd_weight_scratch_bytes(const hoig_conv_desc *d);
int hoig_stream_scratch_set(hoig_stream_t stream, void *ptr, int64_t bytes);

int hoig_tensor2im_u8(const float *x, uint8_t *out, int B, int H, int W, int C, int nrow, int unnormalize,
                      hoig_stream_t stream);
int hoig_tensor2im_nhwc_u8(const float *x, uint8_t *out, int64_t n, int unnormalize, hoig_stream_t stream);

int hoig_prep_texture(const float *src_img, const float *src_faces, const int32_t *src_fim, const int32_t *fim_uv,
                      const float *wim_uv, const float *obj_tex_img, unsigned char *occ_ws, float *tex,
                      hoig_stream_t stream);
int hoig_prep_lookup(const int32_t *fim, const float *wim, const float *map_fn, const float *sem_full,
                     const float *faces_uv_coord, int n_faces, const float *tex, const float *src_faces, float *cond,
                     float *seg, float *hand_region, float *rend, float *T, hoig_stream_t stream);
#define HOIG_PREP_MAX_BATCH 32
int hoig_prep_texture_batched(int B, const float *src_img, const float *src_faces, int64_t face_stride, const int32_t *src_fim,
                              const int32_t *const *fim_uv, const float *const *wim_uv, const float *const *obj_tex_img,
                              unsigned char *occ_ws, float *tex, hoig_stream_t stream);
int hoig_prep_lookup_batched(int B, const int32_t *fim, const float *wim, const float *const *map_fn, const float *const *sem_full,
                             const float *const *faces_uv_coord, const int *n_faces, const float *tex, const float *src_faces,
                             int64_t face_stride, float *cond, float *seg, float *hand_region, float *rend, float *T ,
                             hoig_stream_t stream);
int hoig_prep_assemble(int B, const float *src_img, const float *ref_img, const float *cond_s, const float *cond_r,
                       const float *seg_s, const float *seg_r, const float *hr_s, const float *hr_r, const float *rend_s,
                       const float *rend_r, const float *T_raw, float *src_bg, float *tsf_bg, float *src_obj,
                       float *tsf_obj, float *src_hand, float *ref_hand, int hand_channels, float *T_hand, float *smb,
                       float *rmb, float *smh, float *rmh, hoig_stream_t stream);

size_t hoig_rasterize_workspace_bytes(int B, int F);
int hoig_project_faces(const float *cam, int cam_dim, const float *verts, int V, const int64_t *const *face_lists, const int *n_faces,
                       int B, int Fmax, float eye_z, float pad_value, float *faces_out, hoig_stream_t stream);
int hoig_rasterize_fim_wim(const float *faces, int B, int F, int image_size, float near, float far, int32_t *fim,
                           float *wim, void *workspace, hoig_stream_t stream);

int hoig_resize_linear_u8(const uint8_t *src, int B, int Hs, int Ws, int C, uint8_t *dst, int Hd, int Wd, hoig_stream_t stream);
int hoig_warp_affine_u8(const uint8_t *src, int B, int Hs, int Ws, int C, const double *M, int Hd, int Wd, int mode, void *dst,
                        hoig_stream_t stream);

const char *hoig_version(void);

int hoig_set_tuning(const char *key, int value);

int hoig_mano_lbs(const float *v_template, const float *shapedirs, const float *posedirs, const float *j_template,
                  const float *j_shapedirs, const float *lbs_weights, const int32_t *parents, const float *hands_mean ,
                  const float *hands_components , int ncomps, int V, const float *root, const float *hand,
                  const float *betas, const float *transl , float *verts, int ld_v, float *joints , int B,
                  hoig_stream_t stream);
// ... 64 lines not shown
```

Baseline: 130.0 images/s.

## Fuse activation backward into producer dgrad epilogue and maxpool backward

When a ReLU/LeakyReLU conv output has exactly one reader, that reader's backward (conv dgrad epilogue or maxpool backward) now multiplies in the activation derivative. The producing conv's backward then skips its separate act_bwd pass and extra buffer. A token system tracks reader counts and checks that the masked gradient reaches the right conv. Multi-head act backward plus channel concat is also merged into one gather kernel. This removes elementwise passes and memory traffic in backward, but adds bookkeeping complexity and is not supported with split-K.

```diff
diff --git a/hoig_amd/_lib.py b/hoig_amd/_lib.py
--- a/hoig_amd/_lib.py
+++ b/hoig_amd/_lib.py
@@ -66,6 +66,8 @@
     'hoig_split_planes_bf16': [_vp, _vp, _i64, _i, _vp],
     'hoig_conv2d_bwd_weight_split': [ctypes.POINTER(ConvDesc), _vp, _vp, _vp, _vp],
     'hoig_conv2d_bwd_data_packed_split': [ctypes.POINTER(ConvDesc), _vp, _vp, _vp, _vp, _vp, _vp],
+    'hoig_conv2d_bwd_data_packed_masked': [ctypes.POINTER(ConvDesc), _vp, _vp, _vp, _vp, _vp, _i, _f, _vp, _vp],
+    'hoig_conv2d_bwd_data_packed_split_masked': [ctypes.POINTER(ConvDesc), _vp, _vp, _vp, _vp, _vp, _i, _f, _vp, _vp],
     'hoig_conv2d_fwd_packed_pair': [ctypes.POINTER(ConvDesc)] + [_vp] * 11,
     'hoig_conv2d_bwd_data_packed_split_pair': [ctypes.POINTER(ConvDesc)] + [_vp] * 11,
     'hoig_conv2d_bwd_weight_split_pair': [ctypes.POINTER(ConvDesc)] + [_vp] * 7,
@@ -103,6 +105,8 @@
     'hoig_attn_flow': [_vp, _vp, _i, _i, _vp],
     'hoig_maxpool2_fwd': [_vp, _vp] + [_i] * 4 + [_vp],
     'hoig_maxpool2_bwd': [_vp, _vp, _vp, _vp] + [_i] * 4 + [_vp],
+    'hoig_maxpool2_bwd_masked': [_vp, _vp, _vp] + [_i] * 5 + [_f, _vp],
+    'hoig_heads_act_bwd_gather': [_vp, _vp, _vp, _vp, _i, _vp, _i64, _vp],
     'hoig_nchw_to_nhwc': [_vp, _vp] + [_i] * 4 + [_vp],
     'hoig_nhwc_to_nchw': [_vp, _vp] + [_i] * 4 + [_vp],
     'hoig_copy_channels': [_vp, _vp, _i64, _i, _i, _i, _i, _i, _i, _vp],
diff --git a/hoig_amd/csrc/conv_bf16_common.h b/hoig_amd/csrc/conv_bf16_common.h
--- a/hoig_amd/csrc/conv_bf16_common.h
+++ b/hoig_amd/csrc/conv_bf16_common.h
@@ -95,6 +95,9 @@
     float *C_g2;
     int a_split;
     double *stats;
+    const float *mask_y = nullptr;
+    int mask_act = 0;
+    float mask_slope = 0.f;
 };
 
 struct Geom {
@@ -177,6 +180,9 @@
     const float *bias;
     float *C;
     const float *addend;
+    const float *mask_y = nullptr;
+    int mask_act = 0;
+    float mask_slope = 0.f;
     int Bn, Hc, Wc;
     int Hs, Ws, oy, ox;
     int Hd, Wd;
diff --git a/hoig_amd/csrc/conv_flat16.hip b/hoig_amd/csrc/conv_flat16.hip
--- a/hoig_amd/csrc/conv_flat16.hip
+++ b/hoig_amd/csrc/conv_flat16.hip
@@ -270,6 +270,13 @@
                         const float4 ad = *reinterpret_cast<const float4 *>(p.addend + d + n);
                         o.x += ad.x; o.y += ad.y; o.z += ad.z; o.w += ad.w;
                     }
+                    if (p.mask_y) {
+                        const float4 my = *reinterpret_cast<const float4 *>(p.mask_y + d + n);
+                        o.x *= hoig_act_grad_from_y(my.x, p.mask_act, p.mask_slope);
+                        o.y *= hoig_act_grad_from_y(my.y, p.mask_act, p.mask_slope);
+                        o.z *= hoig_act_grad_from_y(my.z, p.mask_act, p.mask_slope);
+                        o.w *= hoig_act_grad_from_y(my.w, p.mask_act, p.mask_slope);
+                    }
                     *reinterpret_cast<float4 *>(p.C + d + n) = o;
                 }
             }
@@ -362,6 +369,7 @@
     }
     a.steps_per_split = (int)hoig_cdiv(steps, split);
     split = (int)hoig_cdiv(steps, a.steps_per_split);
+    if (split > 1 && a.mask_y) return HOIG_EUNSUPPORTED;
     dim3 grid(a.nblk, split);
     if (split > 1 && hipMemsetAsync(a.C, 0, (size_t)a.Bn * a.Hd * a.Wd * a.N * sizeof(float), st) != hipSuccess) return HOIG_ELAUNCH;
     return KS == 3 ? launch_ks<3>(a, ns, grid, shm, split > 1, st) : launch_ks<5>(a, ns, grid, shm, split > 1, st);
diff --git a/hoig_amd/csrc/conv_halo16.hip b/hoig_amd/csrc/conv_halo16.hip
--- a/hoig_amd/csrc/conv_halo16.hip
+++ b/hoig_amd/csrc/conv_halo16.hip
@@ -325,6 +325,13 @@
                     const float4 ad = *reinterpret_cast<const float4 *>(gadd + pix * p.N + n);
                     v[0] += ad.x; v[1] += ad.y; v[2] += ad.z; v[3] += ad.w;
                 }
+                if (p.mask_y) {
+                    const float4 my = *reinterpret_cast<const float4 *>(p.mask_y + pix * p.N + n);
+                    v[0] *= hoig_act_grad_from_y(my.x, p.mask_act, p.mask_slope);
+                    v[1] *= hoig_act_grad_from_y(my.y, p.mask_act, p.mask_slope);
+                    v[2] *= hoig_act_grad_from_y(my.z, p.mask_act, p.mask_slope);
+                    v[3] *= hoig_act_grad_from_y(my.w, p.mask_act, p.mask_slope);
+                }
 #pragma unroll
                 for (int q = 0; q < 4; ++q) {
                     st1[j][q] += v[q];
diff --git a/hoig_amd/csrc/conv_igemm_bf16.hip b/hoig_amd/csrc/conv_igemm_bf16.hip
--- a/hoig_amd/csrc/conv_igemm_bf16.hip
+++ b/hoig_amd/csrc/conv_igemm_bf16.hip
@@ -953,7 +953,7 @@
             a.nblk = a.Bn * a.tiles_x * a.tiles_y * a.nblk_n;
             return launch_halo3_m16(a, ns, 64, st);
         }
-        if (a.a_split || a.b_split || a.in_scale) return HOIG_EUNSUPPORTED;
+        if (a.a_split || a.b_split || a.in_scale || a.mask_y) return HOIG_EUNSUPPORTED;
         HOIG_NS_SWITCH(ns, return launch_halo3_one<NSX, 2, 2, 64, 0>(a, st));
     }
     if (a.H % 8 == 0 && a.nblk / 2 < 256 && a.nblk >= 192 && a.N % 128 == 0) {
@@ -972,7 +972,7 @@
         a.nblk = a.Bn * a.tiles_x * a.tiles_y * a.nblk_n;
         return launch_halo3_m16(a, ns, 128, st);
     }
-    if (a.a_split || a.b_split || a.in_scale) return HOIG_EUNSUPPORTED;
+    if (a.a_split || a.b_split || a.in_scale || a.mask_y) return HOIG_EUNSUPPORTED;
     const bool wide = a.nblk < 384;
     HOIG_NS_SWITCH(ns, return wide ? launch_halo3_one<NSX, 2, 4, 128, 1>(a, st) : launch_halo3_one<NSX, 2, 2, 128, 0>(a, st));
     return HOIG_EINVAL;
@@ -1316,6 +1316,9 @@
     bool a_split = false;
     const PairSet *g2 = nullptr;
     const InNorm *in = nullptr;
+    const float *mask_y = nullptr;
+    int mask_act = 0;
+    float mask_slope = 0.f;
 };
 
 int run(const Conv &q) {
@@ -1330,6 +1333,8 @@
     const InNorm *in = q.in;
     hipStream_t st = q.st;
     if (in && (dgrad || d->R != 3 || d->S != 3 || d->stride != 1 || d->pad != 1 || d->transposed || a_split || g2))
+        return HOIG_EUNSUPPORTED;
+    if (q.mask_y && (!dgrad || d->R != 3 || d->S != 3 || d->stride != 1 || d->pad != 1 || d->transposed || g2 || q.a2 || q.c2 || q.stats))
         return HOIG_EUNSUPPORTED;
     Args p;
     p.A = a; p.Wh = wh; p.Wl = wl; p.bias = bias; p.C = c;
@@ -1370,6 +1375,7 @@
         h.addend = addend;
         h.stats = stats;
         h.a_split = a_split ? 1 : 0;
+        h.mask_y = q.mask_y; h.mask_act = q.mask_act; h.mask_slope = q.mask_slope;
         h.in_scale = in ? in->scale : nullptr; h.in_shift = in ? in->shift : nullptr; h.in_relu_c0 = in ? in->relu_c0 : 0;
         if (a_split && (d->R != 3 || a2 || !dgrad)) return HOIG_EUNSUPPORTED;
         if ((addend || stats) && c2) return HOIG_EUNSUPPORTED;
@@ -1396,12 +1402,14 @@
         p.N % 128 == 0 && !stats) {
         FlatArgs f;
         f.A = a; f.Wh = wh; f.Wl = wl; f.bias = bias; f.C = c; f.addend = addend;
+        f.mask_y = q.mask_y; f.mask_act = q.mask_act; f.mask_slope = q.mask_slope;
         f.Bn = d->B; f.Hc = d->Hi + 2; f.Wc = d->Wi + 2; f.KS = 3; f.act = p.act; f.slope = p.slope;
         f.Cg = g.Cg; f.N = p.N; f.K = p.K; f.flip = dgrad ? 1 : 0; f.f16 = p.f16; f.oscale = p.oscale;
         f.Hs = d->Hi; f.Ws = d->Wi; f.oy = f.ox = 1; f.Hd = d->Hi; f.Wd = d->Wi;
         const int rc = launch_flat_m16(f, ns, st);
         if (rc != HOIG_EUNSUPPORTED) return rc;
     }
+    if (q.mask_y) return HOIG_EUNSUPPORTED;
     if (hoig_tuning(HOIG_TUNE_FLAT5) != 0 && !d->transposed && d->stride == 1 && d->R == 5 && d->S == 5 && d->pad == 0 &&
         d->Ho == d->Hi - 4 && d->Wo == d->Wi - 4 && p.N % 128 == 0 && !stats) {
         FlatArgs f;
@@ -1543,6 +1551,24 @@
                     .st = (hipStream_t)stream, .addend = addend, .a_split = true});
 }
 
+extern "C" int hoig_conv2d_bwd_data_packed_masked(const hoig_conv_desc *d, const float *dy, const uint16_t *wt_hi, const uint16_t *wt_lo,
+                                                  const float *addend, const float *mask_y, int act, float slope, float *dx,
+                                                  hoig_stream_t stream) {
+    if (!d || !dy || !wt_hi || !dx || !mask_y) return HOIG_EINVAL;
+    if (!is_16bit_precision(d->precision)) return HOIG_EINVAL;
+    return run(Conv{.d = d, .a = dy, .wh = wt_hi, .wl = wt_lo, .c = dx, .dgrad = true, .st = (hipStream_t)stream, .addend = addend,
+                    .mask_y = mask_y, .mask_act = act, .mask_slope = slope});
+}
+extern "C" int hoig_conv2d_bwd_data_packed_split_masked(const hoig_conv_desc *d, const uint16_t *dy_split, const uint16_t *wt_hi,
+                                                        const uint16_t *wt_lo, const float *addend, const float *mask_y, int act,
+                                                        float slope, float *dx, hoig_stream_t stream) {
+    if (!d || !dy_split || !wt_hi || !dx || !mask_y) return HOIG_EINVAL;
+    if (!is_16bit_precision(d->precision)) return HOIG_EINVAL;
+    if (d->precision == HOIG_PREC_BF16X3 || d->transposed || d->stride != 1 || d->R != 3 || d->S != 3) return HOIG_EUNSUPPORTED;
+    return run(Conv{.d = d, .a = reinterpret_cast<const float *>(dy_split), .wh = wt_hi, .wl = wt_lo, .c = dx, .dgrad = true,
+                    .st = (hipStream_t)stream, .addend = addend, .a_split = true, .mask_y = mask_y, .mask_act = act, .mask_slope = slope});
+}
+
 extern "C" int hoig_conv2d_fwd_packed_pair(const hoig_conv_desc *d, const float *xa, const float *xb, const uint16_t *wa_hi,
                                            const uint16_t *wa_lo, const uint16_t *wb_hi, const uint16_t *wb_lo, const float *bias_a,
                                            const float *bias_b, float *ya, float *yb, hoig_stream_t stream) {
diff --git a/hoig_amd/csrc/pointwise.hip b/hoig_amd/csrc/pointwise.hip
--- a/hoig_amd/csrc/pointwise.hip
+++ b/hoig_amd/csrc/pointwise.hip
@@ -168,6 +168,25 @@
                                int act, float slope, int64_t n) {
     for (int64_t i = (int64_t)blockIdx.x * NT + threadIdx.x; i < n; i += (int64_t)gridDim.x * NT)
         dx[i] = dy[i] * hoig_act_grad_from_y(y[i], act, slope);
+}
+
+struct HeadsBwd {
+    const float *y[3], *dy[3];
+    int n[3], act[3];
+};
+__global__ void heads_act_bwd_gather_kernel(HeadsBwd h, float *__restrict__ g, int64_t npix, int Cg) {
+    const int64_t n = npix * Cg;
+    const int e1 = h.n[0], e2 = h.n[0] + h.n[1];
+    for (int64_t i = (int64_t)blockIdx.x * NT + threadIdx.x; i < n; i += (int64_t)gridDim.x * NT) {
+        const int64_t p = i / Cg;
+        const int c = (int)(i - p * Cg);
+        const int k = c < e1 ? 0 : (c < e2 ? 1 : 2);
+        const int ch = c - (k == 0 ? 0 : (k == 1 ? e1 : e2));
+        const int64_t src = p * h.n[k] + ch;
+        float v = h.dy[k] ? h.dy[k][src] : 0.f;
+        if (h.act[k] != HOIG_ACT_NONE) v = v * hoig_act_grad_from_y(h.y[k][src], h.act[k], 0.f);
+        g[i] = v;
+    }
 }
 
 __global__ __launch_bounds__(NT) void act_bwd_colsum_kernel(const float *__restrict__ y, const float *__restrict__ dy,
@@ -421,6 +440,32 @@
     }
 }
 
+__global__ void maxpool_bwd_masked_kernel(const float *__restrict__ x, const float *__restrict__ dy, float *__restrict__ dx,
+                                          int B, int H, int W, int C, int act, float slope) {
+    const int Ho = H / 2, Wo = W / 2;
+    const int64_t n = (int64_t)B * Ho * Wo * C;
+    for (int64_t i = (int64_t)blockIdx.x * NT + threadIdx.x; i < n; i += (int64_t)gridDim.x * NT) {
+        const int c = (int)(i % C);
+        int64_t p = i / C;
+        const int wo = (int)(p % Wo);
+        p /= Wo;
+        const int ho = (int)(p % Ho), b = (int)(p / Ho);
+        const size_t o = (((size_t)b * H + 2 * ho) * W + 2 * wo) * C + c;
+        const size_t offs[4] = {0, (size_t)C, (size_t)W * C, (size_t)W * C + C};
+        float xv[4];
+#pragma unroll
+        for (int k = 0; k < 4; ++k) xv[k] = x[o + offs[k]];
+        int best = 0;
+        float bv = xv[0];
+#pragma unroll
+        for (int k = 1; k < 4; ++k)
+            if (xv[k] > bv) { bv = xv[k]; best = k; }
+        const float g = dy[i];
+#pragma unroll
+        for (int k = 0; k < 4; ++k) dx[o + offs[k]] = ((k == best) ? g : 0.f) * hoig_act_grad_from_y(xv[k], act, slope);
+    }
+}
+
 __global__ __launch_bounds__(NT) void adam_kernel(float *__restrict__ p, const float *__restrict__ g, float *__restrict__ m,
                                                   float *__restrict__ v, int64_t n, float step_size, float omb1, float b2,
                                                   float omb2, float eps, float bc2_sqrt, float gscale) {
@@ -703,6 +748,29 @@
     HOIG_LAUNCH_CHECK();
     return HOIG_OK;
 }
+extern "C" int hoig_maxpool2_bwd_masked(const float *x, const float *dy, float *dx, int B, int H, int W, int C, int act, float slope,
+                                        hoig_stream_t stream) {
+    if (!x || !dy || !dx || (H & 1) || (W & 1)) return HOIG_EINVAL;
+    maxpool_bwd_masked_kernel<<<hoig_stream_grid((int64_t)B * H * W * C / 4, NT), NT, 0, ST>>>(x, dy, dx, B, H, W, C, act, slope);
+    HOIG_LAUNCH_CHECK();
+    return HOIG_OK;
+}
+extern "C" int hoig_heads_act_bwd_gather(const float *const *y, const float *const *dy, const int *n, const int *act, int nheads,
+                                         float *g, int64_t npix, hoig_stream_t stream) {
+    if (!y || !dy || !n || !act || !g || nheads < 1 || nheads > 3 || npix <= 0) return HOIG_EINVAL;
+    HeadsBwd h;
+    int Cg = 0;
+    for (int k = 0; k < 3; ++k) {
+        const bool on = k < nheads;
+        h.y[k] = on ? y[k] : nullptr; h.dy[k] = on ? dy[k] : nullptr;
+        h.n[k] = on ? n[k] : 0; h.act[k] = on ? act[k] : HOIG_ACT_NONE;
+        if (on && (n[k] <= 0 || (act[k] != HOIG_ACT_NONE && !y[k]))) return HOIG_EINVAL;
+        Cg += h.n[k];
+    }
+    heads_act_bwd_gather_kernel<<<hoig_stream_grid(npix * Cg, NT), NT, 0, ST>>>(h, g, npix, Cg);
+    HOIG_LAUNCH_CHECK();
+    return HOIG_OK;
+}
 extern "C" int hoig_adam_step(float *param, const float *grad, float *exp_avg, float *exp_avg_sq, int64_t n, double lr,
                               double beta1, double beta2, double eps, int step, float grad_scale,
                               hoig_stream_t stream) {
diff --git a/hoig_amd/csrc/tuning.h b/hoig_amd/csrc/tuning.h
--- a/hoig_amd/csrc/tuning.h
+++ b/hoig_amd/csrc/tuning.h
@@ -1,3 +1,3 @@
 #pragma once
-enum HoigTuning { HOIG_TUNE_IGEMM16 = 0, HOIG_TUNE_S2_16, HOIG_TUNE_FLAT5, HOIG_TUNE_WFLAT5, HOIG_TUNE_HEAD16, HOIG_TUNE_D_EARLY, HOIG_TUNE_SPLIT_GRADS, HOIG_TUNE_PAIR, HOIG_TUNE_WDMA16, HOIG_TUNE_S2_PIPE, HOIG_TUNE_NORM_IN, HOIG_TUNE_WINO8, HOIG_TUNE_HALO5, HOIG_TUNE_COUNT };
+enum HoigTuning { HOIG_TUNE_IGEMM16 = 0, HOIG_TUNE_S2_16, HOIG_TUNE_FLAT5, HOIG_TUNE_WFLAT5, HOIG_TUNE_HEAD16, HOIG_TUNE_D_EARLY, HOIG_TUNE_SPLIT_GRADS, HOIG_TUNE_PAIR, HOIG_TUNE_WDMA16, HOIG_TUNE_S2_PIPE, HOIG_TUNE_NORM_IN, HOIG_TUNE_WINO8, HOIG_TUNE_HALO5, HOIG_TUNE_EPI_MASK, HOIG_TUNE_COUNT };
 int hoig_tuning(int id);
diff --git a/hoig_amd/csrc/tuning.hip b/hoig_amd/csrc/tuning.hip
--- a/hoig_amd/csrc/tuning.hip
+++ b/hoig_amd/csrc/tuning.hip
@@ -21,6 +21,7 @@
     {"norm_in", 1},
     {"wino8", 0},
     {"halo5", 1},
+    {"epi_mask", 1},
 };
 }
 
diff --git a/hoig_amd/ops.py b/hoig_amd/ops.py
--- a/hoig_amd/ops.py
+++ b/hoig_amd/ops.py
@@ -94,6 +94,9 @@
                                   'do (block_extractor.py:23-24)' % name)
     if t.dtype != torch.float32:
         raise TypeError('%s must be float32' % name)
+    tok = getattr(t, '_hoig_mask', None)
+    if tok is not None:
+        tok.readers += 1
 
 
 _index_cache = collections.OrderedDict()
@@ -477,6 +480,55 @@
             tok.offered = None
         _split_live.clear()
         raise RuntimeError('%d pre-split gradient tensor(s) were not consumed by a convolution backward' % n)
+    if _mask_live:
+        n = len(_mask_live)
+        for tok in list(_mask_live):
+            tok.offered = None
+        _mask_live.clear()
+        raise RuntimeError('%d gradient tensor(s) written with an activation backward applied did not reach that activation\'s '
+                           'convolution' % n)
+
+
+class _MaskToken(object):
+    __slots__ = ('act', 'slope', 'readers', 'offered', '__weakref__')
+
+    def __init__(self, act, slope):
+        self.act, self.slope, self.readers, self.offered = act, slope, 0, None
+
+
+_mask_live = set()
+
+
+def _tag_mask(y, act, slope):
+    if act in (L.ACT_RELU, L.ACT_LRELU) and y.grad_fn is not None and L.lib.hoig_set_tuning(b'epi_mask', -1):
+        y.grad_fn.mask_tok = y._hoig_mask = _MaskToken(act, slope)
+    return y
+
+
+def _mask_of(x):
+    return getattr(x, '_hoig_mask', None)
+
+
+def _mask_args(tok, x):
+    return (x, tok.act, tok.slope) if tok is not None and tok.readers == 1 else None
+
+
+def _offer_mask(tok, dx):
+    tok.offered = dx
+    _mask_live.add(tok)
+
+
+def _take_mask(ctx, dy):
+    tok = getattr(ctx, 'mask_tok', None)
+    if tok is None or tok.offered is None:
+        return False
+    off, tok.offered = tok.offered, None
+    _mask_live.discard(tok)
+    if dy is not off and (dy.data_ptr() != off.data_ptr() or dy.shape != off.shape):
+        raise RuntimeError('the single counted reader of this convolution\'s output applied the activation\'s backward to the gradient it '
+                           'wrote, but the gradient that arrived is another tensor: the output had a reader outside hoig_amd.ops (autograd '
+                           'summed a masked gradient with an unmasked one) or a hook replaced it.  Set the tuning key epi_mask=0.')
+    return True
 
 
 def _unsplit(dys):
@@ -518,9 +570,13 @@
     return made
 
 
-def _dgrad_from_split(d, dys, w, planes, add, dx, unsplit=None):
-    if not L.attempt('hoig_conv2d_bwd_data_packed_split', ctypes.byref(d), _p(dys), _p(planes[0]), _p(planes[1]), _p(add), _p(dx), _st()):
-        _conv_dgrad_raw(d, unsplit if unsplit is not None else _unsplit(dys), w, dx, False, addend=add)
+def _dgrad_from_split(d, dys, w, planes, add, dx, unsplit=None, mask=None):
+    if mask is not None and L.attempt('hoig_conv2d_bwd_data_packed_split_masked', ctypes.byref(d), _p(dys), _p(planes[0]), _p(planes[1]),
+                                      _p(add), _p(mask[0]), mask[1], mask[2], _p(dx), _st()):
+        return True
+    if L.attempt('hoig_conv2d_bwd_data_packed_split', ctypes.byref(d), _p(dys), _p(planes[0]), _p(planes[1]), _p(add), _p(dx), _st()):
+        return False
+    return _conv_dgrad_raw(d, unsplit if unsplit is not None else _unsplit(dys), w, dx, False, addend=add, mask=mask)
 
 
 class _Conv(Function):
@@ -549,6 +605,7 @@
         ctx.has_bias = b is not None and not dead_bias
         ctx.save_for_backward(x, w, b, y if act != L.ACT_NONE else None)
         ctx.fork = fork
+        ctx.mask_in = _mask_of(x) if (not transposed and (R, S, stride, pad) == (3, 3, 1, 1)) else None
         ctx.split_ok = dead_bias and _split_backward_ok(d, w, ctx.has_bias, transposed)
         if fork:
             ctx.set_materialize_grads(False)
@@ -570,7 +627,9 @@
         if ctx.needs_input_grad[1] and ctx.has_bias and ctx.needs_input_grad[2]:
             db, ret_b = _grad_target(b)
             db_ret = db if ret_b else None
-        if d.act != L.ACT_NONE:
+        if d.act != L.ACT_NONE and _take_mask(ctx, dy):
+            g = dy
+        elif d.act != L.ACT_NONE:
             g = torch.empty_like(dy)
             if db is not None:
                 L.call('hoig_act_bwd_colsum', _p(y), _p(dy), _p(g), _p(db), d.act, d.slope, dy.numel() // d.Co, d.Co, _st())
@@ -587,7 +646,9 @@
         dx = None
         if ctx.needs_input_grad[0]:
             dx = torch.empty_like(x)
-            _conv_dgrad_raw(ctx.d_dg, g, w, dx, ctx.transposed, addend=dxr.contiguous() if dxr is not None else None)
+            if _conv_dgrad_raw(ctx.d_dg, g, w, dx, ctx.transposed, addend=dxr.contiguous() if dxr is not None else None,
+                               mask=_mask_args(ctx.mask_in, x)):
+                _offer_mask(ctx.mask_in, dx)
         return dx, dw_ret, db_ret, None, None, None, None, None, None, None, None, None
 
     @staticmethod
@@ -602,12 +663,13 @@
         if ctx.needs_input_grad[0]:
             dx = torch.empty_like(x)
             add = dxr.contiguous() if dxr is not None else None
-            _dgrad_from_split(ctx.d_dg, dys, w, _packed_planes(w, False, True), add, dx, unsplit)
+            if _dgrad_from_split(ctx.d_dg, dys, w, _packed_planes(w, False, True), add, dx, unsplit, _mask_args(ctx.mask_in, x)):
+                _offer_mask(ctx.mask_in, dx)
         return (dx, (dw if (ctx.needs_input_grad[1] and ret_w) else None)) + (None,) * 10
 
 
 def conv2d(x, w, b=None, stride=1, pad=0, act=L.ACT_NONE, slope=0.0, prec=None, dead_bias=False):
-    y = _Conv.apply(x, w, b, stride, pad, False, act, slope, None, precision if prec is None else prec, dead_bias)
+    y = _tag_mask(_Conv.apply(x, w, b, stride, pad, False, act, slope, None, precision if prec is None else prec, dead_bias), act, slope)
     return _tag_split(y) if getattr(y.grad_fn, 'split_ok', False) else y
 
 
@@ -615,6 +677,7 @@
     if not x.requires_grad:
         return conv2d(x, w, b, stride, pad, act, slope, prec, dead_bias), x
     y, xr = _Conv.apply(x, w, b, stride, pad, False, act, slope, None, precision if prec is None else prec, dead_bias, True)
+    _tag_mask(y, act, slope)
     return (_tag_split(y) if getattr(y.grad_fn, 'split_ok', False) else y), xr
 
 
@@ -853,17 +916,23 @@
         B, H, W_, _ = x.shape
         Co = w.shape[0]
         g = torch.empty((B, H, W_, Co), dtype=x.dtype, device=x.device)
-        off = 0
-        for n, a, yv, dy in zip(splits, acts, ys, douts):
-            if dy is None:
-                dy = torch.zeros((B, H, W_, n), dtype=x.dtype, device=x.device)
-            dy = dy.contiguous()
-            if a != L.ACT_NONE:
-                t = torch.empty_like(dy)
-                L.call('hoig_act_bwd', _p(yv), _p(dy), _p(t), a, 0.0, dy.numel(), _st())
-                dy = t
-            _copy_channels(dy, g, 0, off, n)
-            off += n
+        if len(splits) <= 3 and L.lib.hoig_set_tuning(b'epi_mask', -1):
+            dys = [None if dy is None else dy.contiguous() for dy in douts]
+            nh = len(splits)
+            L.call('hoig_heads_act_bwd_gather', (ctypes.c_void_p * nh)(*[_p(t) for t in ys]), (ctypes.c_void_p * nh)(*[_p(t) for t in dys]),
+                   (ctypes.c_int * nh)(*splits), (ctypes.c_int * nh)(*acts), nh, _p(g), B * H * W_, _st())
+        else:
+            off = 0
+            for n, a, yv, dy in zip(splits, acts, ys, douts):
+                if dy is None:
+                    dy = torch.zeros((B, H, W_, n), dtype=x.dtype, device=x.device)
+                dy = dy.contiguous()
+                if a != L.ACT_NONE:
+                    t = torch.empty_like(dy)
+                    L.call('hoig_act_bwd', _p(yv), _p(dy), _p(t), a, 0.0, dy.numel(), _st())
+                    dy = t
+                _copy_channels(dy, g, 0, off, n)
+                off += n
         dw_ret = None
         if ctx.needs_input_grad[1]:
             dw, ret_w = _grad_target(w)
@@ -960,10 +1029,13 @@
     return False
 
 
-def _conv_dgrad_raw(d, g, w, dx, transposed=False, addend=None):
+def _conv_dgrad_raw(d, g, w, dx, transposed=False, addend=None, mask=None):
     packed = d.precision != L.PREC_F32 and d.Co % 32 == 0 and d.Ci % 32 == 0 and d.Ci > 32
     if packed:
         hi, lo = _packed_planes(w, transposed, True)
+        if mask is not None and L.attempt('hoig_conv2d_bwd_data_packed_masked', ctypes.byref(d), _p(g), _p(hi), _p(lo), _p(addend),
+                                          _p(mask[0]), mask[1], mask[2], _p(dx), _st()):
+            return True
         if addend is not None and L.attempt('hoig_conv2d_bwd_data_packed_add', ctypes.byref(d), _p(g), _p(hi), _p(lo), _p(addend), _p(dx), _st()):
             return
     out = dx if addend is None else torch.empty_like(dx)
@@ -971,6 +1043,7 @@
         L.call('hoig_conv2d_bwd_data', ctypes.byref(d), _p(g), _p(w), _p(out), _st())
     if addend is not None:
         L.call('hoig_add', _p(out), _p(addend), _p(dx), dx.numel(), _st())
+    return False
 
 
 def _reexport():
diff --git a/hoig_amd/ops_small.py b/hoig_amd/ops_small.py
--- a/hoig_amd/ops_small.py
+++ b/hoig_amd/ops_small.py
@@ -161,6 +161,7 @@
         y = torch.empty((B, H // 2, W // 2, C), dtype=x.dtype, device=x.device)
         L.call('hoig_maxpool2_fwd', _p(x), _p(y), B, H, W, C, _st())
         ctx.save_for_backward(x)
+        ctx.mask_in = _o._mask_of(x)
         return y
 
     @staticmethod
@@ -168,7 +169,12 @@
         x, = ctx.saved_tensors
         B, H, W, C = x.shape
         dx = torch.empty_like(x)
-        L.call('hoig_maxpool2_bwd', _p(x), None, _p(dy.contiguous()), _p(dx), B, H, W, C, _st())
+        mask = _o._mask_args(ctx.mask_in, x)
+        if mask is not None:
+            L.call('hoig_maxpool2_bwd_masked', _p(x), _p(dy.contiguous()), _p(dx), B, H, W, C, mask[1], mask[2], _st())
+            _o._offer_mask(ctx.mask_in, dx)
+        else:
+            L.call('hoig_maxpool2_bwd', _p(x), None, _p(dy.contiguous()), _p(dx), B, H, W, C, _st())
         return dx
 
 
diff --git a/include/hoig_kernels.h b/include/hoig_kernels.h
--- a/include/hoig_kernels.h
+++ b/include/hoig_kernels.h
@@ -85,6 +85,12 @@
                           hoig_stream_t stream);
 int hoig_conv2d_bwd_data_packed_add(const hoig_conv_desc *d, const float *dy, const uint16_t *wt_hi, const uint16_t *wt_lo,
                                     const float *addend, float *dx, hoig_stream_t stream);
+int hoig_conv2d_bwd_data_packed_masked(const hoig_conv_desc *d, const float *dy, const uint16_t *wt_hi, const uint16_t *wt_lo,
+                                       const float *addend , const float *mask_y, int act, float slope, float *dx,
+                                       hoig_stream_t stream);
+int hoig_conv2d_bwd_data_packed_split_masked(const hoig_conv_desc *d, const uint16_t *dy_split, const uint16_t *wt_hi,
+                                             const uint16_t *wt_lo, const float *addend , const float *mask_y, int act,
+                                             float slope, float *dx, hoig_stream_t stream);
 
 int64_t hoig_f6_plane_bytes(int Co, int RS, int Ci);
 int hoig_pack_conv_weight_f6(const float *w, int Co, int RS, int Ci, uint8_t *q_hi, uint8_t *q_lo, hoig_stream_t stream);
@@ -177,11 +183,15 @@
 int hoig_maxpool2_fwd(const float *x, float *y, int B, int H, int W, int C, hoig_stream_t stream);
 int hoig_maxpool2_bwd(const float *x, const float *y, const float *dy, float *dx, int B, int H, int W, int C,
                       hoig_stream_t stream);
+int hoig_maxpool2_bwd_masked(const float *x, const float *dy, float *dx, int B, int H, int W, int C, int act, float slope,
+                             hoig_stream_t stream);
 
 int hoig_nchw_to_nhwc(const float *x, float *y, int B, int C, int H, int W, hoig_stream_t stream);
 int hoig_nhwc_to_nchw(const float *x, float *y, int B, int C, int H, int W, hoig_stream_t stream);
 int hoig_copy_channels(const float *x, float *y, int64_t npix, int Cx, int x_off, int Cy, int y_off, int Ccopy,
                        int accumulate, hoig_stream_t stream);
+int hoig_heads_act_bwd_gather(const float *const *y, const float *const *dy, const int *n, const int *act, int nheads, float *g,
+                              int64_t npix, hoig_stream_t stream);
 int hoig_cat2_channels(const float *x1, int C1, const float *x2, int C2, float *y, int64_t npix, hoig_stream_t stream);
 int hoig_add(const float *a, const float *b, float *y, int64_t n, hoig_stream_t stream);
 int hoig_add_act(const float *a, const float *b, float *y, int act, float slope, int64_t n, hoig_stream_t stream);
```

Result: no change. 130.4 images/s, median of 4 (+0.3%).
